# ZhongLingXiao/nano-kazen

Measured on AMD Instinct MI355X. Metric: Msamples/s (w*h*spp/s) at 1920x1080, 1 M-tri scene, higher is better.
Workload: dtype f32

## Files before the change

include/kazen_mi355x_dev.h:

```cpp
#ifndef KAZEN_MI355X_DEV_H
#define KAZEN_MI355X_DEV_H
#include "kazen_mi355x.h"
#ifdef __cplusplus
extern "C" {
#endif


typedef struct KzStats {
    uint64_t samples;
    uint64_t rays;
    uint64_t nodeVisits;
    uint64_t triTests;
    uint64_t shadedHits;
    uint64_t lightSamples;
    uint64_t droppedSamples;
    uint64_t beamPixels;
    uint64_t beamListEntries;
    uint64_t beamCompletePixels;
} KzStats;

typedef struct KzHit {
    float t;
    float u, v;
    int32_t mesh;
    int32_t prim;
    float p[3];
    float uv[2];
    float sh_s[3], sh_t[3], sh_n[3];
    float geo_n[3];
} KzHit;

typedef struct KzBvhInfo { uint32_t nNodes, nLeaves, nTris, maxDepth, maxLeafSize; float sahCost; double buildSeconds; } KzBvhInfo;
int kz_scene_bvh_info(const KzScene *scene, KzBvhInfo *out);
int kz_scene_sample_count(const KzScene *scene, uint32_t *out);

int kz_scene_devices(const KzScene *scene, int32_t *devices, uint32_t cap, uint32_t *count);

int kz_film_merge(float *dst, const float *src, size_t nFloats);

int kz_film_download_on(KzScene *scene, int device, float *film, size_t nFloats);
int kz_film_clear_on(KzScene *scene, int device, void *stream);
int kz_sync_on(KzScene *scene, int device);

int kz_trace_rays(KzScene *scene, uint32_t n, const float *o, const float *d,
                  const float *tmin, const float *tmax, KzHit *hits);

int kz_render_samples(KzScene *scene, uint32_t n, const int32_t *pxy, const uint32_t *idx, float *out);
int kz_bsdf_query(KzScene *scene, uint32_t n, const int32_t *bsdf, const float *wi, const float *wo, const float *accRough,
                  const float *s3, const float *uv, float *evalOut, float *pdfOut, float *sampleOut);
int kz_texture_query(KzScene *scene, uint32_t n, const int32_t *tex, const float *uv, float *out);

int kz_camera_rays(KzScene *scene, uint32_t n, const float *sxy, const float *axy, float *out);
int kz_light_query(KzScene *scene, uint32_t n, const int32_t *light, const float *ref, const float *u3, float *out);

int kz_set_stats(KzScene *scene, int enable);
int kz_get_stats(KzScene *scene, KzStats *out, int reset);

int kz_last_kernel_ms(KzScene *scene, float *ms);
int kz_last_stage_ms(KzScene *scene, float *out6);

typedef struct KzPassInfo { uint32_t passes; uint32_t passesInFlight; uint64_t itemsPerPass; uint32_t sppPerPass; uint32_t pixels; uint64_t stateBytes;
                            uint32_t pixelsPerPass; uint32_t shadowBeside ; uint64_t firstPassItems; uint64_t largestPassItems;
                            uint64_t contextItems;
                          } KzPassInfo;
int kz_last_pass_info(KzScene *scene, KzPassInfo *out);
typedef struct KzPassModeInfo { int32_t kept; uint32_t timedPasses; uint64_t items; float msOneStream[2]; float msShadowBeside; float msHalves; } KzPassModeInfo;
int kz_pass_mode_info(KzScene *scene, int device, KzPassModeInfo *out);
int kz_last_grow_note(KzScene *scene, char *buf, size_t cap);

void kz_debug_fail_alloc(int nth);
void kz_debug_fail_device(int device, int nth);
void kz_debug_grow_delay(int ms);
void kz_debug_trace(int on);
void kz_debug_alias_devices(int n);

typedef struct KzPlanQuery {
    int32_t pipeline;
    uint32_t nPix;
    uint32_t sampleBegin, sampleEnd;
    uint64_t passItems;
    int32_t passesInFlight;
    int32_t sppPerPass;
    uint64_t limitBytes;
    uint64_t bytesPerItem;
    int32_t dealer;
    uint32_t takers, batchTiles, nTiles;
    const uint32_t *tilePixOffset;
    uint64_t heldItems;
} KzPlanQuery;
typedef struct KzPlanAnswer {
    int32_t autoShape, nCtx, multi, grow;
    uint32_t S, pixPerPass, batchTiles, nPixSet, nPasses;
    uint64_t need, wantItems, minStart;
    double graceMs;
} KzPlanAnswer;
int kz_plan_passes(const KzPlanQuery *q, KzPlanAnswer *a);
int kz_plan_schedule(const KzPlanQuery *q, const uint64_t *avail, uint32_t nAvail, uint32_t pixBegin, uint32_t pixEnd, uint32_t *passes, uint32_t cap, uint32_t *nPasses);

int kz_kat_dpdf(uint32_t n, const float *values, float *cdf, float *sumAndNormalization);
int kz_kat_pow4(int32_t spp, int32_t *out4);

enum { KZ_TABLE_NODES = 0, KZ_TABLE_NODES4 = 1, KZ_TABLE_TRIS = 2, KZ_TABLE_SHADE = 3, KZ_TABLE_CDF = 4, KZ_TABLE_LIGHTS = 5, KZ_TABLE_IL_TRIS = 6, KZ_TABLE_PARAMS = 7,
       KZ_TABLE_BSDFS = 8  };
int kz_scene_table(KzScene *scene, int device, int table, void *out, size_t cap, size_t *bytes);

#define KZ_BUILD_EXPERIMENTS 1
int kz_build_flags(void);
int kz_device_mem_info(int device, uint64_t *freeBytes, uint64_t *totalBytes);
int kz_kat_exact_math(int device, uint64_t *rcpMismatches, uint64_t *sqrtMismatches, uint64_t *checked);
int kz_kat_permute(int device, uint32_t n, const uint32_t *i, const uint32_t *l, const uint32_t *p, uint32_t *out);
int kz_kat_fresnel(int device, uint32_t n, int form, const float *cosThetaI, const float *a, const float *b, float *out);
int kz_kat_math(int device, int fn, uint32_t n, const float *x, const float *y, float *out);


#ifdef __cplusplus
}
#endif
#endif
```

nano-kazen_amd/abi.py:

```python
import ctypes as C
import os

KZ_ABI_VERSION = 6

KZ_OK, KZ_ERR_INVALID_ARG, KZ_ERR_UNSUPPORTED, KZ_ERR_NO_DEVICE, KZ_ERR_HIP, KZ_ERR_STATE, KZ_ERR_OOM = range(7)
KZ_BSDF_DIFFUSE, KZ_BSDF_KAZENSTANDARD, KZ_BSDF_MIRROR, KZ_BSDF_DIELECTRIC = 0, 1, 2, 3
KZ_BSDF_GGX, KZ_BSDF_ROUGHCONDUCTOR, KZ_BSDF_ROUGHPLASTIC, KZ_BSDF_ROUGHDIELECTRIC, KZ_BSDF_NORMALMAP = 4, 5, 6, 7, 8
KZ_TEX_CONSTANT, KZ_TEX_IMAGE, KZ_TEX_COLORRAMP, KZ_TEX_BLEND = 0, 1, 2, 3
KZ_BLEND_MIX, KZ_BLEND_MULTIPLY, KZ_BLEND_NONE = 0, 1, 2
KZ_PIXEL_U8, KZ_PIXEL_F32 = 0, 1
KZ_TEX_MAX_DEPTH = 8
KZ_SAMPLER_INDEPENDENT, KZ_SAMPLER_PMJ02BN, KZ_SAMPLER_STRATIFIED, KZ_SAMPLER_CORRELATED = 0, 1, 2, 3
KZ_CAMERA_PERSPECTIVE, KZ_CAMERA_THINLENS = 0, 1
KZ_INTEGRATOR_PATH_MIS, KZ_INTEGRATOR_NORMALS, KZ_INTEGRATOR_AO, KZ_INTEGRATOR_PATH_MATS = 0, 1, 2, 3
KZ_FILTER_GAUSSIAN, KZ_FILTER_MITCHELL, KZ_FILTER_TENT, KZ_FILTER_BOX = 0, 1, 2, 3
KZ_FILTER_RESOLUTION = 32
KZ_PMJ02BN_SETS, KZ_PMJ02BN_SAMPLES = 5, 65536
KZ_BLUENOISE_TEXTURES, KZ_BLUENOISE_RES = 48, 128

f32p = C.POINTER(C.c_float)
u32p = C.POINTER(C.c_uint32)
u16p = C.POINTER(C.c_uint16)


# ... 10 lines not shown
class KzImage(C.Structure):
    _fields_ = [("pixels", C.c_void_p), ("width", C.c_int32), ("height", C.c_int32), ("channels", C.c_int32), ("format", C.c_int32)]


class KzTexture(C.Structure):
    _fields_ = [("type", C.c_int32), ("color", C.c_float * 3), ("image", C.c_int32), ("scale", C.c_float), ("srgb", C.c_int32),
                ("rampMin", C.c_float), ("rampMax", C.c_float), ("blendMode", C.c_int32), ("child", C.c_int32 * 3), ("filter", C.c_int32), ("pad_", C.c_int32 * 2)]


class KzLight(C.Structure):
    _fields_ = [("color", C.c_float * 3), ("intensity", C.c_float), ("primaryVisibility", C.c_int32)]


class KzMesh(C.Structure):
    _fields_ = [("V", f32p), ("N", f32p), ("UV", f32p), ("F", u32p), ("nV", C.c_uint32), ("nF", C.c_uint32),
                ("bsdf", C.c_int32), ("light", C.c_int32)]


class KzFilter(C.Structure):
    _fields_ = [("type", C.c_int32), ("radius", C.c_float), ("stddev", C.c_float), ("B", C.c_float), ("C", C.c_float)]


class KzCamera(C.Structure):
    _fields_ = [("type", C.c_int32), ("width", C.c_int32), ("height", C.c_int32), ("toWorld", C.c_float * 16),
                ("fov", C.c_float), ("nearClip", C.c_float), ("farClip", C.c_float),
                ("apertureRadius", C.c_float), ("focusDistance", C.c_float),
                ("sampleToCamera", f32p), ("rfilter", KzFilter)]


class KzSampler(C.Structure):
    _fields_ = [("type", C.c_int32), ("sampleCount", C.c_uint32), ("resolution", C.c_int32), ("pad_", C.c_int32), ("seed", C.c_uint64),
                ("pmj02bnSamples", u32p), ("blueNoise", u16p)]


class KzIntegrator(C.Structure):
    _fields_ = [("type", C.c_int32), ("maxDepth", C.c_int32), ("traceBias", C.c_float),
                ("regularization", C.c_int32), ("accumulatedRoughness", C.c_float)]


class KzBackground(C.Structure):
    _fields_ = [("present", C.c_int32), ("color", C.c_float * 3), ("intensity", C.c_float), ("texture", C.c_int32)]


class KzSceneDesc(C.Structure):
    _fields_ = [("abiVersion", C.c_uint32),
                ("meshes", C.POINTER(KzMesh)), ("nMeshes", C.c_uint32),
                ("bsdfs", C.POINTER(KzBSDF)), ("nBsdfs", C.c_uint32),
                ("lights", C.POINTER(KzLight)), ("nLights", C.c_uint32),
                ("camera", KzCamera), ("sampler", KzSampler), ("integrator", KzIntegrator),
                ("background", KzBackground),
                ("textures", C.POINTER(KzTexture)), ("nTextures", C.c_uint32),
                ("images", C.POINTER(KzImage)), ("nImages", C.c_uint32)]


class KzTile(C.Structure):
    _fields_ = [("x0", C.c_int32), ("y0", C.c_int32), ("w", C.c_int32), ("h", C.c_int32)]


class KzTuning(C.Structure):
    _fields_ = [("refill", C.c_int32), ("postpone", C.c_int32), ("batch", C.c_int32), ("traceBlocksPerCU", C.c_int32),
                ("shadeBlocksPerCU", C.c_int32), ("ldsStack", C.c_int32), ("dev0", C.c_int32), ("packetPrimary", C.c_int32),
                ("dev1", C.c_int32), ("dev2", C.c_int32), ("filmGather", C.c_int32), ("dev3", C.c_int32), ("sppPerPass", C.c_int32), ("dev4", C.c_int32),
                ("dev5", C.c_int32), ("streamPriority", C.c_int32)]


class KzTileDealer(C.Structure):
    _fields_ = [("counter", u32p), ("batchTiles", C.c_uint32), ("takers", C.c_uint32), ("taken", u32p), ("takenCap", C.c_uint32), ("nTaken", u32p), ("agreed", u32p)]


class KzRenderOpts(C.Structure):
    _fields_ = [("sampleBegin", C.c_uint32), ("sampleEnd", C.c_uint32), ("tiles", C.POINTER(KzTile)),
                ("nTiles", C.c_uint32), ("pipeline", C.c_int32), ("accumulate", C.c_int32), ("stream", C.c_void_p),
                ("device", C.c_int32), ("passesInFlight", C.c_int32), ("passItems", C.c_uint64), ("maxStateBytes", C.c_uint64),
                ("tune", KzTuning), ("tileDealing", C.c_int32), ("packedOutput", C.c_int32), ("dealer", C.POINTER(KzTileDealer)),
                ("shadowBeside", C.c_int32), ("passHalves", C.c_int32)]


class KzPassInfo(C.Structure):
    _fields_ = [("passes", C.c_uint32), ("passesInFlight", C.c_uint32), ("itemsPerPass", C.c_uint64), ("sppPerPass", C.c_uint32),
                ("pixels", C.c_uint32), ("stateBytes", C.c_uint64), ("pixelsPerPass", C.c_uint32), ("shadowBeside", C.c_uint32),
                ("firstPassItems", C.c_uint64), ("largestPassItems", C.c_uint64), ("contextItems", C.c_uint64)]

    def as_dict(self):
        return {k: int(getattr(self, k)) for k, _ in self._fields_}


class KzPassModeInfo(C.Structure):
    _fields_ = [("kept", C.c_int32), ("timedPasses", C.c_uint32), ("items", C.c_uint64), ("msOneStream", C.c_float * 2), ("msShadowBeside", C.c_float), ("msHalves", C.c_float)]


class KzPlanQuery(C.Structure):
    _fields_ = [("pipeline", C.c_int32), ("nPix", C.c_uint32), ("sampleBegin", C.c_uint32), ("sampleEnd", C.c_uint32), ("passItems", C.c_uint64),
                ("passesInFlight", C.c_int32), ("sppPerPass", C.c_int32), ("limitBytes", C.c_uint64), ("bytesPerItem", C.c_uint64), ("dealer", C.c_int32),
                ("takers", C.c_uint32), ("batchTiles", C.c_uint32), ("nTiles", C.c_uint32), ("tilePixOffset", u32p), ("heldItems", C.c_uint64)]


class KzPlanAnswer(C.Structure):
    _fields_ = [("autoShape", C.c_int32), ("nCtx", C.c_int32), ("multi", C.c_int32), ("grow", C.c_int32), ("S", C.c_uint32), ("pixPerPass", C.c_uint32),
                ("batchTiles", C.c_uint32), ("nPixSet", C.c_uint32), ("nPasses", C.c_uint32), ("need", C.c_uint64), ("wantItems", C.c_uint64),
                ("minStart", C.c_uint64), ("graceMs", C.c_double)]

    def as_dict(self):
        return {k: getattr(self, k) for k, _ in self._fields_}


class KzStats(C.Structure):
    _fields_ = [("samples", C.c_uint64), ("rays", C.c_uint64), ("nodeVisits", C.c_uint64), ("triTests", C.c_uint64),
                ("shadedHits", C.c_uint64), ("lightSamples", C.c_uint64), ("droppedSamples", C.c_uint64),
                ("beamPixels", C.c_uint64), ("beamListEntries", C.c_uint64), ("beamCompletePixels", C.c_uint64)]

    def as_dict(self):
        return {k: int(getattr(self, k)) for k, _ in self._fields_}


class KzHit(C.Structure):
    _fields_ = [("t", C.c_float), ("u", C.c_float), ("v", C.c_float), ("mesh", C.c_int32), ("prim", C.c_int32),
                ("p", C.c_float * 3), ("uv", C.c_float * 2), ("sh_s", C.c_float * 3), ("sh_t", C.c_float * 3),
                ("sh_n", C.c_float * 3), ("geo_n", C.c_float * 3)]


class KzVertexUpdate(C.Structure):
    _fields_ = [("mesh", C.c_uint32), ("nV", C.c_uint32), ("V", f32p), ("N", f32p)]


class KzBsdfUpdate(C.Structure):
    _fields_ = [("row", C.c_uint32), ("bsdf", KzBSDF)]


class KzLightUpdate(C.Structure):
    _fields_ = [("light", C.c_uint32), ("value", KzLight)]


class KzTransformUpdate(C.Structure):
    _fields_ = [("mesh", C.c_uint32), ("toWorld", C.c_float * 16)]


class KzBvhInfo(C.Structure):
    _fields_ = [("nNodes", C.c_uint32), ("nLeaves", C.c_uint32), ("nTris", C.c_uint32), ("maxDepth", C.c_uint32),
                ("maxLeafSize", C.c_uint32), ("sahCost", C.c_float), ("buildSeconds", C.c_double)]


PRODUCT_EXPORTS = ["kz_scene_create", "kz_scene_destroy", "kz_scene_upload", "kz_scene_evict", "kz_render", "kz_render_tiles", "kz_render_multi", "kz_deal_tiles",
                   "kz_tiles_packed_floats", "kz_film_download_tiles", "kz_film_merge_tiles", "kz_film_merge_rects", "kz_film_download", "kz_film_clear", "kz_film_dims", "kz_film_to_rgb",
                   "kz_film_to_srgb8", "kz_sync", "kz_last_error", "kz_abi_version", "kz_device_count", "kz_device_trim"]
EXPORTS = ["kz_scene_create", "kz_scene_destroy", "kz_scene_bvh_info", "kz_scene_upload", "kz_render",
           "kz_film_download", "kz_film_clear", "kz_film_dims", "kz_film_to_rgb", "kz_trace_rays",
           "kz_set_stats", "kz_get_stats", "kz_sync", "kz_last_kernel_ms", "kz_last_error", "kz_abi_version",
           "kz_device_count", "kz_render_samples", "kz_bsdf_query", "kz_scene_sample_count", "kz_last_stage_ms", "kz_texture_query", "kz_film_to_srgb8",
           "kz_scene_evict", "kz_scene_devices", "kz_render_tiles", "kz_render_multi", "kz_deal_tiles", "kz_film_merge", "kz_film_download_on",
           "kz_film_clear_on", "kz_sync_on", "kz_last_pass_info", "kz_device_mem_info", "kz_camera_rays", "kz_light_query", "kz_kat_exact_math", "kz_kat_permute", "kz_kat_fresnel", "kz_kat_math", "kz_build_flags",
           "kz_tiles_packed_floats", "kz_film_download_tiles", "kz_film_merge_tiles", "kz_film_merge_rects", "kz_device_trim", "kz_kat_dpdf", "kz_kat_pow4", "kz_last_grow_note",
           "kz_plan_passes", "kz_plan_schedule", "kz_pass_mode_info", "kz_scene_table"]
EDIT_EXPORTS = ["kz_scene_set_camera", "kz_scene_set_vertices", "kz_scene_set_bsdfs", "kz_scene_set_lights", "kz_scene_set_transforms"]
KZ_TABLE_NODES, KZ_TABLE_NODES4, KZ_TABLE_TRIS, KZ_TABLE_SHADE, KZ_TABLE_CDF, KZ_TABLE_LIGHTS, KZ_TABLE_IL_TRIS, KZ_TABLE_PARAMS, KZ_TABLE_BSDFS = range(9)
DEV_ONLY_EXPORTS = ["kz_debug_fail_alloc", "kz_debug_fail_device", "kz_debug_grow_delay", "kz_debug_trace", "kz_debug_alias_devices"]

_HERE = os.path.dirname(os.path.abspath(__file__))
LIB_PATH = os.environ.get("KZ_LIB_PATH") or os.path.join(_HERE, "csrc", "libkazen_mi355x.so")
DEV_LIB_PATH = os.path.join(_HERE, "csrc", "variants", "experiments", "libkazen_mi355x.so")
_libs = {}


class KzError(RuntimeError):
    def __init__(self, code, msg):
        super().__init__("kazen_mi355x error %d: %s" % (code, msg))
        self.code = code


def load_dev_library():
    return load_library(DEV_LIB_PATH)


def load_library(path=None):
    path = path or LIB_PATH
    if path in _libs:
        return _libs[path]
    if not os.path.exists(path):
        raise ImportError("HIP extension %s is missing: run `python -c 'import __graft_entry__ as g; g.build()'` "
                          "(the product path has no CPU fallback)" % path)
    lib = C.CDLL(path)
    lib.kz_last_error.restype = C.c_char_p
    lib.kz_scene_create.argtypes = [C.POINTER(KzSceneDesc), C.POINTER(C.c_void_p)]
    lib.kz_scene_destroy.argtypes = [C.c_void_p]
    lib.kz_scene_destroy.restype = None
    lib.kz_scene_bvh_info.argtypes = [C.c_void_p, C.POINTER(KzBvhInfo)]
    lib.kz_scene_sample_count.argtypes = [C.c_void_p, u32p]
    lib.kz_scene_upload.argtypes = [C.c_void_p, C.c_int]
    lib.kz_render.argtypes = [C.c_void_p, C.POINTER(KzRenderOpts)]
    lib.kz_film_download.argtypes = [C.c_void_p, f32p, C.c_size_t]
    lib.kz_film_clear.argtypes = [C.c_void_p, C.c_void_p]
    lib.kz_film_dims.argtypes = [C.c_void_p, C.POINTER(C.c_int32), C.POINTER(C.c_int32), C.POINTER(C.c_int32)]
    lib.kz_film_to_rgb.argtypes = [f32p, C.c_int32, C.c_int32, C.c_int32, f32p]
    lib.kz_trace_rays.argtypes = [C.c_void_p, C.c_uint32, f32p, f32p, f32p, f32p, C.POINTER(KzHit)]
    lib.kz_set_stats.argtypes = [C.c_void_p, C.c_int]
    lib.kz_get_stats.argtypes = [C.c_void_p, C.POINTER(KzStats), C.c_int]
    lib.kz_sync.argtypes = [C.c_void_p]
    lib.kz_last_kernel_ms.argtypes = [C.c_void_p, f32p]
    lib.kz_last_stage_ms.argtypes = [C.c_void_p, f32p]
    lib.kz_render_samples.argtypes = [C.c_void_p, C.c_uint32, C.POINTER(C.c_int32), u32p, f32p]
    lib.kz_bsdf_query.argtypes = [C.c_void_p, C.c_uint32, C.POINTER(C.c_int32), f32p, f32p, f32p, f32p, f32p, f32p, f32p, f32p]
    lib.kz_film_to_srgb8.argtypes = [C.c_void_p, C.POINTER(C.c_uint8), C.c_size_t]
    lib.kz_texture_query.argtypes = [C.c_void_p, C.c_uint32, C.POINTER(C.c_int32), f32p, f32p]
    if hasattr(lib, "kz_camera_rays"):
        lib.kz_camera_rays.argtypes = [C.c_void_p, C.c_uint32, f32p, f32p, f32p]
        lib.kz_light_query.argtypes = [C.c_void_p, C.c_uint32, C.POINTER(C.c_int32), f32p, f32p, f32p]
    lib.kz_scene_evict.argtypes = [C.c_void_p, C.c_int]
    lib.kz_scene_devices.argtypes = [C.c_void_p, C.POINTER(C.c_int32), C.c_uint32, u32p]
    lib.kz_render_tiles.argtypes = [C.c_void_p, C.POINTER(KzRenderOpts), C.POINTER(KzTile), C.c_uint32, C.c_int, f32p, C.c_size_t]
    lib.kz_render_multi.argtypes = [C.c_void_p, C.POINTER(KzRenderOpts), C.POINTER(C.c_int32), C.c_uint32, C.c_int32, f32p, C.c_size_t, f32p]
    lib.kz_deal_tiles.argtypes = [C.c_int32, C.c_int32, C.c_int32, C.c_uint32, C.c_uint32, C.POINTER(KzTile), C.c_uint32, u32p]
    lib.kz_film_merge.argtypes = [f32p, f32p, C.c_size_t]
    lib.kz_tiles_packed_floats.argtypes = [C.c_void_p, C.POINTER(KzTile), C.c_uint32, C.POINTER(C.c_size_t)]
    lib.kz_film_download_tiles.argtypes = [C.c_void_p, C.c_int, C.POINTER(KzTile), C.c_uint32, f32p, C.c_size_t]
    lib.kz_film_merge_tiles.argtypes = [f32p, C.c_int32, C.c_int32, C.c_int32, C.POINTER(KzTile), C.c_uint32, f32p, C.c_size_t, C.c_int32]
    lib.kz_film_merge_rects.argtypes = [f32p, C.c_int32, C.c_int32, C.c_int32, C.POINTER(KzTile), C.POINTER(f32p), C.c_uint32, C.c_int32]
    lib.kz_film_download_on.argtypes = [C.c_void_p, C.c_int, f32p, C.c_size_t]
    lib.kz_film_clear_on.argtypes = [C.c_void_p, C.c_int, C.c_void_p]
    lib.kz_sync_on.argtypes = [C.c_void_p, C.c_int]
    lib.kz_last_pass_info.argtypes = [C.c_void_p, C.POINTER(KzPassInfo)]
    lib.kz_pass_mode_info.argtypes = [C.c_void_p, C.c_int32, C.POINTER(KzPassModeInfo)]
    lib.kz_device_mem_info.argtypes = [C.c_int, C.POINTER(C.c_uint64), C.POINTER(C.c_uint64)]
    lib.kz_device_trim.argtypes = [C.c_int]
    lib.kz_last_grow_note.argtypes = [C.c_void_p, C.c_char_p, C.c_size_t]
    for hook in DEV_ONLY_EXPORTS:
        if hasattr(lib, hook):
            getattr(lib, hook).argtypes = [C.c_int, C.c_int] if hook == "kz_debug_fail_device" else [C.c_int]
            getattr(lib, hook).restype = None
    if hasattr(lib, "kz_plan_passes"):
        lib.kz_plan_passes.argtypes = [C.POINTER(KzPlanQuery), C.POINTER(KzPlanAnswer)]
        lib.kz_plan_schedule.argtypes = [C.POINTER(KzPlanQuery), C.POINTER(C.c_uint64), C.c_uint32, C.c_uint32, C.c_uint32, u32p, C.c_uint32, u32p]
    lib.kz_kat_dpdf.argtypes = [C.c_uint32, f32p, f32p, f32p]
    if hasattr(lib, "kz_scene_set_vertices"):
        lib.kz_scene_set_camera.argtypes = [C.c_void_p, C.POINTER(KzCamera)]
        lib.kz_scene_set_vertices.argtypes = [C.c_void_p, C.POINTER(KzVertexUpdate), C.c_uint32]
        lib.kz_scene_table.argtypes = [C.c_void_p, C.c_int, C.c_int, C.c_void_p, C.c_size_t, C.POINTER(C.c_size_t)]
    if hasattr(lib, "kz_scene_set_transforms"):
        lib.kz_scene_set_bsdfs.argtypes = [C.c_void_p, C.POINTER(KzBsdfUpdate), C.c_uint32]
        lib.kz_scene_set_lights.argtypes = [C.c_void_p, C.POINTER(KzLightUpdate), C.c_uint32]
        lib.kz_scene_set_transforms.argtypes = [C.c_void_p, C.POINTER(KzTransformUpdate), C.c_uint32]
    lib.kz_kat_pow4.argtypes = [C.c_int32, C.POINTER(C.c_int32)]
    if hasattr(lib, "kz_kat_math"):
        lib.kz_kat_math.argtypes = [C.c_int, C.c_int, C.c_uint32, f32p, f32p, f32p]
    if hasattr(lib, "kz_kat_fresnel"):
        lib.kz_kat_fresnel.argtypes = [C.c_int, C.c_uint32, C.c_int, f32p, f32p, f32p, f32p]
    if hasattr(lib, "kz_kat_permute"):
        lib.kz_kat_permute.argtypes = [C.c_int, C.c_uint32, u32p, u32p, u32p, u32p]
    if hasattr(lib, "kz_kat_exact_math"):
        lib.kz_kat_exact_math.argtypes = [C.c_int, C.POINTER(C.c_uint64), C.POINTER(C.c_uint64), C.POINTER(C.c_uint64)]
    _libs[path] = lib
    return lib


def check(lib, rc):
    if rc != KZ_OK:
        msg = lib.kz_last_error()
        raise KzError(rc, msg.decode() if msg else "")
```

nano-kazen_amd/csrc/kz_debug.hip:

```cpp
#include "kz_state.h"

#include <algorithm>
#include <atomic>
#include <chrono>
#include <cmath>
#include <cstdio>
#include <cstdlib>
#include <cstring>
#include <mutex>
#include <string>
#include <thread>
#include <vector>
#include "kz_devfn.h"


__global__ __launch_bounds__(KZ_BLOCK) void kz_trace_kernel(KzParams P, KzDevTables T, uint32_t n, const float *__restrict__ o,
                                                            const float *__restrict__ d, const float *__restrict__ tmin,
                                                            const float *__restrict__ tmax, KzHit *__restrict__ hits) {
    __shared__ uint32_t s_stack[KZ_STACK_DEPTH * KZ_BLOCK];
    const uint32_t i = blockIdx.x * KZ_BLOCK + threadIdx.x;
    if (i >= n) return;
    Counters cn = {0, 0, 0, 0, 0, 0};
    RawHit rh;
    KzHit h; memset(&h, 0, sizeof h);
// ... 131 lines not shown

int kz_kat_fresnel(int device, uint32_t n, int form, const float *cosThetaI, const float *a, const float *b, float *out) {
    int nd = kz_device_count();
    if (device < 0 || device >= nd) return kz_fail(nd ? KZ_ERR_INVALID_ARG : KZ_ERR_NO_DEVICE, "device %d out of range (%d visible)", device, nd);
    if (!n) return KZ_OK;
    if (!cosThetaI || !a || !out || (form == 0 && !b) || (form != 0 && form != 1)) return kz_fail(KZ_ERR_INVALID_ARG, "null argument or form %d (0 = fresnel(cos, extIOR, intIOR), 1 = fresnelDielectric(cos, eta))", form);
    HIP_TRY(hipSetDevice(kzPhysicalDevice(device)));
    DevMem dC, dA, dB, dO;
    const size_t bytes = (size_t)n * sizeof(float);
    KZ_ALLOC(&dC.p, bytes); KZ_ALLOC(&dA.p, bytes); KZ_ALLOC(&dB.p, bytes); KZ_ALLOC(&dO.p, 2 * bytes);
    HIP_TRY(hipMemcpy(dC.p, cosThetaI, bytes, hipMemcpyHostToDevice)); HIP_TRY(hipMemcpy(dA.p, a, bytes, hipMemcpyHostToDevice));
    HIP_TRY(hipMemcpy(dB.p, b ? b : a, bytes, hipMemcpyHostToDevice));
    hipLaunchKernelGGL(kz_fresnel_kernel, dim3((n + 255) / 256), dim3(256), 0, 0, n, form, dC.as<float>(), dA.as<float>(), dB.as<float>(), dO.as<float>());
    HIP_TRY(hipGetLastError());
    HIP_TRY(hipMemcpy(out, dO.p, 2 * bytes, hipMemcpyDeviceToHost));
    return KZ_OK;
}

int kz_kat_math(int device, int fn, uint32_t n, const float *x, const float *y, float *out) {
    int nd = kz_device_count();
    if (device < 0 || device >= nd) return kz_fail(nd ? KZ_ERR_INVALID_ARG : KZ_ERR_NO_DEVICE, "device %d out of range (%d visible)", device, nd);
    if (!n) return KZ_OK;
    if (!x || !out || fn < 0 || fn > 11) return kz_fail(KZ_ERR_INVALID_ARG, "null argument or function %d (0..11)", fn);
    HIP_TRY(hipSetDevice(kzPhysicalDevice(device)));
    DevMem dX, dY, dO;
    const size_t bytes = (size_t)n * sizeof(float);
    KZ_ALLOC(&dX.p, bytes); KZ_ALLOC(&dY.p, bytes); KZ_ALLOC(&dO.p, bytes);
    HIP_TRY(hipMemcpy(dX.p, x, bytes, hipMemcpyHostToDevice)); HIP_TRY(hipMemcpy(dY.p, y ? y : x, bytes, hipMemcpyHostToDevice));
    hipLaunchKernelGGL(kz_math_kernel, dim3((n + 255) / 256), dim3(256), 0, 0, n, fn, dX.as<float>(), dY.as<float>(), dO.as<float>());
    HIP_TRY(hipGetLastError());
    HIP_TRY(hipMemcpy(out, dO.p, bytes, hipMemcpyDeviceToHost));
    return KZ_OK;
}

int kz_kat_exact_math(int device, uint64_t *rcpMismatches, uint64_t *sqrtMismatches, uint64_t *checked) {
    int n = kz_device_count();
    if (device < 0 || device >= n) return kz_fail(n ? KZ_ERR_INVALID_ARG : KZ_ERR_NO_DEVICE, "device %d out of range (%d visible)", device, n);
    HIP_TRY(hipSetDevice(kzPhysicalDevice(device)));
    DevMem dC;
    KZ_ALLOC(&dC.p, 3 * sizeof(unsigned long long));
    HIP_TRY(hipMemset(dC.p, 0, 3 * sizeof(unsigned long long)));
    for (unsigned long long base = 0; base < (1ull << 32); base += (1ull << 28)) {
        hipLaunchKernelGGL(kz_exact_math_kernel, dim3(1u << 20), dim3(256), 0, 0, base, dC.as<unsigned long long>());
        HIP_TRY(hipGetLastError());
    }
    HIP_TRY(hipDeviceSynchronize());
    unsigned long long h[3];
    HIP_TRY(hipMemcpy(h, dC.p, sizeof h, hipMemcpyDeviceToHost));
    if (rcpMismatches) *rcpMismatches = h[0];
    if (sqrtMismatches) *sqrtMismatches = h[1];
    if (checked) *checked = h[2];
    return KZ_OK;
}

int kz_trace_rays(KzScene *scene, uint32_t n, const float *o, const float *d, const float *tmin, const float *tmax, KzHit *hits) {
    KzDeviceState *ds; int rc;
    if ((rc = requireDevice(scene, &ds))) return rc;
    if (n == 0) return KZ_OK;
    if (!o || !d || !tmin || !tmax || !hits) return kz_fail(KZ_ERR_INVALID_ARG, "null ray buffer");
    if ((rc = kzEnsureBvh2(scene, ds))) return rc;
    DevMem dO, dD, dA, dB, dH;
    KZ_ALLOC(&dO.p, (size_t)n * 12); KZ_ALLOC(&dD.p, (size_t)n * 12); KZ_ALLOC(&dA.p, (size_t)n * 4); KZ_ALLOC(&dB.p, (size_t)n * 4);
    KZ_ALLOC(&dH.p, (size_t)n * sizeof(KzHit));
    HIP_TRY(hipMemcpy(dO.p, o, (size_t)n * 12, hipMemcpyHostToDevice)); HIP_TRY(hipMemcpy(dD.p, d, (size_t)n * 12, hipMemcpyHostToDevice));
    HIP_TRY(hipMemcpy(dA.p, tmin, (size_t)n * 4, hipMemcpyHostToDevice)); HIP_TRY(hipMemcpy(dB.p, tmax, (size_t)n * 4, hipMemcpyHostToDevice));
    hipLaunchKernelGGL(kz_trace_kernel, dim3((n + KZ_BLOCK - 1) / KZ_BLOCK), dim3(KZ_BLOCK), 0, 0, scene->prm, ds->T, n, dO.as<float>(), dD.as<float>(), dA.as<float>(),
                       dB.as<float>(), dH.as<KzHit>());
    HIP_TRY(hipGetLastError());
    HIP_TRY(hipDeviceSynchronize());
    HIP_TRY(hipMemcpy(hits, dH.p, (size_t)n * sizeof(KzHit), hipMemcpyDeviceToHost));
    return KZ_OK;
}

int kz_bsdf_query(KzScene *scene, uint32_t n, const int32_t *bsdf, const float *wi, const float *wo, const float *accRough, const float *s3,
                  const float *uv, float *evalOut, float *pdfOut, float *sampleOut) {
    KzDeviceState *ds; int rc;
    if ((rc = requireDevice(scene, &ds))) return rc;
    if (n == 0) return KZ_OK;
    if (!bsdf || !wi || !wo || !accRough || !s3 || !evalOut || !pdfOut || !sampleOut) return kz_fail(KZ_ERR_INVALID_ARG, "null buffer");
    for (uint32_t i = 0; i < n; ++i) if (bsdf[i] < 0 || (size_t)bsdf[i] >= scene->bsdfs.size()) return kz_fail(KZ_ERR_INVALID_ARG, "bsdf index %d", bsdf[i]);
    DevMem dF, dBs;
    const size_t fl = (size_t)n * (3 + 3 + 1 + 3 + 3 + 1 + 8 + 2);
    KZ_ALLOC(&dF.p, fl * 4); KZ_ALLOC(&dBs.p, (size_t)n * 4);
    float *d = dF.as<float>(); int32_t *dB = dBs.as<int32_t>();
    float *dWi = d, *dWo = d + 3 * (size_t)n, *dAcc = d + 6 * (size_t)n, *dS = d + 7 * (size_t)n, *dE = d + 10 * (size_t)n, *dP = d + 13 * (size_t)n,
          *dSm = d + 14 * (size_t)n, *dUv = d + 22 * (size_t)n;
    HIP_TRY(hipMemcpy(dB, bsdf, (size_t)n * 4, hipMemcpyHostToDevice));
    HIP_TRY(hipMemcpy(dWi, wi, (size_t)n * 12, hipMemcpyHostToDevice)); HIP_TRY(hipMemcpy(dWo, wo, (size_t)n * 12, hipMemcpyHostToDevice));
    HIP_TRY(hipMemcpy(dAcc, accRough, (size_t)n * 4, hipMemcpyHostToDevice)); HIP_TRY(hipMemcpy(dS, s3, (size_t)n * 12, hipMemcpyHostToDevice));
    if (uv) HIP_TRY(hipMemcpy(dUv, uv, (size_t)n * 8, hipMemcpyHostToDevice));
    hipLaunchKernelGGL(kz_bsdf_kernel, dim3((n + 63) / 64), dim3(64), 0, 0, ds->T, n, dB, dWi, dWo, dAcc, dS, uv ? dUv : (const float *)nullptr, dE, dP, dSm);
    HIP_TRY(hipGetLastError());
    HIP_TRY(hipDeviceSynchronize());
    HIP_TRY(hipMemcpy(evalOut, dE, (size_t)n * 12, hipMemcpyDeviceToHost)); HIP_TRY(hipMemcpy(pdfOut, dP, (size_t)n * 4, hipMemcpyDeviceToHost));
    HIP_TRY(hipMemcpy(sampleOut, dSm, (size_t)n * 32, hipMemcpyDeviceToHost));
    return KZ_OK;
}

int kz_texture_query(KzScene *scene, uint32_t n, const int32_t *tex, const float *uv, float *out) {
    KzDeviceState *ds; int rc;
    if ((rc = requireDevice(scene, &ds))) return rc;
    if (n == 0) return KZ_OK;
    if (!tex || !uv || !out) return kz_fail(KZ_ERR_INVALID_ARG, "null buffer");
    for (uint32_t i = 0; i < n; ++i) if (tex[i] < 0 || (size_t)tex[i] >= scene->texProgs.size()) return kz_fail(KZ_ERR_INVALID_ARG, "texture index %d", tex[i]);
    DevMem dF, dTx;
    KZ_ALLOC(&dF.p, (size_t)n * 5 * 4); KZ_ALLOC(&dTx.p, (size_t)n * 4);
    float *d = dF.as<float>(); int32_t *dT = dTx.as<int32_t>();
    float *dUv = d, *dO = d + 2 * (size_t)n;
    HIP_TRY(hipMemcpy(dT, tex, (size_t)n * 4, hipMemcpyHostToDevice)); HIP_TRY(hipMemcpy(dUv, uv, (size_t)n * 8, hipMemcpyHostToDevice));
    hipLaunchKernelGGL(kz_texture_kernel, dim3((n + 63) / 64), dim3(64), 0, 0, ds->T, n, dT, dUv, dO);
    HIP_TRY(hipGetLastError());
    HIP_TRY(hipDeviceSynchronize());
    HIP_TRY(hipMemcpy(out, dO, (size_t)n * 12, hipMemcpyDeviceToHost));
    return KZ_OK;
}

int kz_camera_rays(KzScene *scene, uint32_t n, const float *sxy, const float *axy, float *out) {
    KzDeviceState *ds; int rc;
    if ((rc = requireDevice(scene, &ds))) return rc;
    if (n == 0) return KZ_OK;
    if (!sxy || !out) return kz_fail(KZ_ERR_INVALID_ARG, "null buffer");
    DevMem dF;
    KZ_ALLOC(&dF.p, (size_t)n * 12 * 4);
    float *d = dF.as<float>(), *dS = d, *dA = d + 2 * (size_t)n, *dO = d + 4 * (size_t)n;
    HIP_TRY(hipMemcpy(dS, sxy, (size_t)n * 8, hipMemcpyHostToDevice));
    if (axy) HIP_TRY(hipMemcpy(dA, axy, (size_t)n * 8, hipMemcpyHostToDevice));
    hipLaunchKernelGGL(kz_camera_kernel, dim3((n + 63) / 64), dim3(64), 0, 0, scene->prm, n, dS, axy ? dA : (const float *)nullptr, dO);
    HIP_TRY(hipGetLastError());
    HIP_TRY(hipDeviceSynchronize());
    HIP_TRY(hipMemcpy(out, dO, (size_t)n * 32, hipMemcpyDeviceToHost));
    return KZ_OK;
}

int kz_light_query(KzScene *scene, uint32_t n, const int32_t *light, const float *ref, const float *u3, float *out) {
    KzDeviceState *ds; int rc;
    if ((rc = requireDevice(scene, &ds))) return rc;
    if (n == 0) return KZ_OK;
    if (!light || !ref || !u3 || !out) return kz_fail(KZ_ERR_INVALID_ARG, "null buffer");
    for (uint32_t i = 0; i < n; ++i) if (light[i] < 0 || (uint32_t)light[i] >= scene->prm.nLights) return kz_fail(KZ_ERR_INVALID_ARG, "light index %d", light[i]);
    DevMem dF, dL;
    KZ_ALLOC(&dF.p, (size_t)n * 20 * 4); KZ_ALLOC(&dL.p, (size_t)n * 4);
    float *d = dF.as<float>(), *dR = d, *dU = d + 3 * (size_t)n, *dO = d + 6 * (size_t)n;
    HIP_TRY(hipMemcpy(dL.p, light, (size_t)n * 4, hipMemcpyHostToDevice));
    HIP_TRY(hipMemcpy(dR, ref, (size_t)n * 12, hipMemcpyHostToDevice)); HIP_TRY(hipMemcpy(dU, u3, (size_t)n * 12, hipMemcpyHostToDevice));
    hipLaunchKernelGGL(kz_light_kernel, dim3((n + 63) / 64), dim3(64), 0, 0, ds->T, n, dL.as<int32_t>(), dR, dU, dO);
    HIP_TRY(hipGetLastError());
    HIP_TRY(hipDeviceSynchronize());
    HIP_TRY(hipMemcpy(out, dO, (size_t)n * 56, hipMemcpyDeviceToHost));
    return KZ_OK;
}


}
```

nano-kazen_amd/csrc/kz_host.cpp:

```cpp
#include "kz_internal.h"

#include <algorithm>
#include <cmath>
#include <cstdarg>
#include <cstdio>
#include <cstring>

static thread_local char g_err[512] = "";

int kz_fail(int code, const char *fmt, ...) {
    va_list ap; va_start(ap, fmt);
    std::vsnprintf(g_err, sizeof g_err, fmt, ap);
    va_end(ap);
    return code;
}

namespace {

bool isPowerOf4(int n) {
    if (n <= 0) return false;
    int x = (int)std::sqrt((double)n);
    if (x * x != n) return false;
    return !(n & (n - 1));
}
// ... 19 lines not shown
}
bool mat4inv(const double *m, double *out) {
    double a[4][8];
    for (int i = 0; i < 4; ++i) for (int j = 0; j < 4; ++j) { a[i][j] = m[i * 4 + j]; a[i][j + 4] = (i == j); }
    for (int c = 0; c < 4; ++c) {
        int piv = c; for (int r = c + 1; r < 4; ++r) if (std::fabs(a[r][c]) > std::fabs(a[piv][c])) piv = r;
        if (a[piv][c] == 0) return false;
        if (piv != c) for (int j = 0; j < 8; ++j) std::swap(a[c][j], a[piv][j]);
        double inv = 1.0 / a[c][c];
        for (int j = 0; j < 8; ++j) a[c][j] *= inv;
        for (int r = 0; r < 4; ++r) if (r != c) { double f = a[r][c]; for (int j = 0; j < 8; ++j) a[r][j] -= f * a[c][j]; }
    }
    for (int i = 0; i < 4; ++i) for (int j = 0; j < 4; ++j) out[i * 4 + j] = a[i][j + 4];
    return true;
}

float filterEval(const KzFilter &f, float x) {
    switch (f.type) {
    case KZ_FILTER_GAUSSIAN: {
        float alpha = -1.0f / (2.0f * f.stddev * f.stddev);
        return std::max(0.0f, std::exp(alpha * x * x) - std::exp(alpha * f.radius * f.radius));
    }
    case KZ_FILTER_MITCHELL: {
        float B = f.B, C = f.C;
        x = std::fabs(2.0f * x / f.radius);
        float x2 = x * x, x3 = x2 * x;
        if (x < 1) return 1.0f / 6.0f * ((12 - 9 * B - 6 * C) * x3 + (-18 + 12 * B + 6 * C) * x2 + (6 - 2 * B));
        if (x < 2) return 1.0f / 6.0f * ((-B - 6 * C) * x3 + (6 * B + 30 * C) * x2 + (-12 * B - 48 * C) * x + (8 * B + 24 * C));
        return 0.0f;
    }
    case KZ_FILTER_TENT: return std::max(0.0f, 1.0f - std::fabs(x));
    default: return 1.0f;
    }
}

const uint64_t PCG32_MULT = 0x5851f42d4c957f2dULL;

static int emitTexture(const KzSceneDesc *d, KzScene *sc, int32_t t, int depthBudget, int &stackNow, int &stackMax) {
    if (depthBudget <= 0) return kz_fail(KZ_ERR_UNSUPPORTED, "texture graph is cyclic or deeper than 32 levels");
    if (sc->texOps.size() > (1u << 16)) return kz_fail(KZ_ERR_UNSUPPORTED, "texture graphs flatten to more than 65536 operations");
    const KzTexture &k = d->textures[t];
    KzTexOp op; std::memset(&op, 0, sizeof op);
    auto pushConst = [&](float v) { KzTexOp c; std::memset(&c, 0, sizeof c); c.op = KZ_TOP_CONST; c.f0 = c.f1 = c.f2 = v; sc->texOps.push_back(c); stackNow++; stackMax = std::max(stackMax, stackNow); };
    auto child = [&](int i, float dflt) -> int {
        const int32_t c = k.child[i];
        if (c < 0) { pushConst(dflt); return KZ_OK; }
        if (c >= (int32_t)d->nTextures) return kz_fail(KZ_ERR_INVALID_ARG, "texture %d: child %d out of range", t, c);
        return emitTexture(d, sc, c, depthBudget - 1, stackNow, stackMax);
    };
    switch (k.type) {
    case KZ_TEX_CONSTANT:
        op.op = KZ_TOP_CONST; op.f0 = k.color[0]; op.f1 = k.color[1]; op.f2 = k.color[2];
        sc->texOps.push_back(op); stackNow++; stackMax = std::max(stackMax, stackNow);
        return KZ_OK;
    case KZ_TEX_IMAGE:
        if (k.image < 0 || k.image >= (int32_t)d->nImages) return kz_fail(KZ_ERR_INVALID_ARG, "texture %d: image index %d out of range", t, k.image);
        if (k.filter != KZ_TEXFILTER_BILINEAR && k.filter != KZ_TEXFILTER_BICUBIC) return kz_fail(KZ_ERR_INVALID_ARG, "texture %d: filter %d (KZ_TEXFILTER_BILINEAR or KZ_TEXFILTER_BICUBIC)", t, k.filter);
        op.op = KZ_TOP_IMAGE; op.a = (uint32_t)k.image; op.f0 = k.scale; op.b = (k.srgb ? 1u : 0u) | ((uint32_t)k.filter << 1);
        {
            const KzImageRow &row = sc->images[(size_t)k.image];
            const uint32_t off16 = (uint32_t)(row.offset >> 4), wh = (uint32_t)(row.width - 1) | ((uint32_t)(row.height - 1) << 16);
            if ((row.offset >> 4) >> 32) return kz_fail(KZ_ERR_UNSUPPORTED, "more than 64 GB of texels");
            std::memcpy(&op.f1, &off16, 4); std::memcpy(&op.f2, &wh, 4);
            op.b |= ((uint32_t)row.channels << 8) | ((uint32_t)row.format << 16);
        }
        sc->texOps.push_back(op); stackNow++; stackMax = std::max(stackMax, stackNow);
        return KZ_OK;
    case KZ_TEX_COLORRAMP: {
        if (k.child[0] < 0) { pushConst(0.f); return KZ_OK; }
        int rc = child(0, 0.f); if (rc != KZ_OK) return rc;
        op.op = KZ_TOP_RAMP; op.f0 = k.rampMin; op.f1 = k.rampMax;
        sc->texOps.push_back(op);
        return KZ_OK; }
    case KZ_TEX_BLEND: {
        if (k.blendMode < KZ_BLEND_MIX || k.blendMode > KZ_BLEND_NONE) return kz_fail(KZ_ERR_INVALID_ARG, "texture %d: blend mode %d", t, k.blendMode);
        int rc = child(0, 0.5f); if (rc != KZ_OK) return rc;
        rc = child(1, 0.f); if (rc != KZ_OK) return rc;
        rc = child(2, 1.f); if (rc != KZ_OK) return rc;
        op.op = KZ_TOP_BLEND; op.a = (uint32_t)k.blendMode;
        sc->texOps.push_back(op); stackNow -= 2;
        return KZ_OK; }
    default:
        return kz_fail(KZ_ERR_UNSUPPORTED, "texture %d has type %d (supported: constanttexture, imagetexture, colorramp, blend)", t, k.type);
    }
}
static int flattenTextures(const KzSceneDesc *d, KzScene *sc) {
    for (uint32_t i = 0; i < d->nImages; ++i) {
        const KzImage &im = d->images[i];
        if (!im.pixels || im.width <= 0 || im.height <= 0 || im.channels <= 0 || im.channels > 16 || im.width > 65536 || im.height > 65536 ||
            (im.format != KZ_PIXEL_U8 && im.format != KZ_PIXEL_F32))
            return kz_fail(KZ_ERR_INVALID_ARG, "image %u: %dx%dx%d format %d", i, im.width, im.height, im.channels, im.format);
        const size_t bytes = (size_t)im.width * im.height * im.channels * (im.format == KZ_PIXEL_F32 ? 4 : 1);
        KzImageRow row; row.offset = (sc->texels.size() + 15) & ~(size_t)15; row.width = im.width; row.height = im.height; row.channels = im.channels; row.format = im.format;
        sc->texels.resize(row.offset + bytes);
        std::memcpy(sc->texels.data() + row.offset, im.pixels, bytes);
        sc->images.push_back(row);
        if ((im.width & (im.width - 1)) || (im.height & (im.height - 1))) sc->texPow2 = 0;
    }
    for (uint32_t t = 0; t < d->nTextures; ++t) {
        KzTexProg pr; pr.start = (uint32_t)sc->texOps.size();
        int now = 0, mx = 0;
        int rc = emitTexture(d, sc, (int32_t)t, 32, now, mx);
        if (rc != KZ_OK) return rc;
        if (mx > KZ_TEX_MAX_DEPTH) return kz_fail(KZ_ERR_UNSUPPORTED, "texture %u needs an operand stack of %d (limit %d)", t, mx, KZ_TEX_MAX_DEPTH);
        pr.count = ((uint32_t)sc->texOps.size() - pr.start) | ((uint32_t)mx << 16);
        sc->texProgs.push_back(pr);
    }
    return KZ_OK;
}

}

void kzLightCdf(const KzTriShade *shade, uint32_t nF, std::vector<float> &t, float &normalization) {
    t.assign(1, 0.0f);
    for (uint32_t f = 0; f < nF; ++f) {
        const KzTriShade &s = shade[f];
        float e1[3], e2[3];
        for (int a = 0; a < 3; ++a) { e1[a] = s.p[3 + a] - s.p[a]; e2[a] = s.p[6 + a] - s.p[a]; }
        float cx = e1[1] * e2[2] - e1[2] * e2[1], cy = e1[2] * e2[0] - e1[0] * e2[2], cz = e1[0] * e2[1] - e1[1] * e2[0];
        float area = 0.5f * std::sqrt(cx * cx + cy * cy + cz * cz);
        t.push_back(t.back() + area);
    }
    normalization = dpdfNormalize(t, 0, nullptr);
}

void kzInvisibleLights(KzScene *sc) {
    KzParams &p = sc->prm;
    sc->ilTris.clear();
    p.shadowFast = 1; p.nIlTris = 0; p.anyInvisibleLight = 0;
    uint32_t ilGidLo = 0xFFFFFFFFu, ilGidHi = 0;
    for (int a = 0; a < 3; ++a) { p.ilLo[a] = INFINITY; p.ilHi[a] = -INFINITY; }
    for (const KzLightRow &lr : sc->lightRows) {
        if (lr.primaryVisibility) continue;
        p.anyInvisibleLight = 1;
        if (lr.nF) { ilGidLo = std::min(ilGidLo, lr.triOffset); ilGidHi = std::max(ilGidHi, lr.triOffset + lr.nF - 1); }
        for (uint32_t f = 0; f < lr.nF; ++f) {
            const KzTriShade &s = sc->shade[lr.triOffset + f];
            KzTri t; std::memset(&t, 0, sizeof t);
            for (int a = 0; a < 3; ++a) {
                t.p0[a] = s.p[a]; t.e1[a] = s.p[3 + a] - s.p[a]; t.e2[a] = s.p[6 + a] - s.p[a];
                for (int v = 0; v < 3; ++v) { p.ilLo[a] = std::min(p.ilLo[a], s.p[3 * v + a]); p.ilHi[a] = std::max(p.ilHi[a], s.p[3 * v + a]); }
            }
            t.mesh = lr.mesh; t.prim = f; t.gid = lr.triOffset + f;
            sc->ilTris.push_back(t);
        }
    }
    if (sc->ilTris.size() > 64) { p.shadowFast = 0; sc->ilTris.clear(); }
    p.nIlTris = (uint32_t)sc->ilTris.size();
    p.ilGidLo = ilGidLo <= ilGidHi ? ilGidLo : 1u; p.ilGidSpan = ilGidLo <= ilGidHi ? ilGidHi - ilGidLo : 0u;
    for (int a = 0; a < 3; ++a) {
        float m = std::max(std::fabs(p.ilLo[a]), std::fabs(p.ilHi[a]));
        if (std::isfinite(m)) { float e = m * 4e-7f + 1e-30f; p.ilLo[a] -= e; p.ilHi[a] += e; }
    }
}

int kzCheckBsdfs(const char *who, const KzBSDF *rows, uint32_t n, uint32_t nTextures, int32_t integ) {
    for (uint32_t i = 0; i < n; ++i) {
        const KzBSDF &b = rows[i];
        if (b.type < KZ_BSDF_DIFFUSE || b.type > KZ_BSDF_NORMALMAP)
            return kz_fail(KZ_ERR_UNSUPPORTED, "%sbsdf %u has type %d (supported: diffuse, kazenstandard, mirror, dielectric, ggx, roughconductor, roughplastic, roughdielectric, normalmap)", who, i, b.type);
        const int32_t ids[4] = {b.albedoTex, b.roughnessTex, b.metallicTex, b.normalTex};
        for (int32_t id : ids) if (id < 0 || id > (int32_t)nTextures) return kz_fail(KZ_ERR_INVALID_ARG, "%sbsdf %u: texture id %d out of range (0 = constant, 1..%u)", who, i, id, nTextures);
        const bool takesAlbedo = b.type == KZ_BSDF_DIFFUSE || b.type == KZ_BSDF_GGX || b.type == KZ_BSDF_KAZENSTANDARD;
        if ((b.albedoTex && !takesAlbedo) || ((b.roughnessTex || b.metallicTex) && b.type != KZ_BSDF_KAZENSTANDARD) || (b.normalTex && b.type != KZ_BSDF_NORMALMAP))
            return kz_fail(KZ_ERR_INVALID_ARG, "%sbsdf %u (type %d): a texture id is set on a parameter this model does not read through a texture", who, i, b.type);
        const bool rough = b.type == KZ_BSDF_ROUGHCONDUCTOR || b.type == KZ_BSDF_ROUGHPLASTIC || b.type == KZ_BSDF_ROUGHDIELECTRIC;
        if ((b.alphaResolved != 0 && b.alphaResolved != 1) || (b.alphaResolved && !rough))
            return kz_fail(KZ_ERR_INVALID_ARG, "%sbsdf %u (type %d): alphaResolved = %d (0 or 1, and only roughconductor / roughplastic / roughdielectric rows have a resolved alpha)", who, i, b.type, b.alphaResolved);
        if (b.type == KZ_BSDF_NORMALMAP && integ == KZ_INTEGRATOR_PATH_MATS)
            return kz_fail(KZ_ERR_UNSUPPORTED, "%sbsdf %u is a normalmap: path_mats does not support normal maps (its BSDF record carries no intersection frame)", who, i);
        if (b.type == KZ_BSDF_NORMALMAP) {
            if (b.normalTex == 0) return kz_fail(KZ_ERR_INVALID_ARG, "%sbsdf %u: normalmap without a normal texture", who, i);
            if (b.nested < 0 || b.nested >= (int32_t)n || rows[b.nested].type == KZ_BSDF_NORMALMAP)
                return kz_fail(KZ_ERR_INVALID_ARG, "%sbsdf %u: normalmap needs a nested BSDF row that is not itself a normalmap (got %d)", who, i, b.nested);
        }
    }
    return KZ_OK;
}
void kzResolveBsdf(KzBSDF &b) {
    if ((b.type == KZ_BSDF_ROUGHCONDUCTOR || b.type == KZ_BSDF_ROUGHPLASTIC || b.type == KZ_BSDF_ROUGHDIELECTRIC) && !b.alphaResolved) {
        const float MIN_ALPHA = 0.001f, a2 = b.alpha * b.alpha;
        b.alpha = std::max(MIN_ALPHA, a2); b.alphaResolved = 1;
    }
}
int32_t kzBsdfExt(const std::vector<KzBSDF> &rows) {
    int32_t ext = 0;
    for (const KzBSDF &b : rows) {
        if (b.type == KZ_BSDF_NORMALMAP) ext |= 4 | 2;
        else if (b.type > KZ_BSDF_KAZENSTANDARD) ext |= 1;
        if (b.albedoTex || b.roughnessTex || b.metallicTex) ext |= 2;
    }
    return ext;
}

int kzCameraParams(const KzCamera &c, KzParams &p) {
    if (c.type != KZ_CAMERA_PERSPECTIVE && c.type != KZ_CAMERA_THINLENS) return kz_fail(KZ_ERR_UNSUPPORTED, "camera type %d is not supported (\"perspective\", \"thinlens\")", c.type);
    p.width = c.width; p.height = c.height;
    p.invW = 1.0f / (float)c.width; p.invH = 1.0f / (float)c.height;
    p.nearClip = c.nearClip; p.farClip = c.farClip;
    std::memcpy(p.c2w, c.toWorld, sizeof p.c2w);
    if (c.sampleToCamera) std::memcpy(p.s2c, c.sampleToCamera, sizeof p.s2c);
    else {
        float aspect = c.width / (float)c.height;
        float recip = 1.0f / (c.farClip - c.nearClip);
        float cot = 1.0f / std::tan((c.fov / 2.0f) * (3.14159265358979323846f / 180.0f));
        double P[16] = {cot, 0, 0, 0, 0, cot, 0, 0, 0, 0, (double)(c.farClip * recip), (double)(-c.nearClip * c.farClip * recip), 0, 0, 1, 0};
        double T[16] = {1, 0, 0, -1, 0, 1, 0, (double)(-1.0f / aspect), 0, 0, 1, 0, 0, 0, 0, 1};
        double D[16] = {-0.5, 0, 0, 0, 0, (double)(-0.5f * aspect), 0, 0, 0, 0, 1, 0, 0, 0, 0, 1};
        double TP[16], M[16], Mi[16];
        mat4mul(T, P, TP); mat4mul(D, TP, M);
        if (!mat4inv(M, Mi)) return kz_fail(KZ_ERR_INVALID_ARG, "singular projection (fov %g, clip %g..%g)", c.fov, c.nearClip, c.farClip);
        for (int i = 0; i < 16; ++i) p.s2c[i] = (float)Mi[i];
    }
    {
        const float *m = p.s2c, *w = p.c2w;
        p.beamOk = 0;
        for (int r = 0; r < 3; ++r) p.beamO[r] = p.beamA[r] = p.beamU[r] = p.beamV[r] = 0.f;
        const float tiny = 1e-9f * std::fabs(m[15]);
        if (c.type != KZ_CAMERA_THINLENS && std::fabs(m[12]) <= tiny && std::fabs(m[13]) <= tiny && m[15] != 0.f && w[12] == 0.f && w[13] == 0.f && w[14] == 0.f && w[15] != 0.f) {
            const double rw = m[15];
            const double A[3] = {m[3] / rw, m[7] / rw, m[11] / rw}, U[3] = {m[0] * (double)p.invW / rw, m[4] * (double)p.invW / rw, m[8] * (double)p.invW / rw},
                         V[3] = {m[1] * (double)p.invH / rw, m[5] * (double)p.invH / rw, m[9] * (double)p.invH / rw};
            bool fin = true;
            for (int r = 0; r < 3; ++r) {
                p.beamA[r] = (float)(w[4 * r] * A[0] + w[4 * r + 1] * A[1] + w[4 * r + 2] * A[2]);
                p.beamU[r] = (float)(w[4 * r] * U[0] + w[4 * r + 1] * U[1] + w[4 * r + 2] * U[2]);
                p.beamV[r] = (float)(w[4 * r] * V[0] + w[4 * r + 1] * V[1] + w[4 * r + 2] * V[2]);
                p.beamO[r] = w[4 * r + 3] / w[15];
                fin = fin && std::isfinite(p.beamA[r]) && std::isfinite(p.beamU[r]) && std::isfinite(p.beamV[r]) && std::isfinite(p.beamO[r]);
            }
            p.beamOk = fin ? 1 : 0;
        }
    }
    p.cameraType = c.type; p.apertureRadius = c.apertureRadius; p.focusDistance = c.focusDistance;
    return KZ_OK;
}

namespace {
}

extern "C" {

const char *kz_last_error(void) { return g_err; }
int kz_abi_version(void) { return KZ_ABI_VERSION; }

int kz_kat_dpdf(uint32_t n, const float *values, float *cdf, float *sumAndNormalization) {
    if ((n && !values) || !cdf || !sumAndNormalization) return kz_fail(KZ_ERR_INVALID_ARG, "null argument");
    std::vector<float> t(1, 0.0f);
    for (uint32_t i = 0; i < n; ++i) t.push_back(t.back() + values[i]);
    sumAndNormalization[1] = dpdfNormalize(t, 0, &sumAndNormalization[0]);
    std::memcpy(cdf, t.data(), t.size() * sizeof(float));
    return KZ_OK;
}
int kz_kat_pow4(int32_t spp, int32_t *out4) {
    if (spp < 1 || !out4) return kz_fail(KZ_ERR_INVALID_ARG, "kz_kat_pow4(%d)", spp);
    out4[0] = isPowerOf4(spp) ? 1 : 0; out4[1] = roundUpPow4(spp); out4[2] = log4i((uint32_t)out4[1]); out4[3] = pmjPixelTile((uint32_t)spp);
    return KZ_OK;
}
int kz_build_flags(void) {
#ifdef KZ_EXPERIMENTS
    return KZ_BUILD_EXPERIMENTS;
#else
    return 0;
#endif
}

int kz_scene_create(const KzSceneDesc *d, KzScene **out) {
    if (!d || !out) return kz_fail(KZ_ERR_INVALID_ARG, "kz_scene_create: null argument");
    *out = nullptr;
    if (d->abiVersion != KZ_ABI_VERSION) return kz_fail(KZ_ERR_INVALID_ARG, "ABI version %u, library is %u", d->abiVersion, KZ_ABI_VERSION);
    if (d->camera.type != KZ_CAMERA_PERSPECTIVE && d->camera.type != KZ_CAMERA_THINLENS) return kz_fail(KZ_ERR_UNSUPPORTED, "camera type %d is not supported (\"perspective\", \"thinlens\")", d->camera.type);
    const int32_t integ = d->integrator.type;
    if (integ != KZ_INTEGRATOR_PATH_MIS && integ != KZ_INTEGRATOR_NORMALS && integ != KZ_INTEGRATOR_AO && integ != KZ_INTEGRATOR_PATH_MATS)
        return kz_fail(KZ_ERR_UNSUPPORTED, "integrator type %d is not on the hot path (\"path_mis\", \"normals\", \"ao\", \"path_mats\")", integ);
    if (d->sampler.type < KZ_SAMPLER_INDEPENDENT || d->sampler.type > KZ_SAMPLER_CORRELATED)
        return kz_fail(KZ_ERR_UNSUPPORTED, "sampler type %d is not supported (\"independent\", \"pmj02bn\", \"stratified\", \"correlated\")", d->sampler.type);
    if (d->sampler.type == KZ_SAMPLER_STRATIFIED && (d->sampler.resolution < 1 || d->sampler.resolution > 256)) return kz_fail(KZ_ERR_INVALID_ARG, "stratified resolution %d", d->sampler.resolution);
    if (d->sampler.sampleCount > 65536) return kz_fail(KZ_ERR_UNSUPPORTED, "sampleCount %u (limit 65536)", d->sampler.sampleCount);
    if (d->camera.rfilter.type < KZ_FILTER_GAUSSIAN || d->camera.rfilter.type > KZ_FILTER_BOX) return kz_fail(KZ_ERR_UNSUPPORTED, "rfilter type %d", d->camera.rfilter.type);
    if (d->camera.width <= 0 || d->camera.height <= 0 || d->camera.width > 65535 || d->camera.height > 65535) return kz_fail(KZ_ERR_INVALID_ARG, "image size %dx%d", d->camera.width, d->camera.height);
    if (d->sampler.sampleCount == 0) return kz_fail(KZ_ERR_INVALID_ARG, "sampleCount is 0");
    if (!(d->camera.rfilter.radius > 0.f) || d->camera.rfilter.radius > 4.0f) return kz_fail(KZ_ERR_UNSUPPORTED, "filter radius %g (supported: (0, 4])", d->camera.rfilter.radius);
    if ((d->nMeshes && !d->meshes) || (d->nBsdfs && !d->bsdfs) || (d->nLights && !d->lights)) return kz_fail(KZ_ERR_INVALID_ARG, "null table with non-zero count");
    if ((d->nTextures && !d->textures) || (d->nImages && !d->images)) return kz_fail(KZ_ERR_INVALID_ARG, "null texture/image table with non-zero count");
    { const int brc = kzCheckBsdfs("", d->bsdfs, d->nBsdfs, d->nTextures, integ); if (brc != KZ_OK) return brc; }

    KzScene *sc = new KzScene();
    std::memset(&sc->prm, 0, sizeof sc->prm);
    sc->bsdfs.assign(d->bsdfs, d->bsdfs + d->nBsdfs);
    for (KzBSDF &b : sc->bsdfs) kzResolveBsdf(b);
    sc->nDescBsdfs = d->nBsdfs; sc->nDescLights = d->nLights;
    { int trc = flattenTextures(d, sc); if (trc != KZ_OK) { delete sc; return trc; } }
    int defaultBsdf = -1;

    std::vector<KzBuildTri> bt;
    size_t totalF = 0;
    for (uint32_t m = 0; m < d->nMeshes; ++m) totalF += d->meshes[m].nF;
    if (totalF >= (1ull << 28)) { delete sc; return kz_fail(KZ_ERR_UNSUPPORTED, "%zu triangles (limit 2^28)", totalF); }
    bt.reserve(totalF); sc->shade.reserve(totalF); sc->triVtx.reserve(3 * totalF);
    uint32_t gid = 0;
    for (uint32_t m = 0; m < d->nMeshes; ++m) {
        const KzMesh &km = d->meshes[m];
        if (!km.V || !km.F) { delete sc; return kz_fail(KZ_ERR_INVALID_ARG, "mesh %u has no V/F", m); }
        if (km.bsdf >= (int)d->nBsdfs || km.light >= (int)d->nLights || km.bsdf < -1 || km.light < -1) { delete sc; return kz_fail(KZ_ERR_INVALID_ARG, "mesh %u: bsdf/light index out of range", m); }
        KzMeshRow row; std::memset(&row, 0, sizeof row);
        row.bsdf = km.bsdf; row.light = -1;
        if (km.bsdf < 0) {
            if (defaultBsdf < 0) {
                KzBSDF b; std::memset(&b, 0, sizeof b);
                b.type = KZ_BSDF_DIFFUSE; b.albedo[0] = b.albedo[1] = b.albedo[2] = 0.5f;
                defaultBsdf = (int)sc->bsdfs.size(); sc->bsdfs.push_back(b);
            }
            row.bsdf = defaultBsdf;
        }
        row.flags = (km.N ? 1u : 0u) | (km.UV ? 2u : 0u);
        row.triOffset = gid; row.nF = km.nF;
        const int32_t lightRow = km.light >= 0 ? (int32_t)sc->lightRows.size() : -1;
        for (uint32_t f = 0; f < km.nF; ++f, ++gid) {
            uint32_t idx[3] = {km.F[3 * f], km.F[3 * f + 1], km.F[3 * f + 2]};
            KzBuildTri t; t.mesh = m; t.prim = f; t.gid = gid;
            KzTriShade s; std::memset(&s, 0, sizeof s);
            s.mesh = m; s.prim = f; s.bsdf = (uint32_t)row.bsdf; s.lightFlags = ((uint32_t)(lightRow + 1) << 2) | row.flags;
            for (int v = 0; v < 3; ++v) {
                if (idx[v] >= km.nV) { delete sc; return kz_fail(KZ_ERR_INVALID_ARG, "mesh %u face %u: vertex index %u >= %u", m, f, idx[v], km.nV); }
                for (int a = 0; a < 3; ++a) {
                    t.v[v][a] = km.V[3 * (size_t)idx[v] + a];
                    s.p[3 * v + a] = t.v[v][a];
                    if (km.N) s.n[3 * v + a] = km.N[3 * (size_t)idx[v] + a];
                }
                if (km.UV) { s.uv[2 * v] = km.UV[2 * (size_t)idx[v]]; s.uv[2 * v + 1] = km.UV[2 * (size_t)idx[v] + 1]; }
            }
            bt.push_back(t); sc->shade.push_back(s);
            sc->triVtx.insert(sc->triVtx.end(), idx, idx + 3);
        }
        if (km.light >= 0) {
            const KzLight &kl = d->lights[km.light];
            KzLightRow lr; std::memset(&lr, 0, sizeof lr);
            for (int a = 0; a < 3; ++a) lr.radiance[a] = kl.intensity * kl.color[a];
            lr.primaryVisibility = kl.primaryVisibility ? 1 : 0;
            while (sc->cdf.size() & 3u) sc->cdf.push_back(2.0f);
            lr.mesh = m; lr.triOffset = row.triOffset; lr.nF = km.nF; lr.cdfOffset = (uint32_t)sc->cdf.size(); lr.hasN = km.N ? 1u : 0u;
            std::vector<float> t;
            kzLightCdf(&sc->shade[row.triOffset], km.nF, t, lr.normalization);
            sc->cdf.insert(sc->cdf.end(), t.begin(), t.end());
            row.light = (int32_t)sc->lightRows.size();
            sc->lightRows.push_back(lr);
            sc->lightDesc.push_back((uint32_t)km.light);
        }
        sc->meshRows.push_back(row);
        sc->meshNV.push_back(km.nV);
    }
    sc->cdf.insert(sc->cdf.end(), 8, 2.0f);
    std::string berr;
    uint32_t rootRef = 0xFFFFFFFFu;
    int rc = kz_build_bvh(bt, sc->nodes, sc->tris, rootRef, sc->bvh, berr);
    if (rc != KZ_OK) { delete sc; return kz_fail(rc, "BVH build: %s", berr.c_str()); }

    KzParams &p = sc->prm;
    p.rootRef = rootRef;
    { int sb = 1; uint32_t r4 = rootRef;
      rc = kz_collapse_bvh4(sc->nodes, rootRef, sc->nodes4, r4, sb, &sc->slotSrc);
      if (rc != KZ_OK) { delete sc; return kz_fail(rc, "BVH4 collapse failed"); }
      if (sc->nodes4.size() > (size_t(1) << 26)) { delete sc; return kz_fail(KZ_ERR_UNSUPPORTED, "scene too large: %zu BVH4 packets (limit 2^26 = 4 GB of packets)", sc->nodes4.size()); }
      p.rootRef4 = r4; p.stackBound4 = sb; }
    p.stackDepth = (int32_t)std::max<uint32_t>(2u, sc->bvh.maxDepth + 1);
    p.bsdfExt = kzBsdfExt(sc->bsdfs);
    kzInvisibleLights(sc);
    const KzCamera &c = d->camera;
    if ((rc = kzCameraParams(c, p)) != KZ_OK) { delete sc; return rc; }
    sc->rfilter = c.rfilter;
    const KzFilter &rf = c.rfilter;
    p.filterRadius = rf.radius;
    p.border = (int)std::ceil(rf.radius - 0.5f);
    for (int i = 0; i < KZ_FILTER_RESOLUTION; ++i) sc->filter[i] = filterEval(rf, (rf.radius * i) / KZ_FILTER_RESOLUTION);
    sc->filter[KZ_FILTER_RESOLUTION] = 0.0f;
    p.lookupFactor = KZ_FILTER_RESOLUTION / rf.radius;
    p.tapLo = (int)std::floor(-rf.radius - 0.5f) + 1;
    p.tapHi = (int)std::floor(rf.radius + 0.5f);
    if (p.tapHi - p.tapLo + 1 > KZ_MAX_FILTER_TAPS) { delete sc; return kz_fail(KZ_ERR_UNSUPPORTED, "filter radius %g needs too many taps", rf.radius); }
    p.integrator = integ;
    if (integ == KZ_INTEGRATOR_PATH_MIS) {
        p.maxDepth = std::min(512, d->integrator.maxDepth);
        p.traceBias = d->integrator.traceBias;
        p.regularization = d->integrator.regularization ? 1 : 0;
        p.accumulatedRoughness = d->integrator.accumulatedRoughness;
    } else {
        p.maxDepth = integ == KZ_INTEGRATOR_PATH_MATS ? KZ_PATH_MATS_MAX_DEPTH : 1;
        p.traceBias = 1e-5f; p.regularization = 0; p.accumulatedRoughness = 0.f;
    }
    p.nLights = (uint32_t)sc->lightRows.size();
    p.lightPickPdf = p.nLights ? 1.f / (float)p.nLights : 0.f;
    p.lightPickScale = (p.nLights && (p.nLights & (p.nLights - 1)) == 0) ? (float)p.nLights : 0.f;
    p.bgPresent = d->background.present ? 1 : 0;
    p.bgImage = -1; p.bgIntensity = d->background.intensity;
    {
        float col[3] = {d->background.color[0], d->background.color[1], d->background.color[2]};
        if (d->background.present && d->background.texture != 0) {
            const int32_t t = d->background.texture - 1;
            if (t < 0 || (uint32_t)t >= d->nTextures) { delete sc; return kz_fail(KZ_ERR_INVALID_ARG, "background texture id %d out of range", d->background.texture); }
            const KzTexture &k = d->textures[t];
            if (k.type == KZ_TEX_CONSTANT) { col[0] = k.color[0]; col[1] = k.color[1]; col[2] = k.color[2]; }
            else if (k.type == KZ_TEX_IMAGE) {
                if (k.image < 0 || (uint32_t)k.image >= d->nImages) { delete sc; return kz_fail(KZ_ERR_INVALID_ARG, "background image index %d out of range", k.image); }
                if (k.filter != KZ_TEXFILTER_BILINEAR && k.filter != KZ_TEXFILTER_BICUBIC) { delete sc; return kz_fail(KZ_ERR_INVALID_ARG, "background texture: filter %d", k.filter); }
                p.bgImage = k.image; p.bgFilter = k.filter; col[0] = col[1] = col[2] = 0.f;
            } else col[0] = col[1] = col[2] = 0.f;
        }
        for (int a = 0; a < 3; ++a) p.bgRadiance[a] = d->background.present ? d->background.intensity * col[a] : 0.f;
    }
    p.samplerType = d->sampler.type;
    p.seed = d->sampler.seed;
    p.sampleCount = d->sampler.sampleCount;
    p.resX = p.resY = 1;
    if (d->sampler.type == KZ_SAMPLER_STRATIFIED) {
        int res = d->sampler.resolution;
        while ((uint32_t)(res * res) < p.sampleCount) res++;
        p.resX = p.resY = res; p.sampleCount = (uint32_t)(res * res);
    }
    if (d->sampler.type == KZ_SAMPLER_CORRELATED) {
        int r1 = (int)std::sqrt((double)p.sampleCount);
        int r0 = (int)((p.sampleCount + r1 - 1) / r1);
        p.resX = r0; p.resY = r1; p.sampleCount = (uint32_t)(r0 * r1);
    }
    if (d->sampler.type == KZ_SAMPLER_PMJ02BN) {
        if (!d->sampler.pmj02bnSamples || !d->sampler.blueNoise) { delete sc; return kz_fail(KZ_ERR_INVALID_ARG, "pmj02bn sampler without its tables"); }
        if (p.sampleCount > KZ_PMJ02BN_SAMPLES) p.sampleCount = KZ_PMJ02BN_SAMPLES;
        const size_t nPmj = (size_t)KZ_PMJ02BN_SETS * KZ_PMJ02BN_SAMPLES * 2, nBn = (size_t)KZ_BLUENOISE_TEXTURES * KZ_BLUENOISE_RES * KZ_BLUENOISE_RES;
        sc->pmj.resize(nPmj); sc->bn.resize(nBn);
        for (size_t i = 0; i < nPmj; ++i) sc->pmj[i] = (float)((double)d->sampler.pmj02bnSamples[i] * 0x1p-32);
        for (size_t i = 0; i < nBn; ++i) sc->bn[i] = (float)d->sampler.blueNoise[i] / 65535.f;
        uint32_t spp = p.sampleCount;
        int tile = pmjPixelTile(spp);
        p.pixelTileSize = tile;
        sc->pixelSamples.assign((size_t)tile * tile * spp * 2, 0.f);
        std::vector<uint32_t> nStored((size_t)tile * tile, 0);
        for (int i = 0; i < KZ_PMJ02BN_SAMPLES; ++i) {
            float x = sc->pmj[2 * (size_t)i], y = sc->pmj[2 * (size_t)i + 1];
            x *= tile; y *= tile;
            int ix = (int)x, iy = (int)y;
            if (ix >= tile || iy >= tile) { delete sc; return kz_fail(KZ_ERR_INVALID_ARG, "pmj02bn table entry %d rounds to 1.0f (the reference would index out of range)", i); }
            size_t po = (size_t)ix + (size_t)iy * tile;
            if (nStored[po] == spp) continue;
            size_t so = po * spp + nStored[po];
            sc->pixelSamples[2 * so] = x - std::floor(x);
            sc->pixelSamples[2 * so + 1] = y - std::floor(y);
            ++nStored[po];
        }
    } else {
        sc->jump.resize(p.sampleCount);
        for (uint32_t s = 0; s < p.sampleCount; ++s) {
            uint64_t cur_mult = PCG32_MULT, cur_plus = 1u, acc_mult = 1u, acc_plus = 0u;
            uint64_t delta = (uint64_t)s * 65536ull;
            while (delta > 0) {
                if (delta & 1) { acc_mult *= cur_mult; acc_plus = acc_plus * cur_mult + cur_plus; }
                cur_plus = (cur_mult + 1) * cur_plus;
                cur_mult *= cur_mult;
                delta /= 2;
            }
            sc->jump[s].mult = acc_mult; sc->jump[s].plus = acc_plus;
        }
    }
    p.sppPow2 = (p.sampleCount & (p.sampleCount - 1)) == 0 ? 1 : 0;
    p.invSpp = 1.0f / (float)p.sampleCount;
    kz_device_init(sc);
    *out = sc;
    return KZ_OK;
}

void kz_scene_destroy(KzScene *scene) {
    if (!scene) return;
    kz_device_release(scene);
    delete scene;
}

int kz_scene_bvh_info(const KzScene *scene, KzBvhInfo *out) {
    if (!scene || !out) return kz_fail(KZ_ERR_INVALID_ARG, "null argument");
    kzHostSync(const_cast<KzScene *>(scene));
    *out = scene->bvh;
    return KZ_OK;
}

int kz_scene_sample_count(const KzScene *scene, uint32_t *out) {
    if (!scene || !out) return kz_fail(KZ_ERR_INVALID_ARG, "null argument");
    *out = scene->prm.sampleCount;
    return KZ_OK;
}

int kz_film_dims(const KzScene *scene, int32_t *width, int32_t *height, int32_t *border) {
    if (!scene) return kz_fail(KZ_ERR_INVALID_ARG, "null scene");
    if (width) *width = scene->prm.width;
    if (height) *height = scene->prm.height;
    if (border) *border = scene->prm.border;
    return KZ_OK;
}

int kz_film_to_rgb(const float *film, int32_t width, int32_t height, int32_t border, float *rgb) {
    if (!film || !rgb || width <= 0 || height <= 0 || border < 0) return kz_fail(KZ_ERR_INVALID_ARG, "kz_film_to_rgb: bad argument");
    size_t cols = (size_t)width + 2 * (size_t)border;
    for (int y = 0; y < height; ++y)
        for (int x = 0; x < width; ++x) {
            const float *px = film + ((size_t)(y + border) * cols + (size_t)(x + border)) * 4;
            float *o = rgb + ((size_t)y * width + x) * 3;
            if (px[3] != 0) { o[0] = px[0] / px[3]; o[1] = px[1] / px[3]; o[2] = px[2] / px[3]; }
            else { o[0] = o[1] = o[2] = 0.f; }
        }
    return KZ_OK;
}

}
```

nano-kazen_amd/csrc/kz_internal.h:

```cpp
#pragma once
#include "../../include/kazen_mi355x_dev.h"
#include "../../include/kazen_mi355x_edit.h"

#include <cstdint>
#include <mutex>
#include <string>
#include <vector>

#define KZ_STACK_DEPTH 32
#define KZ_MAX_LEAF 4
#define KZ_MAX_FILTER_TAPS 9
#define KZ_PATH_MATS_MAX_DEPTH 512

struct KzNode { float q[12]; uint32_t child[2]; uint32_t pad[2]; };
static_assert(sizeof(KzNode) == 64, "node packet must be 64 B");

struct KzNode4 { float p[3]; float scaleX; uint32_t qlo[3]; uint32_t qhi[3]; float scaleY, scaleZ; uint32_t child[4]; };
static_assert(sizeof(KzNode4) == 64, "BVH4 packet must be 64 B");

struct KzTri { float p0[3]; float e1[3]; float e2[3]; uint32_t mesh, prim, gid; };
static_assert(sizeof(KzTri) == 48, "leaf triangle must be 48 B");

struct KzTriShade { float p[9]; float n[9]; float uv[6]; uint32_t mesh, prim, bsdf, lightFlags; };
static_assert(sizeof(KzTriShade) == 112, "shading record must be 112 B");

struct KzMeshRow {
    int32_t bsdf;
    int32_t light;
    uint32_t flags;
    uint32_t triOffset;
    uint32_t nF;
    uint32_t pad[3];
};
struct KzLightRow {
    float radiance[3];
    int32_t primaryVisibility;
    uint32_t mesh;
    uint32_t triOffset;
    uint32_t nF;
    uint32_t cdfOffset;
    float normalization;
    uint32_t hasN;
    uint32_t pad[2];
};
enum { KZ_TOP_CONST = 0, KZ_TOP_IMAGE = 1, KZ_TOP_RAMP = 2, KZ_TOP_BLEND = 3 };
struct KzTexOp {
    uint32_t op;
    uint32_t a;
    float f0, f1, f2;
    uint32_t b;
    uint32_t pad[2];
};
static_assert(sizeof(KzTexOp) == 32, "texture op must be 32 B");
struct KzTexProg { uint32_t start, count; };
struct KzImageRow { uint64_t offset; int32_t width, height, channels, format; };
static_assert(sizeof(KzBSDF) == 128, "BSDF row must be 128 B");

struct KzPcgJump { uint64_t mult, plus; };

struct KzParams {
    float s2c[16];
    float c2w[16];
    float invW, invH, nearClip, farClip;
    int32_t width, height, border;
    int32_t maxDepth; float traceBias; int32_t regularization; float accumulatedRoughness;
    int32_t samplerType; uint32_t sampleCount; uint64_t seed; int32_t pixelTileSize;
    int32_t resX, resY;
    int32_t sppPow2; float invSpp;
    int32_t cameraType; float apertureRadius, focusDistance;
    uint32_t nLights; float lightPickPdf;
    float lightPickScale;
    int32_t bgPresent; float bgRadiance[3];
    int32_t bgImage; float bgIntensity;
    int32_t bgFilter;
    int32_t integrator;
    float filterRadius, lookupFactor; int32_t tapLo, tapHi;
    uint32_t rootRef;
    uint32_t rootRef4; int32_t stackBound4;
    int32_t shadowFast; uint32_t nIlTris; float ilLo[3], ilHi[3];
    int32_t anyInvisibleLight; int32_t stackDepth;
    uint32_t ilGidLo, ilGidSpan;
    int32_t beamOk; float beamO[3], beamA[3], beamU[3], beamV[3];
    int32_t bsdfExt;
};

struct KzDevTables {
    const KzNode *nodes;
    const KzNode4 *nodes4;
    const KzTri *tris;
    const KzTriShade *shade;
    const KzMeshRow *meshes;
    const KzBSDF *bsdfs;
    const KzLightRow *lights;
    const float *cdf;
    const float *pmj;
    const float *bn;
    const float *pixelSamples;
    const KzPcgJump *jump;
    const float *filter;
    const KzTri *ilTris;
    const KzTexProg *texProgs;
    const KzTexOp *texOps;
    const KzImageRow *images;
    const uint8_t *texels;
    uint32_t texPow2;
};

struct KzXform {
    float m[16];
    double c[9];
    double det;
};

struct KzScene {
    std::vector<KzNode> nodes;
    std::vector<KzNode4> nodes4;
    std::vector<KzTri> tris;
    std::vector<KzTriShade> shade;
    std::vector<KzMeshRow> meshRows;
    std::vector<KzBSDF> bsdfs;
    std::vector<KzLightRow> lightRows;
    std::vector<float> cdf;
    std::vector<float> pmj;
    std::vector<float> bn;
    std::vector<float> pixelSamples;
    std::vector<KzPcgJump> jump;
    std::vector<KzTri> ilTris;
    std::vector<KzTexProg> texProgs;
    std::vector<KzTexOp> texOps;
    std::vector<KzImageRow> images;
    std::vector<uint8_t> texels;
    float filter[KZ_FILTER_RESOLUTION + 1];
    KzParams prm;
    uint32_t texPow2 = 1;
    KzBvhInfo bvh;
    KzFilter rfilter;
    std::vector<uint32_t> triVtx;
    std::vector<uint32_t> meshNV;
    std::vector<uint32_t> slotSrc;
    std::vector<uint32_t> levelStart;
    std::vector<std::vector<float>> pendV, pendN;
    uint32_t nDescBsdfs = 0, nDescLights = 0;
    std::vector<uint32_t> lightDesc;
    std::vector<std::vector<float>> baseV, baseN;
    std::vector<KzXform> pendX;
    std::vector<uint8_t> pendXOn;
    bool hostStale = false;
    std::mutex editMutex;
    void *dev = nullptr;
};

struct KzBuildTri { float v[3][3]; uint32_t mesh, prim, gid; };
int kz_build_bvh(const std::vector<KzBuildTri> &in, std::vector<KzNode> &nodes, std::vector<KzTri> &tris,
                 uint32_t &rootRef, KzBvhInfo &info, std::string &err);
int kz_collapse_bvh4(const std::vector<KzNode> &nodes, uint32_t rootRef, std::vector<KzNode4> &out, uint32_t &rootRef4, int &stackBound,
                     std::vector<uint32_t> *slotSrc = nullptr);

int kz_fail(int code, const char *fmt, ...);
int kzCameraParams(const KzCamera &c, KzParams &p);
void kzLightCdf(const KzTriShade *shade, uint32_t nF, std::vector<float> &t, float &normalization);
void kzInvisibleLights(KzScene *sc);
int kzCheckBsdfs(const char *who, const KzBSDF *rows, uint32_t n, uint32_t nTextures, int32_t integrator);
void kzResolveBsdf(KzBSDF &b);
int32_t kzBsdfExt(const std::vector<KzBSDF> &rows);

void kzHostSync(KzScene *scene);
int kzEditWait(KzScene *scene);
int kzEditPrepare(KzScene *scene);
int kzEditBeamsUnbuilt(KzScene *scene);
int kzEditVertices(KzScene *scene, const KzVertexUpdate *u, uint32_t n, const std::vector<uint32_t> &lightRows);
int kzEditBsdfRows(KzScene *scene, const uint32_t *rows, uint32_t n, bool extChanged);
int kzEditLightRows(KzScene *scene);
struct KzXformJob { uint32_t mesh; const KzXform *x; };
int kzEditReplicaCount(KzScene *scene);
int kzEditXformStage(KzScene *scene, const KzXformJob *jobs, uint32_t n, int32_t *bad);
int kzEditXformCommit(KzScene *scene, const KzXformJob *jobs, uint32_t n, const std::vector<uint32_t> &lightRows);

void kz_device_init(KzScene *scene);
void kz_device_release(KzScene *scene);
```

nano-kazen_amd/csrc/kz_refit.hip:

```cpp
#include <hip/hip_runtime.h>

#include "kz_state.h"
#include "kz_refit.h"
#include "kz_xform.h"

#include <algorithm>
#include <cstring>
#include <vector>

#define KZ_EDIT_BLOCK 256

__global__ __launch_bounds__(KZ_EDIT_BLOCK) void kz_edit_shade(KzTriShade *__restrict__ shade, const uint32_t *__restrict__ triVtx, uint32_t gid0, uint32_t nF,
                                                               const float *__restrict__ V, const float *__restrict__ N) {
    const uint32_t f = blockIdx.x * KZ_EDIT_BLOCK + threadIdx.x;
    if (f >= nF) return;
    const size_t g = (size_t)gid0 + f;
    KzTriShade &s = shade[g];
    for (int v = 0; v < 3; ++v) {
        const size_t i = triVtx[3 * g + v];
        for (int a = 0; a < 3; ++a) {
            s.p[3 * v + a] = V[3 * i + a];
            if (N) s.n[3 * v + a] = N[3 * i + a];
        }
    }
}

__global__ __launch_bounds__(KZ_EDIT_BLOCK) void kz_edit_xform(const float *__restrict__ baseV, const float *__restrict__ baseN, float *__restrict__ outV, float *__restrict__ outN,
                                                               uint32_t nV, KzXform x, uint32_t *__restrict__ flag) {
    const uint32_t i = blockIdx.x * KZ_EDIT_BLOCK + threadIdx.x;
    if (i >= nV) return;
    const size_t o = 3 * (size_t)i;
    const float p[3] = {baseV[o], baseV[o + 1], baseV[o + 2]};
    float q[3];
    kzXfPoint(x, p, q);
    outV[o] = q[0]; outV[o + 1] = q[1]; outV[o + 2] = q[2];
    if (!kzFinite(q[0]) || !kzFinite(q[1]) || !kzFinite(q[2])) flag[0] = 1u;
    if (baseN) {
        const float n[3] = {baseN[o], baseN[o + 1], baseN[o + 2]};
        float r[3];
        kzXfNormal(x, n, r);
        outN[o] = r[0]; outN[o + 1] = r[1]; outN[o + 2] = r[2];
    }
}

__global__ __launch_bounds__(KZ_EDIT_BLOCK) void kz_edit_tris(KzTri *__restrict__ tris, const KzTriShade *__restrict__ shade, uint32_t n) {
    const uint32_t i = blockIdx.x * KZ_EDIT_BLOCK + threadIdx.x;
    if (i >= n) return;
    KzTri &t = tris[i];
    const float *p = shade[t.gid].p;
    for (int a = 0; a < 3; ++a) { t.p0[a] = p[a]; t.e1[a] = __fsub_rn(p[3 + a], p[a]); t.e2[a] = __fsub_rn(p[6 + a], p[a]); }
}

__global__ __launch_bounds__(KZ_EDIT_BLOCK) void kz_edit_level(KzNode *__restrict__ nodes, const KzTri *__restrict__ tris, const KzTriShade *__restrict__ shade,
                                                               uint32_t first, uint32_t count, float *__restrict__ absPad) {
    const uint32_t i = blockIdx.x * KZ_EDIT_BLOCK + threadIdx.x;
    if (i >= count) return;
    const uint32_t h = first + i;
    KzNode &nd = nodes[h];
    KzBox b[2];
    for (int k = 0; k < 2; ++k) {
        const uint32_t c = nd.child[k];
        if (c & 0x80000000u) kzLeafBox(b[k], tris, shade, c);
        else { KzBox r; kzNodeBox(nodes[c].q, 0, b[k]); kzNodeBox(nodes[c].q, 1, r); kzBoxGrow(b[k], r); }
    }
    kzSetNodeBox(nd.q, 0, b[0]); kzSetNodeBox(nd.q, 1, b[1]);
    if (h == 0) { KzBox root = b[0]; kzBoxGrow(root, b[1]); absPad[0] = kzAbsPad(root); }
}

__global__ __launch_bounds__(KZ_EDIT_BLOCK) void kz_edit_pad(KzNode *__restrict__ nodes, uint32_t n, const float *__restrict__ absPad) {
    const uint32_t h = blockIdx.x * KZ_EDIT_BLOCK + threadIdx.x;
    if (h >= n) return;
    const float pad = absPad[0];
    for (int k = 0; k < 2; ++k) { KzBox b; kzNodeBox(nodes[h].q, k, b); kzPadBox(b, pad); kzSetNodeBox(nodes[h].q, k, b); }
}

__global__ __launch_bounds__(KZ_EDIT_BLOCK) void kz_edit_quant(KzNode4 *__restrict__ nodes4, uint32_t n, const KzNode *__restrict__ nodes, const uint32_t *__restrict__ slotSrc) {
    const uint32_t h = blockIdx.x * KZ_EDIT_BLOCK + threadIdx.x;
    if (h >= n) return;
    KzBox cb[4]; int cnt = 0;
    for (int i = 0; i < 4; ++i) { const uint32_t s = slotSrc[4 * (size_t)h + i]; if (s == 0xFFFFFFFFu) break; kzNodeBox(nodes[s >> 1].q, (int)(s & 1u), cb[cnt++]); }
    KzNode4 nd = nodes4[h];
    kzQuantiseNode4(nd, cb, cnt);
    nodes4[h] = nd;
}

static inline dim3 editGrid(size_t n) { return dim3((unsigned)((n + KZ_EDIT_BLOCK - 1) / KZ_EDIT_BLOCK)); }

template <class Fn> static int forEachReplica(KzScene *scene, Fn fn) {
    KzReplicaSet *rs = replicaSet(scene);
    std::vector<KzDeviceState *> v;
    { std::lock_guard<std::mutex> g(rs->m); v = rs->v; }
    for (KzDeviceState *ds : v) {
        HIP_TRY(hipSetDevice(ds->hipDevice));
        const int rc = fn(ds);
        if (rc != KZ_OK) return rc;
    }
    return KZ_OK;
}

int kzEditWait(KzScene *scene) {
    return forEachReplica(scene, [](KzDeviceState *) -> int { HIP_TRY(hipDeviceSynchronize()); return KZ_OK; });
}

static int beamsUnbuilt(KzDeviceState *ds) {
    if (ds->beamCount) HIP_TRY(hipMemset(ds->beamCount, 0xFF, ds->beamCap * sizeof(uint2)));
    ds->beamDone.clear();
    return KZ_OK;
}

int kzEditBeamsUnbuilt(KzScene *scene) {
    return forEachReplica(scene, [](KzDeviceState *ds) -> int {
        const int rc = beamsUnbuilt(ds); if (rc) return rc;
        HIP_TRY(hipDeviceSynchronize());
        return KZ_OK;
    });
}

int kzEditPrepare(KzScene *scene) {
    return forEachReplica(scene, [scene](KzDeviceState *ds) -> int {
        int rc;
        if ((rc = kzEnsureBvh2(scene, ds))) return rc;
        auto up = [&](const std::vector<uint32_t> &v, uint32_t **out) -> int {
            if (*out) return KZ_OK;
            void *p = nullptr;
            const size_t bytes = std::max<size_t>(256, v.size() * sizeof(uint32_t));
            KZ_ALLOC(&p, bytes);
            ds->allocs.push_back(p);
            if (!v.empty()) HIP_TRY(hipMemcpy(p, v.data(), v.size() * sizeof(uint32_t), hipMemcpyHostToDevice));
            *out = (uint32_t *)p; ds->editBytes += bytes;
            return KZ_OK;
        };
        if ((rc = up(scene->triVtx, &ds->editTriVtx))) return rc;
        if ((rc = up(scene->slotSrc, &ds->editSlotSrc))) return rc;
        if (!ds->editPad) {
            void *p = nullptr;
            KZ_ALLOC(&p, 256);
            ds->allocs.push_back(p); ds->editPad = (float *)p; ds->editBytes += 256;
        }
        return KZ_OK;
    });
}

static int stageRoom(KzDeviceState *ds, size_t floats) {
    if (ds->editStageCap >= floats) return KZ_OK;
    if (ds->editStage) { (void)hipFree(ds->editStage); ds->editBytes -= ds->editStageCap * sizeof(float); ds->editStage = nullptr; ds->editStageCap = 0; }
    KZ_ALLOC(&ds->editStage, floats * sizeof(float));
    ds->editStageCap = floats; ds->editBytes += floats * sizeof(float);
    return KZ_OK;
}

static int refitChain(KzScene *scene, KzDeviceState *ds, const std::vector<uint32_t> &lightRows) {
    KzTri *tris = const_cast<KzTri *>(ds->T.tris);
    KzNode *nodes = const_cast<KzNode *>(ds->T.nodes);
    if (!scene->tris.empty()) hipLaunchKernelGGL(kz_edit_tris, editGrid(scene->tris.size()), dim3(KZ_EDIT_BLOCK), 0, 0, tris, ds->T.shade, (uint32_t)scene->tris.size());
    if (!scene->nodes.empty()) {
        const std::vector<uint32_t> &L = scene->levelStart;
        for (size_t d = L.size() - 1; d-- > 0;)
            hipLaunchKernelGGL(kz_edit_level, editGrid(L[d + 1] - L[d]), dim3(KZ_EDIT_BLOCK), 0, 0, nodes, (const KzTri *)tris, ds->T.shade, L[d], L[d + 1] - L[d], ds->editPad);
        hipLaunchKernelGGL(kz_edit_pad, editGrid(scene->nodes.size()), dim3(KZ_EDIT_BLOCK), 0, 0, nodes, (uint32_t)scene->nodes.size(), (const float *)ds->editPad);
        if (!scene->nodes4.empty())
            hipLaunchKernelGGL(kz_edit_quant, editGrid(scene->nodes4.size()), dim3(KZ_EDIT_BLOCK), 0, 0, const_cast<KzNode4 *>(ds->T.nodes4), (uint32_t)scene->nodes4.size(),
                               (const KzNode *)nodes, (const uint32_t *)ds->editSlotSrc);
    }
    HIP_TRY(hipGetLastError());
    for (uint32_t l : lightRows) {
        const KzLightRow &lr = scene->lightRows[l];
        HIP_TRY(hipMemcpy(const_cast<float *>(ds->T.cdf) + lr.cdfOffset, scene->cdf.data() + lr.cdfOffset, (lr.nF + 1) * sizeof(float), hipMemcpyHostToDevice));
    }
    if (!lightRows.empty()) {
        HIP_TRY(hipMemcpy(const_cast<KzLightRow *>(ds->T.lights), scene->lightRows.data(), scene->lightRows.size() * sizeof(KzLightRow), hipMemcpyHostToDevice));
        if (!scene->ilTris.empty()) HIP_TRY(hipMemcpy(const_cast<KzTri *>(ds->T.ilTris), scene->ilTris.data(), scene->ilTris.size() * sizeof(KzTri), hipMemcpyHostToDevice));
    }
    const int rc = beamsUnbuilt(ds); if (rc) return rc;
    HIP_TRY(hipDeviceSynchronize());
    return KZ_OK;
}

int kzEditVertices(KzScene *scene, const KzVertexUpdate *u, uint32_t n, const std::vector<uint32_t> &lightRows) {
    size_t floats = 0;
    for (uint32_t i = 0; i < n; ++i) floats += 3 * (size_t)u[i].nV * (u[i].N ? 2 : 1);
    return forEachReplica(scene, [&](KzDeviceState *ds) -> int {
        int rc;
        if ((rc = stageRoom(ds, floats))) return rc;
        KzTriShade *shade = const_cast<KzTriShade *>(ds->T.shade);
        size_t off = 0;
        for (uint32_t i = 0; i < n; ++i) {
            const KzVertexUpdate &x = u[i];
            const size_t k = 3 * (size_t)x.nV;
            if (!k) continue;
            float *V = ds->editStage + off, *N = x.N ? V + k : nullptr;
            HIP_TRY(hipMemcpy(V, x.V, k * sizeof(float), hipMemcpyHostToDevice));
            if (N) HIP_TRY(hipMemcpy(N, x.N, k * sizeof(float), hipMemcpyHostToDevice));
            off += N ? 2 * k : k;
            if (x.mesh < ds->editBase.size() && ds->editBase[x.mesh]) HIP_TRY(hipMemcpy(ds->editBase[x.mesh], V, (N ? 2 * k : k) * sizeof(float), hipMemcpyDeviceToDevice));
            const KzMeshRow &row = scene->meshRows[x.mesh];
            if (row.nF) hipLaunchKernelGGL(kz_edit_shade, editGrid(row.nF), dim3(KZ_EDIT_BLOCK), 0, 0, shade, (const uint32_t *)ds->editTriVtx, row.triOffset, row.nF, (const float *)V, (const float *)N);
        }
        return refitChain(scene, ds, lightRows);
    });
}

int kzEditReplicaCount(KzScene *scene) {
    KzReplicaSet *rs = replicaSet(scene);
    std::lock_guard<std::mutex> g(rs->m);
    return (int)rs->v.size();
}

int kzEditBsdfRows(KzScene *scene, const uint32_t *rows, uint32_t n, bool extChanged) {
    return forEachReplica(scene, [&](KzDeviceState *ds) -> int {
        for (uint32_t i = 0; i < n; ++i)
            HIP_TRY(hipMemcpy(const_cast<KzBSDF *>(ds->T.bsdfs) + rows[i], &scene->bsdfs[rows[i]], sizeof(KzBSDF), hipMemcpyHostToDevice));
        if (extChanged) { ds->largeMode = -1; ds->probeLaunched = 0; }
        HIP_TRY(hipDeviceSynchronize());
        return KZ_OK;
    });
}

int kzEditLightRows(KzScene *scene) {
    return forEachReplica(scene, [&](KzDeviceState *ds) -> int {
        if (!ds->ilTrisRoomy) {
            void *p = nullptr;
            KZ_ALLOC(&p, 64 * sizeof(KzTri));
            ds->allocs.push_back(p);
            HIP_TRY(hipMemset(p, 0, 64 * sizeof(KzTri)));
            ds->T.ilTris = (const KzTri *)p; ds->ilTrisRoomy = true; ds->editBytes += 64 * sizeof(KzTri);
        }
        if (!scene->lightRows.empty()) HIP_TRY(hipMemcpy(const_cast<KzLightRow *>(ds->T.lights), scene->lightRows.data(), scene->lightRows.size() * sizeof(KzLightRow), hipMemcpyHostToDevice));
        if (!scene->ilTris.empty()) HIP_TRY(hipMemcpy(const_cast<KzTri *>(ds->T.ilTris), scene->ilTris.data(), scene->ilTris.size() * sizeof(KzTri), hipMemcpyHostToDevice));
        HIP_TRY(hipDeviceSynchronize());
        return KZ_OK;
    });
}

static size_t xformFloats(const KzScene *scene, uint32_t mesh) { return 3 * (size_t)scene->meshNV[mesh] * ((scene->meshRows[mesh].flags & 1u) ? 2 : 1); }

int kzEditXformStage(KzScene *scene, const KzXformJob *jobs, uint32_t n, int32_t *bad) {
    *bad = -1;
    size_t floats = 0;
    for (uint32_t i = 0; i < n; ++i) floats += xformFloats(scene, jobs[i].mesh);
    std::vector<uint32_t> flags(n);
    return forEachReplica(scene, [&](KzDeviceState *ds) -> int {
        int rc;
        if ((rc = stageRoom(ds, floats))) return rc;
        if (ds->editBase.size() != scene->meshRows.size()) ds->editBase.assign(scene->meshRows.size(), nullptr);
        if (!ds->editFlag) {
            void *p = nullptr;
            KZ_ALLOC(&p, 4096 * sizeof(uint32_t));
            ds->allocs.push_back(p); ds->editFlag = (uint32_t *)p; ds->editBytes += 4096 * sizeof(uint32_t);
        }
        size_t off = 0;
        for (uint32_t first = 0; first < n; first += 4096) {
            const uint32_t cnt = std::min<uint32_t>(4096, n - first);
            HIP_TRY(hipMemset(ds->editFlag, 0, cnt * sizeof(uint32_t)));
            for (uint32_t j = 0; j < cnt; ++j) {
                const uint32_t m = jobs[first + j].mesh, nV = scene->meshNV[m];
                const size_t k = 3 * (size_t)nV, all = xformFloats(scene, m);
                if (!k) continue;
                if (!ds->editBase[m]) {
                    void *p = nullptr;
                    KZ_ALLOC(&p, all * sizeof(float));
                    ds->allocs.push_back(p); ds->editBytes += all * sizeof(float);
                    HIP_TRY(hipMemcpy(p, scene->baseV[m].data(), k * sizeof(float), hipMemcpyHostToDevice));
                    if (all > k) HIP_TRY(hipMemcpy((float *)p + k, scene->baseN[m].data(), k * sizeof(float), hipMemcpyHostToDevice));
                    ds->editBase[m] = (float *)p;
                }
                const float *bV = ds->editBase[m], *bN = all > k ? bV + k : nullptr;
                float *V = ds->editStage + off, *N = bN ? V + k : nullptr;
                off += all;
                hipLaunchKernelGGL(kz_edit_xform, editGrid(nV), dim3(KZ_EDIT_BLOCK), 0, 0, bV, bN, V, N, nV, *jobs[first + j].x, ds->editFlag + j);
            }
            HIP_TRY(hipGetLastError());
            HIP_TRY(hipMemcpy(flags.data() + first, ds->editFlag, cnt * sizeof(uint32_t), hipMemcpyDeviceToHost));
        }
        for (uint32_t i = 0; i < n; ++i) if (flags[i] && *bad < 0) *bad = (int32_t)i;
        return KZ_OK;
    });
}

int kzEditXformCommit(KzScene *scene, const KzXformJob *jobs, uint32_t n, const std::vector<uint32_t> &lightRows) {
    return forEachReplica(scene, [&](KzDeviceState *ds) -> int {
        KzTriShade *shade = const_cast<KzTriShade *>(ds->T.shade);
        size_t off = 0;
        for (uint32_t i = 0; i < n; ++i) {
            const uint32_t m = jobs[i].mesh;
            const size_t k = 3 * (size_t)scene->meshNV[m], all = xformFloats(scene, m);
            if (!k) continue;
            const float *V = ds->editStage + off, *N = all > k ? V + k : nullptr;
            off += all;
            const KzMeshRow &row = scene->meshRows[m];
            if (row.nF) hipLaunchKernelGGL(kz_edit_shade, editGrid(row.nF), dim3(KZ_EDIT_BLOCK), 0, 0, shade, (const uint32_t *)ds->editTriVtx, row.triOffset, row.nF, V, N);
        }
        return refitChain(scene, ds, lightRows);
    });
}

extern "C" int kz_scene_table(KzScene *scene, int device, int table, void *out, size_t cap, size_t *bytes) {
    if (!scene || !bytes) return kz_fail(KZ_ERR_INVALID_ARG, "kz_scene_table: null argument");
    if (table < KZ_TABLE_NODES || table > KZ_TABLE_BSDFS) return kz_fail(KZ_ERR_INVALID_ARG, "kz_scene_table: table %d (KZ_TABLE_NODES .. KZ_TABLE_BSDFS)", table);
    if (device >= 0 && table == KZ_TABLE_PARAMS) return kz_fail(KZ_ERR_INVALID_ARG, "kz_scene_table: the render constants (KZ_TABLE_PARAMS) are a host table: device must be -1");
    kzHostSync(scene);
    const void *host = nullptr; size_t n = 0;
    switch (table) {
    case KZ_TABLE_NODES: host = scene->nodes.data(); n = scene->nodes.size() * sizeof(KzNode); break;
    case KZ_TABLE_NODES4: host = scene->nodes4.data(); n = scene->nodes4.size() * sizeof(KzNode4); break;
    case KZ_TABLE_TRIS: host = scene->tris.data(); n = scene->tris.size() * sizeof(KzTri); break;
    case KZ_TABLE_SHADE: host = scene->shade.data(); n = scene->shade.size() * sizeof(KzTriShade); break;
    case KZ_TABLE_CDF: host = scene->cdf.data(); n = scene->cdf.size() * sizeof(float); break;
    case KZ_TABLE_LIGHTS: host = scene->lightRows.data(); n = scene->lightRows.size() * sizeof(KzLightRow); break;
    case KZ_TABLE_IL_TRIS: host = scene->ilTris.data(); n = scene->ilTris.size() * sizeof(KzTri); break;
    case KZ_TABLE_BSDFS: host = scene->bsdfs.data(); n = scene->bsdfs.size() * sizeof(KzBSDF); break;
    default: host = &scene->prm; n = sizeof(KzParams); break;
    }
    *bytes = n;
    if (!out || !n) return KZ_OK;
    const size_t copy = std::min(cap, n);
    if (device < 0) { std::memcpy(out, host, copy); return KZ_OK; }
    KzDeviceState *ds; int rc;
    if ((rc = findReplica(scene, device, &ds))) return rc;
    const void *src = nullptr;
    switch (table) {
    case KZ_TABLE_NODES:
        if (!ds->bvh2Resident) return kz_fail(KZ_ERR_STATE, "kz_scene_table: the BVH2 of the replica on device %d is not resident (no BVH2 path or edit has used it)", device);
        src = ds->T.nodes; break;
    case KZ_TABLE_NODES4: src = ds->T.nodes4; break;
    case KZ_TABLE_TRIS: src = ds->T.tris; break;
    case KZ_TABLE_SHADE: src = ds->T.shade; break;
    case KZ_TABLE_CDF: src = ds->T.cdf; break;
    case KZ_TABLE_LIGHTS: src = ds->T.lights; break;
    case KZ_TABLE_BSDFS: src = ds->T.bsdfs; break;
    default: src = ds->T.ilTris; break;
    }
    HIP_TRY(hipDeviceSynchronize());
    HIP_TRY(hipMemcpy(out, src, copy, hipMemcpyDeviceToHost));
    return KZ_OK;
}
```

nano-kazen_amd/csrc/kz_render.hip:

```cpp
#include <hip/hip_runtime.h>

#include "kz_internal.h"
#include "kz_devfn.h"
#include "kz_wavefront.h"
#include "kz_integrators.h"
#include "kz_plan.h"
#include <algorithm>
#include <atomic>
#include <chrono>
#include <cmath>
#include <cstdio>
#include <cstdlib>
#include <cstring>
#include <mutex>
#include <string>
#include <thread>
#include <vector>

template <bool STATS, int EXT>
__global__ __launch_bounds__(KZ_BLOCK) void kz_path_megakernel(KzParams P, KzDevTables T, const uint32_t *__restrict__ pixList,
                                                               uint32_t nItems, uint32_t S, uint32_t sampleBegin, const uint32_t *__restrict__ itemSample,
                                                               float *__restrict__ outJx, float *__restrict__ outJy, float *__restrict__ outR,
                                                               float *__restrict__ outG, float *__restrict__ outB,
                                                               unsigned long long *__restrict__ stats) {
    __shared__ uint32_t s_stack[KZ_STACK_DEPTH * KZ_BLOCK];
    const uint32_t item = blockIdx.x * KZ_BLOCK + threadIdx.x;
    Counters cn = {0, 0, 0, 0, 0, 0};
    if (item < nItems) {
        const uint32_t pl = item / S, so = item - pl * S;
        const uint32_t pxy = pixList[pl];
        const int px = (int)(pxy & 0xffffu), py = (int)(pxy >> 16);
        Sampler smp; smp.type = P.samplerType;
        smp.generateSample(P, T, px, py, itemSample ? itemSample[item] : sampleBegin + so);
        float jx, jy; smp.nextPixel2D(P, T, jx, jy);
        const float sx = (float)px + jx, sy = (float)py + jy;
        float ax, ay; smp.next2D(P, T, ax, ay);
        V3 ro, rd; float mint, maxt;
        cameraRay(P, sx, sy, ax, ay, ro, rd, mint, maxt);
        V3 L = pathLi<STATS, EXT>(P, T, smp, ro, rd, mint, maxt, s_stack + threadIdx.x, cn);
        outJx[item] = jx; outJy[item] = jy; outR[item] = L.x; outG[item] = L.y; outB[item] = L.z;
        if (STATS) {
            bool valid = L.x >= 0 && L.y >= 0 && L.z >= 0 && isfinite(L.x) && isfinite(L.y) && isfinite(L.z);
            if (!valid) cn.dropped++;
        }
    }
    if (STATS) {
        unsigned long long v[7] = {item < nItems ? 1ull : 0ull, cn.rays, cn.nodes, cn.tris, cn.hits, cn.lsamples, cn.dropped};
        for (int k = 0; k < 7; ++k) {
            unsigned long long x = v[k];
            for (int off = 32; off > 0; off >>= 1) x += __shfl_down(x, off, 64);
            if ((threadIdx.x & 63) == 0 && x) atomicAdd(&stats[k], x);
        }
    }
}

#ifdef KZ_EXPERIMENTS
static thread_local int g_failAlloc = 0;
static std::atomic<int> g_failDevice[64];
#endif
hipError_t kzMalloc(void **p, size_t bytes) {
    *p = nullptr;
#ifdef KZ_EXPERIMENTS
    if (g_failAlloc > 0 && --g_failAlloc == 0) return hipErrorOutOfMemory;
#endif
    hipError_t e = hipMalloc(p, bytes);
    if (e == hipErrorOutOfMemory) {
        (void)hipGetLastError();
        int dev = 0;
        if (hipGetDevice(&dev) == hipSuccess && kzCtxPoolTrimPhysical(dev) > 0) e = hipMalloc(p, bytes);
    }
    return e;
}

template <class Tp> static int uploadVec(KzDeviceState *ds, const std::vector<Tp> &v, const Tp **out) {
    *out = nullptr;
    void *p = nullptr;
    const size_t bytes = v.empty() ? 256 : v.size() * sizeof(Tp);
    KZ_ALLOC(&p, bytes);
    ds->allocs.push_back(p);
    if (v.empty()) HIP_TRY(hipMemset(p, 0, bytes));
    else HIP_TRY(hipMemcpy(p, v.data(), bytes, hipMemcpyHostToDevice));
    *out = (const Tp *)p;
    return KZ_OK;
}

static void releaseReplica(KzDeviceState *ds) {
    (void)hipSetDevice(ds->hipDevice);
    (void)hipDeviceSynchronize();
    for (void *p : ds->allocs) (void)hipFree(p);
    for (void *p : {(void *)ds->film, (void *)ds->tapSums, (void *)ds->srgb, (void *)ds->pixList, (void *)ds->stats, (void *)ds->packDev, (void *)ds->rectsDev, (void *)ds->beamEntries, (void *)ds->beamCount, (void *)ds->tileDev, (void *)ds->editStage}) if (p) (void)hipFree(p);
    if (ds->tileHost) (void)hipHostFree(ds->tileHost);
    if (ds->evTiles) (void)hipEventDestroy(ds->evTiles);
    if (ds->evBeam) (void)hipEventDestroy(ds->evBeam);
    if (ds->packHost) (void)hipHostFree(ds->packHost);
    for (PassCtx *&c : ds->ctx) if (c) { kzCtxRelease(ds->device, c); c = nullptr; }
    for (auto &e : ds->events) { (void)hipEventDestroy(e.a); (void)hipEventDestroy(e.b); }
    for (hipStream_t st : ds->passStream) if (st) (void)hipStreamDestroy(st);
    for (hipEvent_t e : ds->evFilm) if (e) (void)hipEventDestroy(e);
    for (hipEvent_t e : {ds->evFork, ds->evCallA, ds->evCallB, ds->evProbe[0][0], ds->evProbe[0][1], ds->evProbe[1][0], ds->evProbe[1][1], ds->evProbe[2][0], ds->evProbe[2][1], ds->evProbe[3][0], ds->evProbe[3][1]}) if (e) (void)hipEventDestroy(e);
    delete ds;
}

void kz_device_init(KzScene *scene) { scene->dev = new KzReplicaSet(); }

void kz_device_release(KzScene *scene) {
    KzReplicaSet *rs = replicaSet(scene);
    if (!rs) return;
    for (KzDeviceState *ds : rs->v) releaseReplica(ds);
    delete rs;
    scene->dev = nullptr;
}

static int resolveTune(const KzTuning &t, KzTune &r) {
    auto pick = [](int a, int d) { return a > 0 ? a : d; };
    r = KzTune{};
    r.refill = pick(t.refill, 0); r.postpone = pick(t.postpone, 24); r.batch = pick(t.batch, 0);
    r.travBlocksPerCU = std::min(8, pick(t.traceBlocksPerCU, KZ_TRACE_WAVES)); r.shadeBlocksPerCU = std::min(16, pick(t.shadeBlocksPerCU, 0));
    r.ldsStack = pick(t.ldsStack, 16);
    r.packet = pick(t.packetPrimary, 0); r.filmGather = pick(t.filmGather, 0);
    if (t.dev0 || t.dev1 > 0 || t.dev2 > 0 || t.dev3 > 1 || t.dev4 > 0 || t.dev5 > 0)
        return kz_fail(KZ_ERR_UNSUPPORTED, "KzTuning.dev0 .. dev5 are reserved: the kernels of rejected experiments they selected (LAB_NOTES 4) have been removed");
    r.ovf = nullptr; r.ovfStride = 0;
    return KZ_OK;
}

int findReplica(const KzScene *scene, int device, KzDeviceState **out) {
    if (!scene) return kz_fail(KZ_ERR_INVALID_ARG, "null scene");
    KzReplicaSet *rs = replicaSet(scene);
    KzDeviceState *ds = nullptr;
    if (rs) {
        std::lock_guard<std::mutex> g(rs->m);
        if (device < 0) ds = rs->v.empty() ? nullptr : rs->v.front();
        else for (KzDeviceState *d : rs->v) if (d->device == device) { ds = d; break; }
    }
    if (!ds) {
        if (device < 0 || !rs || rs->v.empty()) return kz_fail(KZ_ERR_STATE, "scene is not on a device: call kz_scene_upload first");
        return kz_fail(KZ_ERR_STATE, "scene is not resident on device %d: call kz_scene_upload(scene, %d) first", device, device);
    }
    hipError_t e = hipSetDevice(ds->hipDevice);
    if (e != hipSuccess) return kz_fail(KZ_ERR_HIP, "hipSetDevice(%d): %s", ds->hipDevice, hipGetErrorString(e));
#ifdef KZ_EXPERIMENTS
    { const int n = g_failDevice[ds->device & 63].exchange(0); if (n > 0) g_failAlloc = n; }
#endif
    *out = ds;
    return KZ_OK;
}

static int uploadReplica(KzScene *scene, KzDeviceState *ds) {
    int rc;
    KZ_TRACE("upload: start (%.1f MB of tables)", (scene->nodes.size() * sizeof(scene->nodes[0]) + scene->nodes4.size() * sizeof(scene->nodes4[0]) + scene->tris.size() * sizeof(scene->tris[0]) + scene->shade.size() * sizeof(scene->shade[0])) / 1e6);
    {
        struct Job { const void *src; void *dst; size_t bytes; hipError_t err; };
        Job jobs[4] = {};
        auto prep = [&](auto &vec, auto **out, Job &j) -> int {
            using Tp = typename std::remove_reference<decltype(vec)>::type::value_type;
            *out = nullptr;
            void *p = nullptr;
            const size_t bytes = vec.empty() ? 256 : vec.size() * sizeof(Tp);
            KZ_ALLOC(&p, bytes);
            ds->allocs.push_back(p);
            if (vec.empty()) HIP_TRY(hipMemset(p, 0, bytes));
            *out = (const Tp *)p;
            j = Job{vec.empty() ? nullptr : (const void *)vec.data(), p, bytes, hipSuccess};
            return KZ_OK;
        };
        static const std::vector<KzNode> noNodes;
        if ((rc = prep(noNodes, &ds->T.nodes, jobs[0]))) return rc;
        if ((rc = prep(scene->nodes4, &ds->T.nodes4, jobs[1]))) return rc;
        if ((rc = prep(scene->tris, &ds->T.tris, jobs[2]))) return rc;
        if ((rc = prep(scene->shade, &ds->T.shade, jobs[3]))) return rc;
        std::vector<std::thread> th;
        const int dev = ds->hipDevice;
        for (Job &j : jobs) if (j.src && j.bytes >= ((size_t)4 << 20)) th.emplace_back([&j, dev] { j.err = hipSetDevice(dev); if (j.err == hipSuccess) j.err = hipMemcpy(j.dst, j.src, j.bytes, hipMemcpyHostToDevice); });
        for (Job &j : jobs) if (j.src && j.bytes < ((size_t)4 << 20)) j.err = hipMemcpy(j.dst, j.src, j.bytes, hipMemcpyHostToDevice);
        for (std::thread &t : th) t.join();
        for (Job &j : jobs) if (j.err != hipSuccess) return kz_fail(KZ_ERR_HIP, "upload of a scene table (%zu bytes) failed: %s", j.bytes, hipGetErrorString(j.err));
    }
    KZ_TRACE("upload: nodes, nodes4, tris, shade there");
    if ((rc = uploadVec(ds, scene->meshRows, &ds->T.meshes))) return rc;
    if ((rc = uploadVec(ds, scene->bsdfs, &ds->T.bsdfs))) return rc;
    if ((rc = uploadVec(ds, scene->lightRows, &ds->T.lights))) return rc;
    if ((rc = uploadVec(ds, scene->cdf, &ds->T.cdf))) return rc;
    if ((rc = uploadVec(ds, scene->pmj, &ds->T.pmj))) return rc;
    if ((rc = uploadVec(ds, scene->bn, &ds->T.bn))) return rc;
    if ((rc = uploadVec(ds, scene->pixelSamples, &ds->T.pixelSamples))) return rc;
    if ((rc = uploadVec(ds, scene->jump, &ds->T.jump))) return rc;
    std::vector<float> ft(scene->filter, scene->filter + KZ_FILTER_RESOLUTION + 1);
    if ((rc = uploadVec(ds, ft, &ds->T.filter))) return rc;
    if ((rc = uploadVec(ds, scene->ilTris, &ds->T.ilTris))) return rc;
    if ((rc = uploadVec(ds, scene->texProgs, &ds->T.texProgs))) return rc;
    if ((rc = uploadVec(ds, scene->texOps, &ds->T.texOps))) return rc;
    if ((rc = uploadVec(ds, scene->images, &ds->T.images))) return rc;
    if ((rc = uploadVec(ds, scene->texels, &ds->T.texels))) return rc;
    ds->T.texPow2 = scene->texPow2;
    const KzParams &P = scene->prm;
    ds->filmPixels = (size_t)(P.width + 2 * P.border) * (size_t)(P.height + 2 * P.border);
    KZ_TRACE("upload: small tables there");
    KZ_ALLOC(&ds->film, ds->filmPixels * sizeof(float4));
    HIP_TRY(hipMemset(ds->film, 0, ds->filmPixels * sizeof(float4)));
    KZ_ALLOC(&ds->stats, 32 * sizeof(unsigned long long));
    HIP_TRY(hipMemset(ds->stats, 0, 32 * sizeof(unsigned long long)));
    { hipDeviceProp_t prop; HIP_TRY(hipGetDeviceProperties(&prop, ds->hipDevice)); ds->numCU = prop.multiProcessorCount > 0 ? prop.multiProcessorCount : 256; ds->totalMem = prop.totalGlobalMem; }
    KZ_TRACE("upload: film + counters there");
    HIP_TRY(hipDeviceSynchronize());
    KZ_TRACE("upload: done");
    return KZ_OK;
}

int kzEnsureBvh2(KzScene *scene, KzDeviceState *ds) {
    if (ds->bvh2Resident || scene->nodes.empty()) return KZ_OK;
    kzHostSync(scene);
    void *p = nullptr;
    const size_t bytes = scene->nodes.size() * sizeof(KzNode);
    KZ_ALLOC(&p, bytes);
    ds->allocs.push_back(p);
    HIP_TRY(hipMemcpy(p, scene->nodes.data(), bytes, hipMemcpyHostToDevice));
    ds->T.nodes = (const KzNode *)p;
    ds->bvh2Resident = true;
    return KZ_OK;
}

extern "C" {

#ifdef KZ_EXPERIMENTS
void kz_debug_fail_alloc(int nth) { g_failAlloc = nth > 0 ? nth : 0; }
void kz_debug_fail_device(int device, int nth) { g_failDevice[device & 63].store(nth > 0 ? nth : 0); }
#endif

int kz_device_count(void) { return kzLogicalDeviceCount(); }

int kz_device_mem_info(int device, uint64_t *freeBytes, uint64_t *totalBytes) {
    int n = kz_device_count();
    if (device < 0 || device >= n) return kz_fail(n ? KZ_ERR_INVALID_ARG : KZ_ERR_NO_DEVICE, "device %d out of range (%d visible)", device, n);
    HIP_TRY(hipSetDevice(kzPhysicalDevice(device)));
    size_t f = 0, t = 0;
    HIP_TRY(hipMemGetInfo(&f, &t));
    if (freeBytes) *freeBytes = f;
    if (totalBytes) *totalBytes = t;
    return KZ_OK;
}

int kz_scene_upload(KzScene *scene, int device) {
    if (!scene) return kz_fail(KZ_ERR_INVALID_ARG, "null scene");
    const int n = kzLogicalDeviceCount();
    if (n <= 0) return kz_fail(KZ_ERR_NO_DEVICE, "no HIP device visible (the product path has no CPU fallback)");
    if (device < 0 || device >= n) return kz_fail(KZ_ERR_INVALID_ARG, "device %d out of range (%d visible)", device, n);
    KzReplicaSet *rs = replicaSet(scene);
    {
        std::lock_guard<std::mutex> g(rs->m);
        for (KzDeviceState *d : rs->v) if (d->device == device) return KZ_OK;
    }
    KZ_TRACE("kz_scene_upload(%d)", device);
    HIP_TRY(hipSetDevice(kzPhysicalDevice(device)));
    KZ_TRACE("upload: hipSetDevice done");
    kzHostSync(scene);
    KzDeviceState *ds = new KzDeviceState();
    ds->device = device; ds->hipDevice = kzPhysicalDevice(device);
    const int rc = uploadReplica(scene, ds);
    if (rc) { releaseReplica(ds); return rc; }
    std::lock_guard<std::mutex> g(rs->m);
    for (KzDeviceState *d : rs->v) if (d->device == device) { releaseReplica(ds); return KZ_OK; }
    rs->v.push_back(ds);
    return KZ_OK;
}

int kz_scene_evict(KzScene *scene, int device) {
    if (!scene) return kz_fail(KZ_ERR_INVALID_ARG, "null scene");
    KzReplicaSet *rs = replicaSet(scene);
    std::vector<KzDeviceState *> gone;
    {
        std::lock_guard<std::mutex> g(rs->m);
        for (size_t i = 0; i < rs->v.size();) {
            if (device < 0 || rs->v[i]->device == device) { gone.push_back(rs->v[i]); rs->v.erase(rs->v.begin() + i); } else ++i;
        }
    }
    if (gone.empty() && device >= 0) return kz_fail(KZ_ERR_STATE, "scene is not resident on device %d", device);
    for (KzDeviceState *d : gone) releaseReplica(d);
    return KZ_OK;
}

int kz_scene_devices(const KzScene *scene, int32_t *devices, uint32_t cap, uint32_t *count) {
    if (!scene || !count) return kz_fail(KZ_ERR_INVALID_ARG, "null argument");
    KzReplicaSet *rs = replicaSet(scene);
    std::lock_guard<std::mutex> g(rs->m);
    *count = (uint32_t)rs->v.size();
    for (uint32_t i = 0; i < *count && i < cap && devices; ++i) devices[i] = rs->v[i]->device;
    return KZ_OK;
}

}

__global__ __launch_bounds__(256) void kz_tiles_expand(const KzTileDesc *__restrict__ tiles, uint32_t nTiles, uint32_t nPix, int width,
                                                       uint32_t *__restrict__ pixList) {
    const uint32_t i = blockIdx.x * 256u + threadIdx.x;
    if (i >= nPix) return;
    uint32_t lo = 0, hi = nTiles;
    while (hi - lo > 1) { const uint32_t mid = (lo + hi) >> 1; if (tiles[mid].pixOffset <= i) lo = mid; else hi = mid; }
    const KzTileDesc t = tiles[lo];
    const uint32_t local = i - t.pixOffset, w = (uint32_t)t.w, h = (uint32_t)t.h;
    const uint32_t r = local / (8u * w), rem = local - r * 8u * w, hb = min(8u, h - 8u * r);
    const uint32_t c = rem / (8u * hb), rem2 = rem - c * 8u * hb, wb = min(8u, w - 8u * c);
    const uint32_t yl = rem2 / wb, xl = rem2 - yl * wb;
    const uint32_t x = (uint32_t)t.x0 + 8u * c + xl, y = (uint32_t)t.y0 + 8u * r + yl;
    pixList[i] = x | (y << 16);
}

static int prepareTiles(KzScene *scene, KzDeviceState *ds, const KzTile *tiles, uint32_t nTiles, hipStream_t stream) {
    const KzParams &P = scene->prm;
    KzTile whole = {0, 0, P.width, P.height};
    if (!tiles || nTiles == 0) { tiles = &whole; nTiles = 1; }
    bool same = ds->tilesValid && ds->curTiles.size() == nTiles && std::memcmp(ds->curTiles.data(), tiles, nTiles * sizeof(KzTile)) == 0;
    if (same) return KZ_OK;
    std::vector<KzTileDesc> desc(nTiles);
    std::vector<uint32_t> offs(nTiles + 1);
    bool grid = true;
    uint64_t total = 0;
    for (uint32_t t = 0; t < nTiles; ++t) {
        const KzTile &tl = tiles[t];
        if (tl.x0 < 0 || tl.y0 < 0 || tl.w <= 0 || tl.h <= 0 || tl.x0 + tl.w > P.width || tl.y0 + tl.h > P.height)
            return kz_fail(KZ_ERR_INVALID_ARG, "tile %u (%d,%d %dx%d) outside the %dx%d image", t, tl.x0, tl.y0, tl.w, tl.h, P.width, P.height);
        if ((tl.x0 & 7) || (tl.y0 & 7) || ((tl.w & 7) && tl.x0 + tl.w != P.width) || ((tl.h & 7) && tl.y0 + tl.h != P.height)) grid = false;
        desc[t] = KzTileDesc{tl.x0, tl.y0, tl.w, tl.h, (uint32_t)total};
        offs[t] = (uint32_t)total;
        total += (uint64_t)tl.w * (uint64_t)tl.h;
    }
    offs[nTiles] = (uint32_t)total;
    if (total > (uint64_t)P.width * (uint64_t)P.height) return kz_fail(KZ_ERR_INVALID_ARG, "tiles overlap (%llu pixels in a %dx%d image)", (unsigned long long)total, P.width, P.height);
    if (grid) {
        const int gw = (P.width + 7) / 8, gh = (P.height + 7) / 8;
        std::vector<uint8_t> occ((size_t)gw * gh, 0);
        for (uint32_t t = 0; t < nTiles; ++t) {
            const KzTile &tl = tiles[t];
            for (int gy = tl.y0 / 8; gy < (tl.y0 + tl.h + 7) / 8; ++gy)
                for (int gx = tl.x0 / 8; gx < (tl.x0 + tl.w + 7) / 8; ++gx) {
                    uint8_t &o = occ[(size_t)gy * gw + gx];
                    if (o) return kz_fail(KZ_ERR_INVALID_ARG, "tiles overlap at pixel (%d,%d)", gx * 8, gy * 8);
                    o = 1;
                }
        }
    } else {
        for (uint32_t a = 0; a < nTiles; ++a) for (uint32_t b2 = a + 1; b2 < nTiles; ++b2) {
            const KzTile &A = tiles[a], &B = tiles[b2];
            if (A.x0 < B.x0 + B.w && B.x0 < A.x0 + A.w && A.y0 < B.y0 + B.h && B.y0 < A.y0 + A.h)
                return kz_fail(KZ_ERR_INVALID_ARG, "tiles overlap at pixel (%d,%d)", std::max(A.x0, B.x0), std::max(A.y0, B.y0));
        }
    }
    const size_t framePix = (size_t)P.width * P.height;
    if (ds->pixCap < framePix || ds->tileDevCap < nTiles) {
        HIP_TRY(hipDeviceSynchronize());
        if (ds->pixCap < framePix) {
            if (ds->pixList) (void)hipFree(ds->pixList);
            ds->pixList = nullptr; ds->pixCap = 0;
            KZ_ALLOC(&ds->pixList, framePix * sizeof(uint32_t));
            ds->pixCap = framePix;
        }
        if (ds->tileDevCap < nTiles) {
            if (ds->tileDev) (void)hipFree(ds->tileDev);
            ds->tileDev = nullptr; ds->tileDevCap = 0;
            const size_t cap = std::max<size_t>(nTiles, 4096);
            KZ_ALLOC(&ds->tileDev, cap * sizeof(KzTileDesc));
            ds->tileDevCap = cap;
        }
    }
    ds->tilesValid = false;
    if (ds->evCallB) HIP_TRY(hipStreamWaitEvent(stream, ds->evCallB, 0));
    if (ds->tileHostCap < nTiles) {
        if (ds->evTiles) HIP_TRY(hipEventSynchronize(ds->evTiles));
        if (ds->tileHost) (void)hipHostFree(ds->tileHost);
        ds->tileHost = nullptr; ds->tileHostCap = 0;
        const size_t cap = std::max<size_t>(nTiles, 4096);
        HIP_TRY(hipHostMalloc((void **)&ds->tileHost, cap * sizeof(KzTileDesc), hipHostMallocDefault));
        ds->tileHostCap = cap;
    }
    if (!ds->evTiles) HIP_TRY(hipEventCreateWithFlags(&ds->evTiles, hipEventDisableTiming));
    else HIP_TRY(hipEventSynchronize(ds->evTiles));
    std::memcpy(ds->tileHost, desc.data(), nTiles * sizeof(KzTileDesc));
    HIP_TRY(hipMemcpyAsync(ds->tileDev, ds->tileHost, nTiles * sizeof(KzTileDesc), hipMemcpyHostToDevice, stream));
    HIP_TRY(hipEventRecord(ds->evTiles, stream));
    hipLaunchKernelGGL(kz_tiles_expand, dim3((unsigned)((total + 255) / 256)), dim3(256), 0, stream, (const KzTileDesc *)ds->tileDev, nTiles, (uint32_t)total, P.width, ds->pixList);
    HIP_TRY(hipGetLastError());
    ds->nPix = (uint32_t)total;
    ds->curTiles.assign(tiles, tiles + nTiles);
    ds->tilePixOffset = std::move(offs);
    ds->tilesValid = true; ++ds->tileGen;
    return KZ_OK;
}

static int stageMark(PassCtx &c, hipStream_t stream, int kind) {
    if (c.stageUsed == c.stageEv.size()) { hipEvent_t e; HIP_TRY(hipEventCreate(&e)); c.stageEv.push_back(e); c.stageKind.push_back(0); }
    c.stageKind[c.stageUsed] = kind;
    HIP_TRY(hipEventRecord(c.stageEv[c.stageUsed++], stream));
    return KZ_OK;
}

static constexpr size_t KZ_STATE_BYTES_PER_ITEM = 8 * sizeof(float4) + sizeof(uint4) + 3 * sizeof(uint32_t);
static constexpr size_t KZ_SAMPLE_BYTES_PER_ITEM = 5 * sizeof(float);

static int ctxEnsure(PassCtx &c, size_t want, size_t minItems, double graceMs, hipStream_t stream, size_t *usable) {
    if (!c.counts) { KZ_ALLOC(&c.counts, 8 * 520 * sizeof(uint32_t)); }
    KzArena &A = *c.arena;
    if (A.wouldReallocate(want)) HIP_TRY(hipDeviceSynchronize());
#ifdef KZ_EXPERIMENTS
    if (g_failAlloc > 0) { A.failCountdown.store(g_failAlloc); g_failAlloc = 0; }
#endif
    size_t got = 0;
    const int rc = A.request(want, minItems, graceMs, &got);
#ifdef KZ_EXPERIMENTS
    { std::lock_guard<std::mutex> g(A.m); if (!A.busy) g_failAlloc = A.failCountdown.exchange(0); }
#endif
    if (rc) return rc;
    KzWf W{};
    W.rayA.p = A.array<float4>(0); W.rayB.p = A.array<float4>(1); W.hit.p = A.array<float4>(2); W.thr.p = A.array<float4>(3);
    W.misc.p = A.array<float4>(4); W.shA.p = A.array<float4>(5); W.shB.p = A.array<float4>(6); W.shL.p = A.array<float4>(7);
    W.smp = A.array<uint4>(8);
    for (int q = 0; q < 3; ++q) W.queue[q] = A.array<uint32_t>(9 + q);
    W.counts = c.counts;
    c.wf = W;
    for (int k = 0; k < 5; ++k) c.plane[k] = A.array<float>(12 + k);
    *usable = std::min(got, want);
    return KZ_OK;
}

typedef void (*KzTraceFn)(KzParams, KzDevTables, KzWf, const uint32_t *, const uint32_t *, uint32_t, uint32_t *, KzTune, uint32_t *, uint32_t *);
static KzTraceFn traceFn(int mode, bool stats) {
    static const KzTraceFn tab[5][2] = {{kz_wf_trace<0, false>, kz_wf_trace<0, true>}, {kz_wf_trace<1, false>, kz_wf_trace<1, true>},
                                        {kz_wf_trace<2, false>, kz_wf_trace<2, true>}, {nullptr, nullptr}, {kz_wf_trace<4, false>, kz_wf_trace<4, true>}};
    return tab[mode][stats ? 1 : 0];
}
typedef void (*KzListFn)(KzParams, KzDevTables, KzWf, const uint32_t *, uint32_t, uint32_t, const uint2 *, const uint2 *, uint32_t *, uint32_t *, uint32_t *, uint32_t *);
static KzListFn listFn(bool stats, bool fix) {
    static const KzListFn tab[2][2] = {{kz_wf_trace_list<false, false>, kz_wf_trace_list<false, true>}, {kz_wf_trace_list<true, false>, kz_wf_trace_list<true, true>}};
    return tab[stats ? 1 : 0][fix ? 1 : 0];
}
typedef void (*KzPacketFn)(KzParams, KzDevTables, KzWf, const uint32_t *, const uint32_t *, uint32_t, uint32_t *, int, uint32_t *, uint32_t *);
static KzPacketFn packetFn(bool stats, bool fix) {
    static const KzPacketFn tab[2][2] = {{kz_wf_trace_packet<false, false>, kz_wf_trace_packet<false, true>}, {kz_wf_trace_packet<true, false>, kz_wf_trace_packet<true, true>}};
    return tab[stats ? 1 : 0][fix ? 1 : 0];
}

static int ensureBeamBuffers(KzScene *scene, KzDeviceState *ds, hipStream_t stream) {
    const KzParams &P = scene->prm;
    const size_t framePix = (size_t)P.width * P.height;
    if (!ds->evBeam) HIP_TRY(hipEventCreateWithFlags(&ds->evBeam, hipEventDisableTiming));
    if (!ds->beamEntries || !ds->beamCount) {
        if (!ds->beamEntries) KZ_ALLOC(&ds->beamEntries, framePix * KZ_BEAM_CAP * sizeof(uint2));
        if (!ds->beamCount) KZ_ALLOC(&ds->beamCount, framePix * sizeof(uint2));
        ds->beamCap = framePix;
        HIP_TRY(hipMemsetAsync(ds->beamCount, 0xFF, framePix * sizeof(uint2), stream));
        ds->beamDone.clear(); ds->beamDoneGen = ds->tileGen;
    }
    return KZ_OK;
}
static int ensureBeams(KzScene *scene, KzDeviceState *ds, hipStream_t stream, uint32_t p0, uint32_t n) {
    const KzParams &P = scene->prm;
    { const int rc_ = ensureBeamBuffers(scene, ds, stream); if (rc_) return rc_; }
    if (ds->beamDoneGen != ds->tileGen) { ds->beamDone.clear(); ds->beamDoneGen = ds->tileGen; }
    for (const auto &r : ds->beamDone) if (r.first <= p0 && p0 + n <= r.first + r.second) return KZ_OK;
    const int LS = std::max(1, std::min(P.stackBound4, KZ_BEAM_STACK));
    const dim3 gBeam((n + KZ_BLOCK - 1) / KZ_BLOCK);
    const size_t beamLds = (size_t)2 * LS * KZ_BLOCK * sizeof(uint32_t);
    hipLaunchKernelGGL(kz_wf_beam, gBeam, dim3(KZ_BLOCK), beamLds, stream, P, ds->T, (const uint32_t *)(ds->pixList + p0), n, LS, ds->beamEntries, ds->beamCount);
    if (ds->statsOn) hipLaunchKernelGGL(kz_wf_beam_count, gBeam, dim3(KZ_BLOCK), 0, stream, (const uint2 *)ds->beamCount, (const uint32_t *)(ds->pixList + p0), P.width, n, ds->stats + 24);
    HIP_TRY(hipGetLastError());
    HIP_TRY(hipEventRecord(ds->evBeam, stream));
    ++ds->beamSeq;
    ds->beamDone.emplace_back(p0, n);
    return KZ_OK;
}

static int ensureOverflow(KzScene *scene, KzDeviceState *ds, PassCtx &c, const KzTune &tune, hipStream_t stream) {
    const KzParams &P = scene->prm;
    const int stackBound = std::max(P.stackBound4, 2);
    const int ldsStack = std::max(2, std::min(tune.ldsStack, stackBound));
    const size_t stride = (size_t)(ds->numCU * tune.travBlocksPerCU) * KZ_BLOCK, needOvf = stride * (size_t)std::max(1, stackBound - ldsStack) * 3;
    if (needOvf > c.ovfCap) {
        HIP_TRY(hipStreamSynchronize(stream));
        if (c.ovf) (void)hipFree(c.ovf);
        c.ovf = nullptr; c.ovfCap = 0;
        KZ_ALLOC(&c.ovf, needOvf * sizeof(uint32_t));
        c.ovfCap = needOvf;
    }
    return KZ_OK;
}

#ifndef KZ_BESIDE_ITEMS
#define KZ_BESIDE_ITEMS (1u << 27)
#endif
#ifndef KZ_BESIDE_ITEMS_IN_FLIGHT
#define KZ_BESIDE_ITEMS_IN_FLIGHT (1u << 24)
#endif

static int wfPass(KzScene *scene, KzDeviceState *ds, PassCtx &c, hipStream_t stream, const uint32_t *pixList, uint32_t p0, uint32_t nPixPass, uint32_t sBegin, uint32_t Sp, uint32_t items, KzTune tune, bool beams, int shadowBeside) {
    const bool mis = scene->prm.integrator == KZ_INTEGRATOR_PATH_MIS;
    KzParams P = scene->prm;
    if (!mis) { P.anyInvisibleLight = 0; P.nIlTris = 0; P.shadowFast = 1; }
    KzWf W = c.wf;
    W.outJx = c.plane[0]; W.outJy = c.plane[1]; W.outR = c.plane[2]; W.outG = c.plane[3]; W.outB = c.plane[4]; W.stats = ds->stats;
    const bool st = ds->statsOn;
    const dim3 blk(KZ_BLOCK);
    const int shadeBlocks = tune.shadeBlocksPerCU > 0 ? tune.shadeBlocksPerCU : !mis ? 8 : (P.bsdfExt ? 6 : KZ_SHADE_WAVES);
    const dim3 gTrav((unsigned)(ds->numCU * tune.travBlocksPerCU)), gShade((unsigned)(ds->numCU * shadeBlocks));
    const dim3 gPacket((unsigned)(ds->numCU * 8));
    const int stackBound = std::max(P.stackBound4, 2);
    tune.ldsStack = std::max(2, std::min(tune.ldsStack, stackBound));
    const size_t traceLds = (size_t)(tune.ldsStack + 1) * KZ_BLOCK * sizeof(uint32_t);
    {
        const int rc_ = ensureOverflow(scene, ds, c, tune, stream);
        if (rc_) return rc_;
        tune.ovf = c.ovf; tune.ovfStride = (uint32_t)((size_t)gTrav.x * KZ_BLOCK);
    }
    const int maxDepth = P.maxDepth;
    c.stageUsed = 0;
    HIP_TRY(hipMemsetAsync(W.counts, 0, 8 * 520 * sizeof(uint32_t), stream));
    { int rc_ = stageMark(c, stream, -1); if (rc_) return rc_; }
    hipLaunchKernelGGL(kz_wf_generate, dim3((items + KZ_BLOCK - 1) / KZ_BLOCK), blk, 0, stream, P, ds->T, W, pixList, items, Sp, sBegin);
    { int rc_ = stageMark(c, stream, 0); if (rc_) return rc_; }
    if (mis && maxDepth <= 0) return KZ_OK;
    const size_t ovfPart = (size_t)tune.ovfStride * (size_t)std::max(1, stackBound - tune.ldsStack);
    auto trace = [&](int mode, const uint32_t *q, const uint32_t *cptr, uint32_t cimm, uint32_t *head, uint32_t *qb, uint32_t *cb, hipStream_t on = nullptr) {
        KzTune t = tune;
        const bool side = on != nullptr;
        if (side) t.ovf = tune.ovf + 2 * ovfPart; else on = stream;
        if (t.batch <= 0) t.batch = 128;
        if (t.refill <= 0) t.refill = (mode == 2 || mode == 4) ? 32 : 40;
        hipLaunchKernelGGL(traceFn(mode, st), gTrav, blk, traceLds, on, P, ds->T, W, q, cptr, cimm, head, t, qb, cb);
    };
    const bool packet = tune.packet != 1 && P.stackBound4 <= 128, fix = P.anyInvisibleLight != 0;
    if (packet && beams) {
        uint32_t *fbQ = W.queue[0], *fbCount = W.counts + 8 * 520 - 8, *fbHead = fbCount + 1;
        hipLaunchKernelGGL(listFn(st, fix), dim3((items + KZ_BLOCK - 1) / KZ_BLOCK), blk, 0, stream, P, ds->T, W, pixList, items, Sp, (const uint2 *)ds->beamEntries, (const uint2 *)ds->beamCount,
                           fbQ, fbCount, W.queue[2], W.counts + 0);
        hipLaunchKernelGGL(packetFn(st, fix), gPacket, blk, 0, stream, P, ds->T, W, (const uint32_t *)fbQ, (const uint32_t *)fbCount, 0u, fbHead, 8, W.queue[2], W.counts + 0);
    } else if (packet) {
        hipLaunchKernelGGL(packetFn(st, fix), gPacket, blk, 0, stream, P, ds->T, W, (const uint32_t *)nullptr, (const uint32_t *)nullptr, items, W.counts + 2, 8, W.queue[2], W.counts + 0);
    } else {
        trace(0, nullptr, nullptr, items, W.counts + 2, nullptr, nullptr);
        if (fix) hipLaunchKernelGGL(kz_wf_primary_fix, gShade, blk, 0, stream, P, ds->T, W, items, W.queue[2], W.counts + 0);
    }
    if (fix) trace(1, W.queue[2], W.counts + 0, 0u, W.counts + 3, nullptr, nullptr);
    { int rc_ = stageMark(c, stream, 5); if (rc_) return rc_; }
    const uint32_t *cur = nullptr, *curCount = nullptr;
    if (P.integrator == KZ_INTEGRATOR_NORMALS) {
        hipLaunchKernelGGL(kz_wf_normals, gShade, blk, 0, stream, P, ds->T, W, items);
        { int rc_ = stageMark(c, stream, 2); if (rc_) return rc_; }
    } else if (P.integrator == KZ_INTEGRATOR_AO) {
        uint32_t *shQ = W.queue[2], *shCount = W.counts + 5;
        hipLaunchKernelGGL(kz_wf_ao, gShade, blk, 0, stream, P, ds->T, W, pixList, Sp, sBegin, items, shQ, shCount);
        { int rc_ = stageMark(c, stream, 2); if (rc_) return rc_; }
        trace(4, shQ, shCount, 0u, W.counts + 7, nullptr, nullptr);
        { int rc_ = stageMark(c, stream, 3); if (rc_) return rc_; }
    } else if (!mis) {
        const int xsel = P.bsdfExt == 0 ? 0 : (P.bsdfExt == KZ_X_MODELS ? KZ_X_MODELS : KZ_X_MATS);
        for (int iter = 0; iter < maxDepth; ++iter) {
            uint32_t *nextQ = W.queue[iter & 1], *nextCount = W.counts + 4 * (iter + 1);
#define KZ_MATS(EX) hipLaunchKernelGGL((kz_wf_mats<EX>), gShade, blk, 0, stream, P, ds->T, W, pixList, Sp, sBegin, iter, cur, curCount, cur ? 0u : items, nextQ, nextCount)
            if (xsel == KZ_X_MATS) KZ_MATS(KZ_X_MATS); else if (xsel) KZ_MATS(KZ_X_MODELS); else KZ_MATS(0);
#undef KZ_MATS
            { int rc_ = stageMark(c, stream, 2); if (rc_) return rc_; }
            if (iter == maxDepth - 1) break;
            if ((iter & 3) == 3) {
                uint32_t left = 0;
                HIP_TRY(hipMemcpyAsync(&left, nextCount, sizeof left, hipMemcpyDeviceToHost, stream));
                HIP_TRY(hipStreamSynchronize(stream));
                if (left == 0) break;
            }
            trace(0, nextQ, nextCount, 0u, nextCount + 2, nullptr, nullptr);
            { int rc_ = stageMark(c, stream, 1); if (rc_) return rc_; }
            cur = nextQ; curCount = nextCount;
        }
    } else {
        const bool beside = P.nLights > 0 && maxDepth > 1 && (shadowBeside == 2 || (shadowBeside == 0 && items <= KZ_BESIDE_ITEMS));
        ds->lastInfo.shadowBeside = beside ? 1u : 0u;
        if (beside && !c.side) {
            HIP_TRY(hipStreamCreateWithFlags(&c.side, hipStreamNonBlocking));
            HIP_TRY(hipEventCreateWithFlags(&c.evFork, hipEventDisableTiming));
            HIP_TRY(hipEventCreateWithFlags(&c.evJoin, hipEventDisableTiming));
        }
        for (int iter = 0; iter < maxDepth; ++iter) {
            uint32_t *nextQ = W.queue[iter & 1], *nextCount = W.counts + 4 * (iter + 1), *shQ = W.queue[2], *shCount = W.counts + 4 * (iter + 1) + 1;
#define KZ_SHADE(ST, EX) hipLaunchKernelGGL((kz_wf_shade<ST, EX>), gShade, blk, 0, stream, P, ds->T, W, pixList, Sp, sBegin, iter, cur, curCount, items, nextQ, nextCount, shQ, shCount)
            const int xsel = P.bsdfExt == 0 ? 0 : (P.bsdfExt == KZ_X_MODELS ? KZ_X_MODELS : KZ_X_ALL);
            if (st) { if (xsel == KZ_X_ALL) KZ_SHADE(true, KZ_X_ALL); else if (xsel) KZ_SHADE(true, KZ_X_MODELS); else KZ_SHADE(true, 0); }
            else { if (xsel == KZ_X_ALL) KZ_SHADE(false, KZ_X_ALL); else if (xsel) KZ_SHADE(false, KZ_X_MODELS); else KZ_SHADE(false, 0); }
#undef KZ_SHADE
            const bool needExtend = iter < maxDepth - 1 || P.bgPresent;
            { int rc_ = stageMark(c, stream, 2); if (rc_) return rc_; }
            hipStream_t shOn = nullptr;
            if (beside && needExtend) {
                HIP_TRY(hipEventRecord(c.evFork, stream));
                HIP_TRY(hipStreamWaitEvent(c.side, c.evFork, 0));
                shOn = c.side;
            }
            if (P.nLights > 0) {
                if (P.shadowFast) {
                    uint32_t *litQ = W.queue[(iter & 1) ^ 1], *litCount = W.counts + 4 * 520 + 2 * (iter + 1), *litHead = litCount + 1;
                    trace(4, shQ, shCount, 0u, nextCount + 3, litQ, litCount, shOn);
                    if (P.anyInvisibleLight) trace(2, litQ, litCount, 0u, litHead, nullptr, nullptr, shOn);
                } else trace(2, shQ, shCount, 0u, nextCount + 3, nullptr, nullptr, shOn);
            }
            if (shOn) HIP_TRY(hipEventRecord(c.evJoin, c.side));
            { int rc_ = stageMark(c, stream, 3); if (rc_) return rc_; }
            if (needExtend) {
                trace(0, nextQ, nextCount, 0u, nextCount + 2, nullptr, nullptr);
                if (shOn) HIP_TRY(hipStreamWaitEvent(stream, c.evJoin, 0));
                int rc_ = stageMark(c, stream, 1); if (rc_) return rc_;
            }
            cur = nextQ; curCount = nextCount;
        }
        if (P.bgPresent) hipLaunchKernelGGL(kz_wf_final, gShade, blk, 0, stream, P, ds->T, W, cur, curCount);
    }
    if (st) hipLaunchKernelGGL(kz_wf_count, dim3((items + KZ_BLOCK - 1) / KZ_BLOCK), blk, 0, stream, W, items);
    HIP_TRY(hipGetLastError());
    return KZ_OK;
}

static int renderOn(KzScene *scene, KzDeviceState *ds, const KzRenderOpts *opts) {
    int rc;
    const KzParams &P = scene->prm;
    if (opts->pipeline < 0 || opts->pipeline > 2) return kz_fail(KZ_ERR_INVALID_ARG, "pipeline %d (0 = default, 1 = megakernel, 2 = wavefront)", opts->pipeline);
    if (opts->passesInFlight < 0 || opts->passesInFlight > KZ_MAX_PASSES_IN_FLIGHT)
        return kz_fail(KZ_ERR_INVALID_ARG, "passesInFlight %d (0 = default, 1 .. %d)", opts->passesInFlight, KZ_MAX_PASSES_IN_FLIGHT);
    if (opts->shadowBeside < 0 || opts->shadowBeside > 2) return kz_fail(KZ_ERR_INVALID_ARG, "shadowBeside %d (0 = default, 1 = never, 2 = always)", opts->shadowBeside);
    if (opts->passHalves < 0 || opts->passHalves > 2) return kz_fail(KZ_ERR_INVALID_ARG, "passHalves %d (0 = default, 1 = never, 2 = always)", opts->passHalves);
    const int pipeline = opts->pipeline ? opts->pipeline : 2;
    if (pipeline == 1 && (rc = kzEnsureBvh2(scene, ds))) return rc;
    uint32_t s0 = opts->sampleBegin, s1 = opts->sampleEnd;
    if (s0 == 0 && s1 == 0) s1 = P.sampleCount;
    if (s0 >= s1 || s1 > P.sampleCount) return kz_fail(KZ_ERR_INVALID_ARG, "sample range [%u,%u) outside [0,%u)", s0, s1, P.sampleCount);
    hipStream_t stream = (hipStream_t)opts->stream;
    if (ds->evCallB && stream != ds->lastStream) HIP_TRY(hipStreamWaitEvent(stream, ds->evCallB, 0));
    ds->lastStream = stream;
    KzTune tune;
    if ((rc = resolveTune(opts->tune, tune))) return rc;
    if (tune.filmGather != 0 && tune.filmGather != 3) return kz_fail(KZ_ERR_UNSUPPORTED, "KzTuning.filmGather %d: the staged gather kernel of round 1 is gone (round 6: the film is resolved from running tap sums for every filter); 0 = default, 3 = one lane per pixel", tune.filmGather);
    if ((rc = prepareTiles(scene, ds, opts->tiles, opts->nTiles, stream))) return rc;
    { const bool fresh = !ds->tapSums; if ((rc = kzFilmEnsureTapSums(scene, ds, stream))) return rc; if (!opts->accumulate && !fresh) HIP_TRY(hipMemsetAsync(ds->tapSums, 0, ds->tapSumsBytes, stream)); }
    const KzTileDealer *dealer = opts->dealer;
    if (dealer) {
        if (!dealer->counter || (dealer->takenCap && (!dealer->taken || !dealer->nTaken))) return kz_fail(KZ_ERR_INVALID_ARG, "KzTileDealer: null counter / taken buffer");
        if (pipeline != 2) return kz_fail(KZ_ERR_UNSUPPORTED, "dynamic tile dealing needs the wavefront pipeline");
        if (dealer->nTaken) *dealer->nTaken = 0;
    }
    KzPlanIn in;
    in.pipeline = pipeline; in.nPix = ds->nPix; in.s0 = s0; in.s1 = s1;
    in.passItems = opts->passItems; in.passesInFlight = opts->passesInFlight; in.sppPerPass = opts->tune.sppPerPass;
    in.perItem = (pipeline == 2 ? KZ_STATE_BYTES_PER_ITEM : 0) + KZ_SAMPLE_BYTES_PER_ITEM;
    in.limit = opts->maxStateBytes;
    if (!in.limit) {
        size_t freeB = 0, totalB = 0;
        const size_t held = ds->ctxBytes() + kzCtxPoolBytes(ds->device);
        if (hipMemGetInfo(&freeB, &totalB) == hipSuccess && totalB > 0) in.limit = std::min(totalB / 4 * 3, freeB + held - std::min(freeB + held, KzArena::kRuntimeReserve + ((size_t)256 << 20)));
        else in.limit = (size_t)32 << 30;
        if (in.limit == 0) return kz_fail(KZ_ERR_OOM, "the device has %.2f GB free and this replica holds no pass context: nothing is left for path state beyond the %.2f GB a context leaves to the HIP runtime's own allocations",
                                          freeB / 1e9, (KzArena::kRuntimeReserve + ((size_t)256 << 20)) / 1e9);
    }
    const uint32_t nTilesSet = (uint32_t)ds->curTiles.size();
    in.dealer = dealer != nullptr;
    if (dealer) { in.takers = dealer->takers; in.dealerBatchTiles = dealer->batchTiles; in.nTiles = nTilesSet; in.tilePixOffset = ds->tilePixOffset.data(); }
    in.heldBefore = ds->ctx[0] ? std::max(ds->ctx[0]->wanted, ds->ctx[0]->items()) : kzCtxPoolMaxItems(ds->device);
    KzPlan pl;
    { std::string why; if ((rc = kzPlanCall(in, pl, why))) return kz_fail(rc, "%s", why.c_str()); }
    const int nCtx = pl.nCtx;
    const bool multi = pl.multi;
    const size_t need = pl.need, limit = in.limit, perItem = in.perItem;
    const uint32_t batchTiles = pl.batchTiles;
    if (dealer && !kzDealerAgree(dealer, batchTiles, nTilesSet))
        return kz_fail(KZ_ERR_INVALID_ARG, "KzTileDealer: this taker resolved batches of %u tiles of a list of %u, another taker of the same counter resolved something else "
                                           "(all takers must pass the same tile list, sample range, pass options and `takers`)", batchTiles, nTilesSet);
    const bool beams = pipeline == 2 && P.beamOk && tune.packet != 1 && tune.packet != 2 && P.maxDepth > 0;
    {
        const size_t perCtx = need * perItem;
        size_t keep = 0;
        for (int i = 0; i < nCtx; ++i) { PassCtx &c = ds->ctxAt(i); if (c.arena) c.arena->lowerTarget(need); keep += std::max(c.bytes(), perCtx); }
        for (int i = KZ_MAX_PASSES_IN_FLIGHT - 1; i >= nCtx; --i) {
            if (!ds->ctx[i] || !ds->ctx[i]->bytes()) continue;
            if (keep + ds->ctx[i]->bytes() > limit) { HIP_TRY(hipDeviceSynchronize()); ds->ctx[i]->release(); } else keep += ds->ctx[i]->bytes();
        }
        if (keep + kzCtxPoolBytes(ds->device) > limit) (void)kzCtxPoolTrim(ds->device, limit > keep ? limit - keep : 0);
        if (keep > limit)
            for (int i = 0; i < nCtx; ++i) if (ds->ctx[i] && ds->ctx[i]->bytes() > perCtx) {
                HIP_TRY(hipDeviceSynchronize());
                if (need <= KzArena::kSmallMax) ds->ctx[i]->arena->releaseAll(); else ds->ctx[i]->arena->shrinkTo(need);
                ds->ctx[i]->trimAux();
            }
    }
    if (!ds->evCallA) { HIP_TRY(hipEventCreate(&ds->evCallA)); HIP_TRY(hipEventCreate(&ds->evCallB)); }
    if (multi) {
        int prLeast = 0, prGreatest = 0;
        HIP_TRY(hipDeviceGetStreamPriorityRange(&prLeast, &prGreatest));
        const int mode = opts->tune.streamPriority > 0 ? opts->tune.streamPriority : 3;
        if (mode != ds->streamMode) {
            HIP_TRY(hipDeviceSynchronize());
            for (hipStream_t &st : ds->passStream) if (st) { (void)hipStreamDestroy(st); st = nullptr; }
            ds->streamMode = mode;
        }
        const int nPr = std::max(1, prLeast - prGreatest + 1);
        for (int i = 0; i < nCtx; ++i) {
            if (!ds->evFilm[i]) HIP_TRY(hipEventCreateWithFlags(&ds->evFilm[i], hipEventDisableTiming));
            if (ds->passStream[i]) continue;
            const int pr = mode == 1 ? (prLeast + prGreatest) / 2 : mode == 2 ? ((i & 1) ? prGreatest : prLeast) : prLeast - (i % nPr);
            HIP_TRY(hipStreamCreateWithPriority(&ds->passStream[i], hipStreamNonBlocking, pr));
        }
        if (!ds->evFork) HIP_TRY(hipEventCreateWithFlags(&ds->evFork, hipEventDisableTiming));
    }
    if (dealer && !ds->evFilm[0]) HIP_TRY(hipEventCreateWithFlags(&ds->evFilm[0], hipEventDisableTiming));
    ds->eventsUsed = 0;
    HIP_TRY(hipEventRecord(ds->evCallA, stream));
    if (multi) {
        HIP_TRY(hipEventRecord(ds->evFork, stream));
        for (int i = 0; i < nCtx; ++i) HIP_TRY(hipStreamWaitEvent(ds->passStream[i], ds->evFork, 0));
    }
    if (pl.autoShape) for (int i = 0; i < nCtx; ++i) ds->ctxAt(i).wanted = need;
    KZ_TRACE("renderOn: %u pixels x samples [%u, %u), target pass %zu items (%u px x %u spp), limit %.1f GB, %d context(s)", ds->nPix, s0, s1, need, pl.pixPerPass, pl.S, limit / 1e9, nCtx);
    if (beams && (rc = ensureBeamBuffers(scene, ds, stream))) return rc;
    if (pipeline == 2) for (int i = 0; i < nCtx; ++i) if ((rc = ensureOverflow(scene, ds, ds->ctxAt(i), tune, multi ? ds->passStream[i] : stream))) return rc;
    KZ_TRACE("renderOn: beam / overflow buffers there");
    bool inFlight[KZ_MAX_PASSES_IN_FLIGHT] = {};
    uint32_t pass = 0;
    size_t firstPassItems = 0, largestPassItems = 0;
    size_t lastAvail = need;
    auto nextCtx = [&](size_t *usable) -> int {
        const int ci = multi ? (int)(pass % (uint32_t)nCtx) : 0;
        PassCtx &c = ds->ctxAt(ci);
        hipStream_t pst = multi ? ds->passStream[ci] : stream;
        if (pl.grow && !dealer && lastAvail < need && pass >= 2) HIP_TRY(hipEventSynchronize(ds->events[pass - 2].b));
        if (dealer && inFlight[ci]) HIP_TRY(hipEventSynchronize(ds->evFilm[ci]));
        const int rc_ = ctxEnsure(c, need, pl.minStart, pl.graceMs, pst, usable);
        lastAvail = *usable;
        KZ_TRACE("pass %u: context %d holds %zu M items", pass, ci, *usable >> 20);
        return rc_;
    };
    auto onePass = [&](uint32_t p0, uint32_t nPixPass, uint32_t s, uint32_t Sp) -> int {
        const uint32_t *pixList = ds->pixList + p0;
// ... 332 lines not shown
```

nano-kazen_amd/csrc/kz_state.h:

```cpp
#pragma once
#include <hip/hip_runtime.h>
#include "kz_internal.h"

#include <atomic>
#include <chrono>
#include <condition_variable>
#include <mutex>
#include <string>
#include <thread>
#include <vector>

template <class Tp> struct KzField {
    Tp *p;
    __device__ __forceinline__ Tp &operator[](uint32_t i) const { return p[(size_t)i]; }
};
struct KzWf {
    KzField<float4> rayA, rayB;
    KzField<float4> hit;
    KzField<float4> thr;
    KzField<float4> misc;
    uint4 *smp;
    KzField<float4> shA, shB, shL;
    uint32_t *queue[3];
    uint32_t *counts;
    float *outJx, *outJy, *outR, *outG, *outB;
    unsigned long long *stats;
};

struct KzTune { int refill, postpone, batch, travBlocksPerCU, shadeBlocksPerCU, ldsStack, packet, filmGather;
                uint32_t *ovf; uint32_t ovfStride; };


#ifndef KZ_BEAM_CAP
#define KZ_BEAM_CAP 32
#endif

struct KzTileRect { int32_t x0, y0, w, h; uint32_t offset; };
struct KzTileDesc { int32_t x0, y0, w, h; uint32_t pixOffset; };

#define HIP_TRY(expr) do { hipError_t e_ = (expr); if (e_ != hipSuccess) return kz_fail(KZ_ERR_HIP, "%s failed: %s", #expr, hipGetErrorString(e_)); } while (0)

hipError_t kzMalloc(void **p, size_t bytes);
#define KZ_ALLOC(pp, bytes) do { hipError_t e_ = kzMalloc((void **)(pp), (bytes)); if (e_ != hipSuccess) \
    return kz_fail(e_ == hipErrorOutOfMemory ? KZ_ERR_OOM : KZ_ERR_HIP, "device allocation of %zu bytes failed: %s", (size_t)(bytes), hipGetErrorString(e_)); } while (0)
struct DevMem {
    void *p = nullptr;
    DevMem() = default;
    DevMem(const DevMem &) = delete; DevMem &operator=(const DevMem &) = delete;
    ~DevMem() { if (p) (void)hipFree(p); }
    template <class Tp> Tp *as() const { return (Tp *)p; }
};

#ifdef KZ_EXPERIMENTS
extern std::atomic<int> g_kzTrace;
void kzTraceLine(const char *fmt, ...);
#define KZ_TRACE(...) do { if (g_kzTrace.load(std::memory_order_relaxed)) kzTraceLine(__VA_ARGS__); } while (0)
int kzPhysicalDevice(int logical);
#else
#define KZ_TRACE(...) do { } while (0)
static inline int kzPhysicalDevice(int logical) { return logical; }
#endif
int kzLogicalDeviceCount();

struct EventPair { hipEvent_t a, b; };
struct KzArena {
    static constexpr int kArrays = 17;
    size_t levelItems = (size_t)1 << 23;
    static constexpr size_t kSmallMax = (size_t)1 << 23;
    static constexpr size_t kRuntimeReserve = (size_t)2 << 30;
    int device;
    size_t capItems = 0;
    size_t smallItems = 0;
    char *base[kArrays]; size_t elem[kArrays];
    struct Level { size_t firstItem, items; hipMemGenericAllocationHandle_t h[kArrays]; int mappedArrays; };
    std::vector<Level> levels;
    std::atomic<size_t> mapped{0};
    std::mutex m; std::condition_variable cvProgress; std::thread th;
    bool stop = false, busy = false, growthFailed = false; size_t target = 0;
    std::atomic<int> failCountdown{0};
    bool injectedFailure() {
#ifdef KZ_EXPERIMENTS
        int fc = failCountdown.load();
        return fc > 0 && failCountdown.compare_exchange_strong(fc, fc - 1) && fc == 1;
#else
        return false;
#endif
    }
    int err = 0; std::string errMsg;
    std::chrono::steady_clock::time_point lastProgress;
    explicit KzArena(int dev);
    ~KzArena();
    KzArena(const KzArena &) = delete; KzArena &operator=(const KzArena &) = delete;
    static size_t bytesPerItem();
    size_t bytes() const { return mapped.load() * bytesPerItem(); }
    bool wouldReallocate(size_t items) const;
    int request(size_t items, size_t minItems, double graceMs, size_t *got);
    void shrinkTo(size_t items);
    void lowerTarget(size_t items);
    void releaseAll();
    template <class Tp> Tp *array(int a) const { return (Tp *)base[a]; }
private:
    int reserve(size_t cap, size_t firstTarget); int requestSmall(size_t items, size_t *got); void freeSmall();
    void growLoop(); bool growOneLevel(size_t first); void dropLevels(size_t keepLevels); void stopThread();
};
struct PassCtx {
    KzArena *arena = nullptr;
    KzWf wf{};
    float *plane[5] = {};
    uint32_t *counts = nullptr;
    uint32_t *ovf = nullptr; size_t ovfCap = 0;
    hipStream_t side = nullptr; hipEvent_t evFork = nullptr, evJoin = nullptr;
    PassCtx *view[2] = {nullptr, nullptr}; hipStream_t halfStream = nullptr; hipEvent_t evHalfFork = nullptr, evHalfJoin = nullptr;
    size_t wanted = 0;
    uint64_t beamSeen = 0;
    std::vector<hipEvent_t> stageEv; std::vector<int> stageKind; size_t stageUsed = 0;
    size_t items() const { return arena ? arena->mapped.load() : 0; }
    size_t bytes() const { return (arena ? arena->bytes() : 0) + ovfCap * sizeof(uint32_t) + (view[0] ? view[0]->bytes() : 0) + (view[1] ? view[1]->bytes() : 0); }
    void release() {
        if (arena) arena->shrinkTo(0);
        wf = KzWf{}; for (float *&q : plane) q = nullptr; wanted = 0;
        if (ovf) (void)hipFree(ovf); ovf = nullptr; ovfCap = 0;
        for (PassCtx *v : view) if (v) v->release();
    }
    void trimAux() {
        if (ovf) { (void)hipFree(ovf); ovf = nullptr; ovfCap = 0; }
        for (PassCtx *v : view) if (v) v->trimAux();
    }
    void destroy() {
        release();
        for (PassCtx *&v : view) if (v) { v->destroy(); delete v; v = nullptr; }
        if (halfStream) { (void)hipStreamDestroy(halfStream); halfStream = nullptr; }
        if (evHalfFork) { (void)hipEventDestroy(evHalfFork); evHalfFork = nullptr; }
        if (evHalfJoin) { (void)hipEventDestroy(evHalfJoin); evHalfJoin = nullptr; }
        if (counts) (void)hipFree(counts); counts = nullptr;
        delete arena; arena = nullptr;
        for (auto &e : stageEv) (void)hipEventDestroy(e);
        stageEv.clear(); stageKind.clear();
        if (side) { (void)hipStreamDestroy(side); side = nullptr; }
        if (evFork) { (void)hipEventDestroy(evFork); evFork = nullptr; }
        if (evJoin) { (void)hipEventDestroy(evJoin); evJoin = nullptr; }
    }
};
PassCtx *kzCtxAcquire(int device);
void kzCtxRelease(int device, PassCtx *c);
size_t kzCtxPoolBytes(int device);
size_t kzCtxPoolMaxItems(int device);
size_t kzCtxPoolTrim(int device, size_t keepBytes);
size_t kzCtxPoolTrimPhysical(int hipDevice);
struct KzDeviceState {
    int device = -1;
    int hipDevice = -1;
    KzDevTables T{};
    std::vector<void *> allocs;
    bool bvh2Resident = false;
    float4 *film = nullptr; size_t filmPixels = 0;
    float4 *tapSums = nullptr; size_t tapSumsBytes = 0;
    uint8_t *srgb = nullptr;
    float4 *packDev = nullptr; size_t packCap = 0; KzTileRect *rectsDev = nullptr; size_t rectsCap = 0;
    float4 *packHost = nullptr; size_t packHostCap = 0;
    uint32_t *pixList = nullptr; size_t pixCap = 0; uint32_t nPix = 0;
    KzTileDesc *tileDev = nullptr; size_t tileDevCap = 0; KzTileDesc *tileHost = nullptr; size_t tileHostCap = 0; hipEvent_t evTiles = nullptr;
    std::vector<KzTile> curTiles; std::vector<uint32_t> tilePixOffset;
    bool tilesValid = false; uint64_t tileGen = 0;
    unsigned long long *stats = nullptr; bool statsOn = false;
    hipStream_t lastStream = nullptr;
    int numCU = 256; size_t totalMem = 0;
    PassCtx *ctx[KZ_MAX_PASSES_IN_FLIGHT] = {};
    PassCtx &ctxAt(int i) { if (!ctx[i]) ctx[i] = kzCtxAcquire(device); return *ctx[i]; }
    std::vector<EventPair> events; size_t eventsUsed = 0;
    hipStream_t passStream[KZ_MAX_PASSES_IN_FLIGHT] = {}; hipEvent_t evFork = nullptr, evFilm[KZ_MAX_PASSES_IN_FLIGHT] = {}, evCallA = nullptr, evCallB = nullptr;
    hipEvent_t evProbe[4][2] = {}; size_t probeItems[4] = {}; int probeLaunched = 0; int largeMode = -1; float probeMs[4] = {};
    int lastCtx = 0; bool lastDual = false; int streamMode = 0;
    PassCtx *lastStageCtx = nullptr;
    uint2 *beamEntries = nullptr, *beamCount = nullptr; size_t beamCap = 0; hipEvent_t evBeam = nullptr; uint64_t beamSeq = 0;
    std::vector<std::pair<uint32_t, uint32_t>> beamDone; uint64_t beamDoneGen = 0;
    size_t beamBytes() const { return beamCap * (KZ_BEAM_CAP + 1) * sizeof(uint2); }
    size_t ctxBytes() const { size_t b = 0; for (const PassCtx *c : ctx) if (c) b += c->bytes(); return b; }
    KzPassInfo lastInfo{}; std::string growNote;
    uint32_t *editTriVtx = nullptr, *editSlotSrc = nullptr; float *editPad = nullptr; float *editStage = nullptr; size_t editStageCap = 0; size_t editBytes = 0;
    std::vector<float *> editBase; uint32_t *editFlag = nullptr; bool ilTrisRoomy = false;
};
struct KzReplicaSet { std::mutex m; std::vector<KzDeviceState *> v; };

static inline KzReplicaSet *replicaSet(const KzScene *scene) { return (KzReplicaSet *)scene->dev; }
int findReplica(const KzScene *scene, int device, KzDeviceState **out);
int kzEnsureBvh2(KzScene *scene, KzDeviceState *ds);
static inline int requireDevice(KzScene *scene, KzDeviceState **out) { return findReplica(scene, -1, out); }
size_t packedFloats(const KzParams &P, const KzTile *tiles, uint32_t nTiles);
int checkTiles(const KzParams &P, const KzTile *tiles, uint32_t nTiles);
int downloadTiles(KzScene *scene, KzDeviceState *ds, const KzTile *tiles, uint32_t nTiles, float *packed, size_t nFloats, hipStream_t stream);
#define KZ_FILM_GRID 64
int kzFilmEnsureTapSums(KzScene *scene, KzDeviceState *ds, hipStream_t stream);
int kzFilmClear(KzDeviceState *ds, hipStream_t stream);
int kzFilmStage(KzScene *scene, KzDeviceState *ds, PassCtx &c, hipStream_t pst, const uint32_t *pixList, uint32_t nPixPass, uint32_t Sp, hipEvent_t waitFilm, int lanesPerPixel);
int kzFilmResolve(KzScene *scene, KzDeviceState *ds, hipStream_t stream);
```

nano-kazen_amd/csrc/kz_wavefront.h:

```cpp
#pragma once
#include "kz_state.h"
#include "kz_devfn.h"

#ifndef KZ_WF_QCAP
#define KZ_WF_QCAP 960
#endif
#define KZ_WF_ROUNDS (KZ_WF_QCAP / KZ_BLOCK)

struct WfAppender {
    uint32_t *s_buf; uint32_t *s_n; uint32_t *s_gb; uint32_t *gQueue; uint32_t *gCount;
    __device__ __forceinline__ void push(bool pred, uint32_t val) {
        const unsigned long long m = __ballot(pred);
        const int lane = threadIdx.x & 63;
        uint32_t base = 0;
        if (lane == 0 && m) base = atomicAdd(s_n, (uint32_t)__popcll(m));
        base = __shfl(base, 0, 64);
        if (pred) s_buf[base + __popcll(m & ((1ull << lane) - 1ull))] = val;
    }
    __device__ __forceinline__ void maybeFlush(bool force) {
        __syncthreads();
        const uint32_t n = *s_n;
        if (force ? (n > 0) : (n > KZ_WF_QCAP - KZ_BLOCK)) {
            if (threadIdx.x == 0) *s_gb = atomicAdd(gCount, n);
            __syncthreads();
            const uint32_t gb = *s_gb;
            for (uint32_t i = threadIdx.x; i < n; i += KZ_BLOCK) gQueue[gb + i] = s_buf[i];
            __syncthreads();
            if (threadIdx.x == 0) *s_n = 0;
        }
        __syncthreads();
    }
};

__device__ __forceinline__ void wfStatsFlush(unsigned long long *stats, const Counters &cn, uint32_t samples) {
    unsigned long long v[7] = {samples, cn.rays, cn.nodes, cn.tris, cn.hits, cn.lsamples, cn.dropped};
    for (int k = 0; k < 7; ++k) {
        unsigned long long x = v[k];
        for (int off = 32; off > 0; off >>= 1) x += __shfl_down(x, off, 64);
        if ((threadIdx.x & 63) == 0 && x) atomicAdd(&stats[k], x);
    }
}

__device__ __forceinline__ uint32_t wfPmjDim(const KzParams &P, int iter) {
    return 4u + (uint32_t)iter * (4u + (P.nLights > 0 ? 3u : 0u)) + (iter > 3 ? (uint32_t)(iter - 3) : 0u);
}
__device__ __forceinline__ void wfLoadSampler(const KzParams &P, const KzWf &W, uint32_t slot, int px, int py, uint32_t sampleIndex, Sampler &s, uint32_t dimPmj) {
    s.type = P.samplerType; s.px = px; s.py = py; s.idx = sampleIndex;
    if (P.samplerType == KZ_SAMPLER_PMJ02BN) {
        s.state = 0ull; s.inc = 0ull; s.dim = dimPmj; s.hp = hashPixelBlock(px, py);
        return;
    }
    const uint4 v = W.smp[slot];
    s.state = (uint64_t)v.x | ((uint64_t)v.y << 32);
    s.dim = (uint32_t)__builtin_amdgcn_readfirstlane((int)v.z);
    s.inc = (P.samplerType == KZ_SAMPLER_PMJ02BN) ? 0ull : ((hashPixelSeed(px, py, P.seed) << 1u) | 1u);
    s.hp = (P.samplerType != KZ_SAMPLER_INDEPENDENT) ? hashPixelBlock(px, py) : 0ull;
}
__device__ __forceinline__ void wfStoreSampler(const KzParams &P, const KzWf &W, uint32_t slot, const Sampler &s) {
    uint4 v;
    if (P.samplerType == KZ_SAMPLER_PMJ02BN) return;
    v.x = (uint32_t)s.state; v.y = (uint32_t)(s.state >> 32); v.z = s.dim; v.w = 0;
    W.smp[slot] = v;
}

__global__ __launch_bounds__(KZ_BLOCK) void kz_wf_generate(KzParams P, KzDevTables T, KzWf W, const uint32_t *__restrict__ pixList,
                                                           uint32_t nItems, uint32_t S, uint32_t sampleBegin) {
    const uint32_t item = blockIdx.x * KZ_BLOCK + threadIdx.x;
    if (item >= nItems) return;
    uint32_t pl, pxy;
    if ((S & 63u) == 0) { pl = (uint32_t)__builtin_amdgcn_readfirstlane((int)item) / S; pxy = (uint32_t)__builtin_amdgcn_readfirstlane((int)pixList[pl]); }
    else { pl = item / S; pxy = pixList[pl]; }
    const uint32_t so = item - pl * S;
    const int px = (int)(pxy & 0xffffu), py = (int)(pxy >> 16);
    Sampler smp; smp.type = P.samplerType;
    smp.generateSample(P, T, px, py, sampleBegin + so);
    float jx, jy; smp.nextPixel2D(P, T, jx, jy);
    const float sx = (float)px + jx, sy = (float)py + jy;
    float ax, ay; smp.next2D(P, T, ax, ay);
    V3 ro, rd; float mint, maxt;
    cameraRay(P, sx, sy, ax, ay, ro, rd, mint, maxt);
    kzStoreStream(&W.rayA[item], make_float4(ro.x, ro.y, ro.z, mint));
    kzStoreStream(&W.rayB[item], make_float4(rd.x, rd.y, rd.z, maxt));
    wfStoreSampler(P, W, item, smp);
    W.outJx[item] = jx; W.outJy[item] = jy; W.outR[item] = 0.f; W.outG[item] = 0.f; W.outB[item] = 0.f;
}


__global__ __launch_bounds__(KZ_BLOCK) void kz_wf_primary_fix(KzParams P, KzDevTables T, KzWf W, uint32_t nItems, uint32_t *__restrict__ outQueue,
                                                              uint32_t *__restrict__ outCount) {
    __shared__ uint32_t s_buf[KZ_WF_QCAP]; __shared__ uint32_t s_n, s_gb;
    if (threadIdx.x == 0) s_n = 0;
    __syncthreads();
    WfAppender ap = {s_buf, &s_n, &s_gb, outQueue, outCount};
    for (uint32_t base = blockIdx.x * KZ_BLOCK; base < nItems; base += gridDim.x * KZ_BLOCK) {
        const uint32_t slot = base + threadIdx.x;
        bool need = false;
        if (slot < nItems) {
            const float4 h = kzLoadStream(&W.hit[slot]);
            if (h.x < KZ_INF) {
                RawHit rh; rh.t = h.x; rh.u = h.y; rh.v = h.z; rh.tri = 0; rh.gid = __float_as_uint(h.w);
                const int li = lightOfGid(T, rh.gid);
                if (li >= 0 && !T.lights[li].primaryVisibility) {
                    Its its; postIntersect<false>(T, rh, its);
                    const float4 b = kzLoadStream(&W.rayB[slot]);
                    const V3 rd = mk(b.x, b.y, b.z);
                    const V3 no = its.p + P.traceBias * rd;
                    kzStoreStream(&W.shA[slot], make_float4(no.x, no.y, no.z, KZ_INF));
                    kzStoreStream(&W.shB[slot], make_float4(rd.x, rd.y, rd.z, KZ_EPSILON));
                    need = true;
                }
            }
        }
        ap.push(need, slot);
        ap.maybeFlush(false);
    }
    ap.maybeFlush(true);
}

#ifndef KZ_SHADE_WAVES
#define KZ_SHADE_WAVES 4
#endif
struct KzSst {
#ifdef KZ_SHADESTAT
    unsigned long long t = __builtin_amdgcn_s_memtime(), acc[14] = {0, 0, 0, 0, 0, 0, 0, 0, 0, 0, 0, 0, 0, 0};
    __device__ __forceinline__ void mark(int k) { const unsigned long long t_ = __builtin_amdgcn_s_memtime(); acc[k] += t_ - t; t = t_; }
    __device__ __forceinline__ void markw(int k) { __builtin_amdgcn_s_waitcnt(0); mark(k); }
    __device__ __forceinline__ void flush(unsigned long long *stats) { if ((threadIdx.x & 63) == 0) for (int k = 0; k < 14; ++k) atomicAdd(stats + 8 + k, acc[k]); }
#else
    __device__ __forceinline__ void mark(int) {}
    __device__ __forceinline__ void markw(int) {}
    __device__ __forceinline__ void flush(unsigned long long *) {}
#endif
};

template <bool STATS, int EXT>
__device__ __forceinline__ bool wfClassify(const KzParams &P, const KzDevTables &T, const KzWf &W, const uint32_t *__restrict__ pixList, uint32_t S, uint32_t sampleBegin,
                                           int iter, bool compact, uint32_t slot, Its &its, uint32_t &modelKey, Counters &cn, KzSst &sst) {
    bool survivor = false;
    const float4 h = kzLoadStream(&W.hit[slot]);
    const float4 rb = kzLoadStream(&W.rayB[slot]);
    const V3 rd = mk(rb.x, rb.y, rb.z);
#ifdef KZ_SHADESTAT
    sst.markw(10);
    if (h.x < KZ_INF) { const float4 *sp_ = reinterpret_cast<const float4 *>(T.shade + __float_as_uint(h.w)); const float4 a_ = sp_[0], b_ = sp_[6]; asm volatile("" :: "v"(a_.x), "v"(b_.x)); }
    sst.markw(11);
#endif
    if (!(h.x < KZ_INF)) {
        if (iter > 0 && P.bgPresent) {
            const float4 th = kzLoadStream(&W.thr[slot]);
            const V3 c = mk(th.x, th.y, th.z) * backgroundRadiance(P, T, rd);
            unsafeAtomicAdd(W.outR + slot, c.x); unsafeAtomicAdd(W.outG + slot, c.y); unsafeAtomicAdd(W.outB + slot, c.z);
        }
        return false;
    }
    RawHit rh; rh.t = h.x; rh.u = h.y; rh.v = h.z; rh.tri = 0; rh.gid = __float_as_uint(h.w);
    postIntersect<false>(T, rh, its); if (STATS) cn.hits++;
    sst.markw(12);
    if (its.light >= 0) {
        const KzLightRow &lr = T.lights[its.light];
        const float4 ra = kzLoadStream(&W.rayA[slot]);
        const float4 th = iter == 0 ? make_float4(1.f, 1.f, 1.f, 1.f) : kzLoadStream(&W.thr[slot]);
        const float4 mi = iter == 0 ? make_float4(0.f, 0.f, 0.f, 0.f) : (compact ? make_float4(th.w, 0.f, 0.f, 0.f) : kzLoadStream(&W.misc[slot]));
        const V3 ro = mk(ra.x, ra.y, ra.z);
        const V3 wi = normalized(its.p - ro);
        float bsdfWeight = 1.f;
        if (iter > 0 && mi.z == 0.f) bsdfWeight = powerHeuristic(mi.x, lightPdfSolidAngle(lr.normalization, its.sh.n, wi, its.p, ro));
        if (dot(its.sh.n, -wi) > 0.f) {
            const V3 c = (bsdfWeight * mk(th.x, th.y, th.z)) * mk(lr.radiance[0], lr.radiance[1], lr.radiance[2]);
            unsafeAtomicAdd(W.outR + slot, c.x); unsafeAtomicAdd(W.outG + slot, c.y); unsafeAtomicAdd(W.outB + slot, c.z);
        }
        return false;
    }
    const float wz = dot(-rd, its.sh.n);
    bool twoSided = false;
    if (EXT) {
        const int bt = T.bsdfs[its.bsdf].type;
        twoSided = bt == KZ_BSDF_DIELECTRIC || bt == KZ_BSDF_ROUGHDIELECTRIC || bt == KZ_BSDF_NORMALMAP;
        modelKey = (uint32_t)bt;
        if ((EXT & KZ_X_NMAP) && bt == KZ_BSDF_NORMALMAP) modelKey = 8u + ((uint32_t)T.bsdfs[T.bsdfs[its.bsdf].nested].type & 7u);
    }
    survivor = (wz > 0.f) || twoSided || isnan(wz);
    if (survivor && iter >= 3) {
        const uint32_t pl = slot / S; const uint32_t pxy = pixList[pl];
        Sampler smp; wfLoadSampler(P, W, slot, (int)(pxy & 0xffffu), (int)(pxy >> 16), sampleBegin + (slot - pl * S), smp, wfPmjDim(P, iter));
        const float4 th = kzLoadStream(&W.thr[slot]);
        V3 throughput = mk(th.x, th.y, th.z);
        const float etaA = compact ? 1.f : th.w;
        const float probability = fminf(maxCoeff(throughput) * etaA * etaA, 0.95f);
        if (probability <= smp.next1D(P, T)) survivor = false;
        else {
            throughput = throughput / probability;
            kzStoreStream(&W.thr[slot], make_float4(throughput.x, throughput.y, throughput.z, th.w));
            wfStoreSampler(P, W, slot, smp);
        }
    } else if (STATS && !survivor && P.nLights > 0) {
        bool alive = true;
        if (iter >= 3) {
            const uint32_t pl = slot / S; const uint32_t pxy = pixList[pl];
            Sampler smp; wfLoadSampler(P, W, slot, (int)(pxy & 0xffffu), (int)(pxy >> 16), sampleBegin + (slot - pl * S), smp, wfPmjDim(P, iter));
            const float4 th = kzLoadStream(&W.thr[slot]);
            const float etaA = compact ? 1.f : th.w;
            if (fminf(maxCoeff(mk(th.x, th.y, th.z)) * etaA * etaA, 0.95f) <= smp.next1D(P, T)) alive = false;
        }
        if (alive) cn.lsamples++;
    }
    return survivor;
}

template <bool STATS, int EXT>
__device__ __forceinline__ void wfShadeSurvivor(const KzParams &P, const KzDevTables &T, const KzWf &W, const uint32_t *__restrict__ pixList, uint32_t S, uint32_t sampleBegin,
                                                int iter, bool compact, uint32_t slot, const Its &its, bool &pushNext, bool &pushShadow, Counters &cn, KzSst &sst) {
    const float eps = P.traceBias;
    const float4 rb = kzLoadStream(&W.rayB[slot]);
    const V3 rd = mk(rb.x, rb.y, rb.z);
    float4 th = iter == 0 ? make_float4(1.f, 1.f, 1.f, 1.f) : kzLoadStream(&W.thr[slot]);
    V3 throughput = mk(th.x, th.y, th.z);
    const float eta = compact ? 1.f : th.w;
    float accRough = (iter == 0 || compact) ? 0.f : W.misc[slot].y;
    const uint32_t pl = slot / S;
    const uint32_t pxy = pixList[pl];
    Sampler smp; wfLoadSampler(P, W, slot, (int)(pxy & 0xffffu), (int)(pxy >> 16), sampleBegin + (slot - pl * S), smp, wfPmjDim(P, iter) + (iter >= 3 ? 1u : 0u));
    KzBSDF bsdf = T.bsdfs[its.bsdf];
    NMap nm; surfaceSetup<EXT>(T, its, bsdf, nm);
    const V3 wiLocal = toLocal(its.sh, -rd);
    sst.mark(2);
    const float pick = smp.next1D(P, T);
    if (P.nLights > 0) {
        const uint32_t li = min((uint32_t)floorf((float)P.nLights * pick), P.nLights - 1);
        const KzLightRow lrow = T.lights[li];
        if (STATS) cn.lsamples++;
        const LightSample ls = lightSample(T, lrow, its.p, [&]() { return smp.next1D(P, T); });
        const V3 lwi = ls.wi; const float dist = ls.dist, lpdf = ls.pdf;
        V3 Ls = ls.Ls;
        Ls = lightPickDivide(P, Ls);
        sst.mark(3);
        const V3 woL = toLocal(its.sh, lwi);
        V3 f; float bpdfL;
        surfEvalPdf<EXT>(bsdf, nm, its, wiLocal, woL, accRough, f, bpdfL);
        const V3 pend = throughput * Ls * f * powerHeuristic(lpdf, bpdfL);
        if (!(pend.x == 0.f && pend.y == 0.f && pend.z == 0.f)) {
            kzStoreStream(&W.shA[slot], make_float4(its.p.x, its.p.y, its.p.z, dist - eps));
            kzStoreStream(&W.shB[slot], make_float4(lwi.x, lwi.y, lwi.z, eps));
            kzStoreStream(&W.shL[slot], make_float4(pend.x, pend.y, pend.z, 0.f));
            pushShadow = true;
        }
    }
    sst.mark(4);
    if (P.regularization && bsdf.type == KZ_BSDF_KAZENSTANDARD) accRough += bsdf.roughness * P.accumulatedRoughness;
    float s2x, s2y; smp.next2D(P, T, s2x, s2y);
    const float s1 = smp.next1D(P, T);
    sst.mark(5);
    V3 woLocal; bool ok, discrete, solid; float etaScale, pdfS;
    const V3 weight = surfSample<EXT>(bsdf, nm, its, wiLocal, accRough, s1, s2x, s2y, woLocal, ok, discrete, etaScale, pdfS, solid);
    sst.mark(6);
    throughput = throughput * weight;
    const float etaNext = eta * etaScale;
    if (ok && !(weight.x == 0.f && weight.y == 0.f && weight.z == 0.f)) {
        const float bpdf = pdfS >= 0.f ? pdfS : surfPdf<EXT>(bsdf, nm, its, wiLocal, woLocal, accRough, solid);
        const V3 nd = toWorld(its.sh, woLocal);
        if (iter + 1 < P.maxDepth || P.bgPresent) {
            kzStoreStream(&W.rayA[slot], make_float4(its.p.x, its.p.y, its.p.z, eps));
            kzStoreStream(&W.rayB[slot], make_float4(nd.x, nd.y, nd.z, KZ_INF));
            kzStoreStream(&W.thr[slot], make_float4(throughput.x, throughput.y, throughput.z, compact ? bpdf : etaNext));
            if (!compact) kzStoreStream(&W.misc[slot], make_float4(bpdf, accRough, discrete ? 1.f : 0.f, 0.f));
            wfStoreSampler(P, W, slot, smp);
            pushNext = true;
        }
    }
}

struct WfQueuePair {
    uint32_t *s_bufN, *s_bufS, *s_nN, *s_nS, *s_gbN, *s_gbS;
    uint32_t *nextQueue, *nextCount, *shadowQueue, *shadowCount;
    uint32_t cap = KZ_WF_QCAP;
    __device__ __forceinline__ void flush(bool force) {
        const uint32_t nN = *s_nN, nS = *s_nS;
        const bool fN = force ? (nN > 0) : (nN > cap - KZ_BLOCK), fS = force ? (nS > 0) : (nS > cap - KZ_BLOCK);
        if (fN || fS) {
            if (threadIdx.x == 0) { if (fN) *s_gbN = atomicAdd(nextCount, nN); if (fS) *s_gbS = atomicAdd(shadowCount, nS); }
            __syncthreads();
            if (fN) { const uint32_t gb = *s_gbN; for (uint32_t i = threadIdx.x; i < nN; i += KZ_BLOCK) nextQueue[gb + i] = s_bufN[i]; }
            if (fS) { const uint32_t gb = *s_gbS; for (uint32_t i = threadIdx.x; i < nS; i += KZ_BLOCK) shadowQueue[gb + i] = s_bufS[i]; }
            __syncthreads();
            if (threadIdx.x == 0) { if (fN) *s_nN = 0; if (fS) *s_nS = 0; }
        }
    }
    __device__ __forceinline__ void flushAll() {
        const uint32_t nN = *s_nN, nS = *s_nS;
        if (threadIdx.x == 0) { if (nN) *s_gbN = atomicAdd(nextCount, nN); if (nS) *s_gbS = atomicAdd(shadowCount, nS); }
        __syncthreads();
        { const uint32_t gb = *s_gbN; for (uint32_t i = threadIdx.x; i < nN; i += KZ_BLOCK) nextQueue[gb + i] = s_bufN[i]; }
        { const uint32_t gb = *s_gbS; for (uint32_t i = threadIdx.x; i < nS; i += KZ_BLOCK) shadowQueue[gb + i] = s_bufS[i]; }
        __syncthreads();
        if (threadIdx.x == 0) { *s_nN = 0; *s_nS = 0; }
        __syncthreads();
    }
};

#define KZ_SV_CAP (2 * KZ_BLOCK)
template <bool STATS, int EXT>
__global__ __launch_bounds__(KZ_BLOCK, ((EXT & (KZ_X_TEX | KZ_X_NMAP)) ? 3 : KZ_SHADE_WAVES)) void kz_wf_shade(KzParams P, KzDevTables T, KzWf W, const uint32_t *__restrict__ pixList, uint32_t S,
                                                        uint32_t sampleBegin, int iter, const uint32_t *__restrict__ queue,
                                                        const uint32_t *__restrict__ countPtr, uint32_t countImm,
                                                        uint32_t *__restrict__ nextQueue, uint32_t *__restrict__ nextCount,
                                                        uint32_t *__restrict__ shadowQueue, uint32_t *__restrict__ shadowCount) {
    constexpr bool NMAPX = (EXT & KZ_X_NMAP) != 0;
    constexpr int SVW = NMAPX ? 19 : 16;
    constexpr uint32_t QCAP = (uint32_t)KZ_WF_QCAP;
    __shared__ uint32_t s_bufN[QCAP], s_bufS[QCAP]; __shared__ uint32_t s_nN, s_nS, s_gbN, s_gbS;
    constexpr bool SORT = NMAPX;
    __shared__ uint32_t s_hist[SORT ? 16 : 1]; __shared__ uint16_t s_perm[SORT ? KZ_BLOCK : 1];
    __shared__ uint32_t s_sv[SVW * KZ_SV_CAP]; __shared__ uint32_t s_svCnt[2];
    if (threadIdx.x == 0) { s_nN = 0; s_nS = 0; s_svCnt[0] = 0; s_svCnt[1] = 0; }
    if (SORT && threadIdx.x < 16) s_hist[threadIdx.x] = 0;
    __syncthreads();
    WfAppender apN = {s_bufN, &s_nN, &s_gbN, nextQueue, nextCount}, apS = {s_bufS, &s_nS, &s_gbS, shadowQueue, shadowCount};
    WfQueuePair qp = {s_bufN, s_bufS, &s_nN, &s_nS, &s_gbN, &s_gbS, nextQueue, nextCount, shadowQueue, shadowCount, QCAP};
    const uint32_t count = countPtr ? *countPtr : countImm;
    const int lane = threadIdx.x & 63;
    const bool compact = !EXT && !P.regularization;
    Counters cn = {0, 0, 0, 0, 0, 0};
    KzSst sst;
    uint32_t round = 0;
    for (uint32_t base = blockIdx.x * KZ_BLOCK;; base += gridDim.x * KZ_BLOCK, ++round) {
        const bool more = base < count;
        sst.mark(9);
        bool survivor = false;
        uint32_t slot = 0;
        Its its;
        uint32_t modelKey = 0;
        if (more && base + threadIdx.x < count) {
            const uint32_t qi = base + threadIdx.x;
            slot = queue ? queue[qi] : qi;
            survivor = wfClassify<STATS, EXT>(P, T, W, pixList, S, sampleBegin, iter, compact, slot, its, modelKey, cn, sst);
        }
        sst.mark(0);
        {
            const unsigned long long m = __ballot(survivor);
            uint32_t b = 0;
            if (lane == 0 && m) b = atomicAdd(&s_svCnt[round & 1u], (uint32_t)__popcll(m));
            b = __shfl(b, 0, 64);
            if (survivor) {
                const uint32_t e = b + __builtin_amdgcn_mbcnt_hi((uint32_t)(m >> 32), __builtin_amdgcn_mbcnt_lo((uint32_t)m, 0u));
                uint32_t *r = s_sv + e;
                r[0] = slot; r[KZ_SV_CAP] = __float_as_uint(its.p.x); r[2 * KZ_SV_CAP] = __float_as_uint(its.p.y); r[3 * KZ_SV_CAP] = __float_as_uint(its.p.z);
                r[4 * KZ_SV_CAP] = __float_as_uint(its.sh.s.x); r[5 * KZ_SV_CAP] = __float_as_uint(its.sh.s.y); r[6 * KZ_SV_CAP] = __float_as_uint(its.sh.s.z);
                r[7 * KZ_SV_CAP] = __float_as_uint(its.sh.t.x); r[8 * KZ_SV_CAP] = __float_as_uint(its.sh.t.y); r[9 * KZ_SV_CAP] = __float_as_uint(its.sh.t.z);
                r[10 * KZ_SV_CAP] = __float_as_uint(its.sh.n.x); r[11 * KZ_SV_CAP] = __float_as_uint(its.sh.n.y); r[12 * KZ_SV_CAP] = __float_as_uint(its.sh.n.z);
                r[13 * KZ_SV_CAP] = __float_as_uint(its.uvx); r[14 * KZ_SV_CAP] = __float_as_uint(its.uvy); r[15 * KZ_SV_CAP] = EXT ? (its.bsdf | (modelKey << 24)) : its.bsdf;
                if (NMAPX) { r[16 * KZ_SV_CAP] = __float_as_uint(its.dpdu.x); r[17 * KZ_SV_CAP] = __float_as_uint(its.dpdu.y); r[18 * KZ_SV_CAP] = __float_as_uint(its.dpdu.z); }
            }
        }
        __syncthreads();
        sst.mark(1);
        const uint32_t n0 = s_svCnt[round & 1u];
        bool pushNext = false, pushShadow = false;
        const uint32_t take = n0 >= KZ_BLOCK ? (uint32_t)KZ_BLOCK : (more ? 0u : n0);
        if (threadIdx.x == 0) s_svCnt[(round + 1u) & 1u] = n0 - take;
        uint32_t mine = threadIdx.x;
        if (SORT && take > 64u) {
            uint32_t key = 0, rank = 0;
            if (threadIdx.x < take) { key = s_sv[15 * KZ_SV_CAP + (n0 - take) + threadIdx.x] >> 24; rank = atomicAdd(&s_hist[key & 15u], 1u); }
            __syncthreads();
            if (threadIdx.x < take) {
                uint32_t basePos = 0;
                for (uint32_t k = 0; k < (key & 15u); ++k) basePos += s_hist[k];
                s_perm[basePos + rank] = (uint16_t)threadIdx.x;
            }
            __syncthreads();
            if (threadIdx.x < take) mine = s_perm[threadIdx.x];
        }
        if (threadIdx.x < take) {
            const uint32_t *r = s_sv + (n0 - take) + mine;
            slot = r[0];
            its.p = mk(__uint_as_float(r[KZ_SV_CAP]), __uint_as_float(r[2 * KZ_SV_CAP]), __uint_as_float(r[3 * KZ_SV_CAP]));
            its.sh.s = mk(__uint_as_float(r[4 * KZ_SV_CAP]), __uint_as_float(r[5 * KZ_SV_CAP]), __uint_as_float(r[6 * KZ_SV_CAP]));
            its.sh.t = mk(__uint_as_float(r[7 * KZ_SV_CAP]), __uint_as_float(r[8 * KZ_SV_CAP]), __uint_as_float(r[9 * KZ_SV_CAP]));
            its.sh.n = mk(__uint_as_float(r[10 * KZ_SV_CAP]), __uint_as_float(r[11 * KZ_SV_CAP]), __uint_as_float(r[12 * KZ_SV_CAP]));
            its.uvx = __uint_as_float(r[13 * KZ_SV_CAP]); its.uvy = __uint_as_float(r[14 * KZ_SV_CAP]); its.bsdf = EXT ? (r[15 * KZ_SV_CAP] & 0xFFFFFFu) : r[15 * KZ_SV_CAP];
            if (NMAPX) its.dpdu = mk(__uint_as_float(r[16 * KZ_SV_CAP]), __uint_as_float(r[17 * KZ_SV_CAP]), __uint_as_float(r[18 * KZ_SV_CAP]));
            wfShadeSurvivor<STATS, EXT>(P, T, W, pixList, S, sampleBegin, iter, compact, slot, its, pushNext, pushShadow, cn, sst);
        }
        sst.mark(7);
        apN.push(pushNext, slot); apS.push(pushShadow, slot);
        __syncthreads();
        if (SORT && threadIdx.x < 16) s_hist[threadIdx.x] = 0;
        qp.flush(false);
        sst.mark(8);
        if (!more && n0 - take == 0) break;
        if (!more) base -= gridDim.x * KZ_BLOCK;
    }
    __syncthreads();
    qp.flush(true);
    if (STATS) wfStatsFlush(W.stats, cn, 0);
    sst.flush(W.stats);
}



#ifndef KZ_TRACE_WAVES
#define KZ_TRACE_WAVES 8
#endif
template <int MODE, bool STATS>
__global__ __launch_bounds__(KZ_BLOCK) __attribute__((amdgpu_waves_per_eu(STATS ? KZ_TRACE_WAVES - 1 : KZ_TRACE_WAVES, STATS ? KZ_TRACE_WAVES - 1 : KZ_TRACE_WAVES)))
void kz_wf_trace(KzParams P, KzDevTables T, KzWf W, const uint32_t *__restrict__ queue,
                                                        const uint32_t *__restrict__ countPtr, uint32_t countImm, uint32_t *__restrict__ head, KzTune tune,
                                                        uint32_t *__restrict__ queueB, uint32_t *__restrict__ countPtrB) {
    extern __shared__ uint32_t s_stack[];
    const uint32_t count = countPtr ? *countPtr : countImm;
    [[maybe_unused]] constexpr bool SHADOW = MODE == 2 || MODE == 4;
    constexpr int kind = MODE == 4 ? 2 : MODE;
    const int lane = threadIdx.x & 63;
    constexpr uint32_t rowB = KZ_BLOCK * 4u;
    const uint32_t stkBase = kzLdsAddr(s_stack + threadIdx.x), ldsRows = (uint32_t)tune.ldsStack * rowB;
    uint32_t top = stkBase;
    uint32_t *const ovfBase = tune.ovf;
    const uint32_t ovfLane = blockIdx.x * KZ_BLOCK + threadIdx.x;
    const size_t ovfStride = tune.ovfStride;
#define ovf(row) ovfBase[(size_t)(row) * ovfStride + ovfLane]
    auto push = [&](uint32_t v) {
// ... 516 lines not shown
```

Measured before the change: 1843.

## Apply Russian roulette ahead of tracing unless the ray can reach an emitter

At depth 3 and beyond, the shade stage now peeks at the next roulette draw. A path that would be killed is not pushed to the next wavefront, unless its ray could hit one of a small set of emitter triangles, tested with a bounding box and then a wave-cooperative triangle test. This is meant to avoid tracing extension rays and re-classifying paths that roulette would end anyway, with emission hits still counted. The change also returns early when no next ray is needed, skipping BSDF sampling. It adds an emitter-triangle table and upload path, and only applies to MIS scenes with no background and at most 64 emitter triangles.

```diff
diff --git a/include/kazen_mi355x_dev.h b/include/kazen_mi355x_dev.h
--- a/include/kazen_mi355x_dev.h
+++ b/include/kazen_mi355x_dev.h
@@ -73,6 +73,7 @@
 void kz_debug_grow_delay(int ms);
 void kz_debug_trace(int on);
 void kz_debug_alias_devices(int n);
+void kz_debug_rr_ahead(int on);
 
 typedef struct KzPlanQuery {
     int32_t pipeline;
@@ -101,7 +102,8 @@
 int kz_kat_pow4(int32_t spp, int32_t *out4);
 
 enum { KZ_TABLE_NODES = 0, KZ_TABLE_NODES4 = 1, KZ_TABLE_TRIS = 2, KZ_TABLE_SHADE = 3, KZ_TABLE_CDF = 4, KZ_TABLE_LIGHTS = 5, KZ_TABLE_IL_TRIS = 6, KZ_TABLE_PARAMS = 7,
-       KZ_TABLE_BSDFS = 8  };
+       KZ_TABLE_BSDFS = 8 ,
+       KZ_TABLE_EM_TRIS = 9  };
 int kz_scene_table(KzScene *scene, int device, int table, void *out, size_t cap, size_t *bytes);
 
 #define KZ_BUILD_EXPERIMENTS 1
diff --git a/nano-kazen_amd/abi.py b/nano-kazen_amd/abi.py
--- a/nano-kazen_amd/abi.py
+++ b/nano-kazen_amd/abi.py
@@ -186,8 +186,8 @@
            "kz_tiles_packed_floats", "kz_film_download_tiles", "kz_film_merge_tiles", "kz_film_merge_rects", "kz_device_trim", "kz_kat_dpdf", "kz_kat_pow4", "kz_last_grow_note",
            "kz_plan_passes", "kz_plan_schedule", "kz_pass_mode_info", "kz_scene_table"]
 EDIT_EXPORTS = ["kz_scene_set_camera", "kz_scene_set_vertices", "kz_scene_set_bsdfs", "kz_scene_set_lights", "kz_scene_set_transforms"]
-KZ_TABLE_NODES, KZ_TABLE_NODES4, KZ_TABLE_TRIS, KZ_TABLE_SHADE, KZ_TABLE_CDF, KZ_TABLE_LIGHTS, KZ_TABLE_IL_TRIS, KZ_TABLE_PARAMS, KZ_TABLE_BSDFS = range(9)
-DEV_ONLY_EXPORTS = ["kz_debug_fail_alloc", "kz_debug_fail_device", "kz_debug_grow_delay", "kz_debug_trace", "kz_debug_alias_devices"]
+KZ_TABLE_NODES, KZ_TABLE_NODES4, KZ_TABLE_TRIS, KZ_TABLE_SHADE, KZ_TABLE_CDF, KZ_TABLE_LIGHTS, KZ_TABLE_IL_TRIS, KZ_TABLE_PARAMS, KZ_TABLE_BSDFS, KZ_TABLE_EM_TRIS = range(10)
+DEV_ONLY_EXPORTS = ["kz_debug_fail_alloc", "kz_debug_fail_device", "kz_debug_grow_delay", "kz_debug_trace", "kz_debug_alias_devices", "kz_debug_rr_ahead"]
 
 _HERE = os.path.dirname(os.path.abspath(__file__))
 LIB_PATH = os.environ.get("KZ_LIB_PATH") or os.path.join(_HERE, "csrc", "libkazen_mi355x.so")
diff --git a/nano-kazen_amd/csrc/kz_debug.hip b/nano-kazen_amd/csrc/kz_debug.hip
--- a/nano-kazen_amd/csrc/kz_debug.hip
+++ b/nano-kazen_amd/csrc/kz_debug.hip
@@ -307,3 +307,8 @@
 
 
 }
+
+#ifdef KZ_EXPERIMENTS
+std::atomic<int> g_kzRrAhead{1};
+extern "C" void kz_debug_rr_ahead(int on) { g_kzRrAhead.store(on == 2 ? 2 : on ? 1 : 0); }
+#endif
diff --git a/nano-kazen_amd/csrc/kz_host.cpp b/nano-kazen_amd/csrc/kz_host.cpp
--- a/nano-kazen_amd/csrc/kz_host.cpp
+++ b/nano-kazen_amd/csrc/kz_host.cpp
@@ -195,6 +195,36 @@
         float m = std::max(std::fabs(p.ilLo[a]), std::fabs(p.ilHi[a]));
         if (std::isfinite(m)) { float e = m * 4e-7f + 1e-30f; p.ilLo[a] -= e; p.ilHi[a] += e; }
     }
+    kzEmitterTris(sc);
+}
+
+void kzEmitterTris(KzScene *sc) {
+    const KzParams &p = sc->prm;
+    sc->emTris.clear();
+    for (int a = 0; a < 3; ++a) { sc->emLo[a] = INFINITY; sc->emHi[a] = -INFINITY; }
+    size_t total = 0;
+    for (const KzLightRow &lr : sc->lightRows) total += lr.nF;
+    const bool on = total <= KZ_EM_MAX && !p.bgPresent && p.integrator == KZ_INTEGRATOR_PATH_MIS;
+    if (on) for (const KzLightRow &lr : sc->lightRows)
+        for (uint32_t f = 0; f < lr.nF; ++f) {
+            const KzTriShade &s = sc->shade[lr.triOffset + f];
+            KzTri t; std::memset(&t, 0, sizeof t);
+            for (int a = 0; a < 3; ++a) {
+                t.p0[a] = s.p[a]; t.e1[a] = s.p[3 + a] - s.p[a]; t.e2[a] = s.p[6 + a] - s.p[a];
+                for (int v = 0; v < 3; ++v) { sc->emLo[a] = std::min(sc->emLo[a], s.p[3 * v + a]); sc->emHi[a] = std::max(sc->emHi[a], s.p[3 * v + a]); }
+            }
+            t.mesh = lr.mesh; t.prim = f; t.gid = lr.triOffset + f;
+            sc->emTris.push_back(t);
+        }
+    sc->nEmTris = on ? (uint32_t)sc->emTris.size() : KZ_EM_OFF;
+    for (int a = 0; a < 3; ++a) {
+        float m = std::max(std::fabs(sc->emLo[a]), std::fabs(sc->emHi[a]));
+        if (std::isfinite(m)) { float e = m * 4e-7f + 1e-30f; sc->emLo[a] -= e; sc->emHi[a] += e; }
+    }
+    KzTri h; std::memset(&h, 0, sizeof h);
+    for (int a = 0; a < 3; ++a) { h.p0[a] = sc->emLo[a]; h.e1[a] = sc->emHi[a]; }
+    h.mesh = sc->nEmTris;
+    sc->emTris.push_back(h);
 }
 
 int kzCheckBsdfs(const char *who, const KzBSDF *rows, uint32_t n, uint32_t nTextures, int32_t integ) {
@@ -451,6 +481,7 @@
         }
         for (int a = 0; a < 3; ++a) p.bgRadiance[a] = d->background.present ? d->background.intensity * col[a] : 0.f;
     }
+    kzEmitterTris(sc);
     p.samplerType = d->sampler.type;
     p.seed = d->sampler.seed;
     p.sampleCount = d->sampler.sampleCount;
diff --git a/nano-kazen_amd/csrc/kz_internal.h b/nano-kazen_amd/csrc/kz_internal.h
--- a/nano-kazen_amd/csrc/kz_internal.h
+++ b/nano-kazen_amd/csrc/kz_internal.h
@@ -11,6 +11,8 @@
 #define KZ_MAX_LEAF 4
 #define KZ_MAX_FILTER_TAPS 9
 #define KZ_PATH_MATS_MAX_DEPTH 512
+#define KZ_EM_MAX 64
+#define KZ_EM_OFF 0xFFFFFFFFu
 
 struct KzNode { float q[12]; uint32_t child[2]; uint32_t pad[2]; };
 static_assert(sizeof(KzNode) == 64, "node packet must be 64 B");
@@ -104,6 +106,9 @@
     const KzImageRow *images;
     const uint8_t *texels;
     uint32_t texPow2;
+    uint32_t nEmTris = KZ_EM_OFF;
+    const KzTri *emTris;
+    float emLo[3], emHi[3];
 };
 
 struct KzXform {
@@ -126,6 +131,7 @@
     std::vector<float> pixelSamples;
     std::vector<KzPcgJump> jump;
     std::vector<KzTri> ilTris;
+    std::vector<KzTri> emTris; uint32_t nEmTris = KZ_EM_OFF; float emLo[3] = {0, 0, 0}, emHi[3] = {0, 0, 0};
     std::vector<KzTexProg> texProgs;
     std::vector<KzTexOp> texOps;
     std::vector<KzImageRow> images;
@@ -160,6 +166,7 @@
 int kzCameraParams(const KzCamera &c, KzParams &p);
 void kzLightCdf(const KzTriShade *shade, uint32_t nF, std::vector<float> &t, float &normalization);
 void kzInvisibleLights(KzScene *sc);
+void kzEmitterTris(KzScene *sc);
 int kzCheckBsdfs(const char *who, const KzBSDF *rows, uint32_t n, uint32_t nTextures, int32_t integrator);
 void kzResolveBsdf(KzBSDF &b);
 int32_t kzBsdfExt(const std::vector<KzBSDF> &rows);
diff --git a/nano-kazen_amd/csrc/kz_refit.hip b/nano-kazen_amd/csrc/kz_refit.hip
--- a/nano-kazen_amd/csrc/kz_refit.hip
+++ b/nano-kazen_amd/csrc/kz_refit.hip
@@ -170,6 +170,7 @@
     if (!lightRows.empty()) {
         HIP_TRY(hipMemcpy(const_cast<KzLightRow *>(ds->T.lights), scene->lightRows.data(), scene->lightRows.size() * sizeof(KzLightRow), hipMemcpyHostToDevice));
         if (!scene->ilTris.empty()) HIP_TRY(hipMemcpy(const_cast<KzTri *>(ds->T.ilTris), scene->ilTris.data(), scene->ilTris.size() * sizeof(KzTri), hipMemcpyHostToDevice));
+        const int erc = kzEmitterUpload(scene, ds); if (erc) return erc;
     }
     const int rc = beamsUnbuilt(ds); if (rc) return rc;
     HIP_TRY(hipDeviceSynchronize());
@@ -227,6 +228,7 @@
         }
         if (!scene->lightRows.empty()) HIP_TRY(hipMemcpy(const_cast<KzLightRow *>(ds->T.lights), scene->lightRows.data(), scene->lightRows.size() * sizeof(KzLightRow), hipMemcpyHostToDevice));
         if (!scene->ilTris.empty()) HIP_TRY(hipMemcpy(const_cast<KzTri *>(ds->T.ilTris), scene->ilTris.data(), scene->ilTris.size() * sizeof(KzTri), hipMemcpyHostToDevice));
+        { const int erc = kzEmitterUpload(scene, ds); if (erc) return erc; }
         HIP_TRY(hipDeviceSynchronize());
         return KZ_OK;
     });
@@ -296,7 +298,7 @@
 
 extern "C" int kz_scene_table(KzScene *scene, int device, int table, void *out, size_t cap, size_t *bytes) {
     if (!scene || !bytes) return kz_fail(KZ_ERR_INVALID_ARG, "kz_scene_table: null argument");
-    if (table < KZ_TABLE_NODES || table > KZ_TABLE_BSDFS) return kz_fail(KZ_ERR_INVALID_ARG, "kz_scene_table: table %d (KZ_TABLE_NODES .. KZ_TABLE_BSDFS)", table);
+    if (table < KZ_TABLE_NODES || table > KZ_TABLE_EM_TRIS) return kz_fail(KZ_ERR_INVALID_ARG, "kz_scene_table: table %d (KZ_TABLE_NODES .. KZ_TABLE_EM_TRIS)", table);
     if (device >= 0 && table == KZ_TABLE_PARAMS) return kz_fail(KZ_ERR_INVALID_ARG, "kz_scene_table: the render constants (KZ_TABLE_PARAMS) are a host table: device must be -1");
     kzHostSync(scene);
     const void *host = nullptr; size_t n = 0;
@@ -309,6 +311,7 @@
     case KZ_TABLE_LIGHTS: host = scene->lightRows.data(); n = scene->lightRows.size() * sizeof(KzLightRow); break;
     case KZ_TABLE_IL_TRIS: host = scene->ilTris.data(); n = scene->ilTris.size() * sizeof(KzTri); break;
     case KZ_TABLE_BSDFS: host = scene->bsdfs.data(); n = scene->bsdfs.size() * sizeof(KzBSDF); break;
+    case KZ_TABLE_EM_TRIS: host = scene->emTris.data(); n = scene->emTris.size() * sizeof(KzTri); break;
     default: host = &scene->prm; n = sizeof(KzParams); break;
     }
     *bytes = n;
@@ -328,6 +331,7 @@
     case KZ_TABLE_CDF: src = ds->T.cdf; break;
     case KZ_TABLE_LIGHTS: src = ds->T.lights; break;
     case KZ_TABLE_BSDFS: src = ds->T.bsdfs; break;
+    case KZ_TABLE_EM_TRIS: src = ds->T.emTris; break;
     default: src = ds->T.ilTris; break;
     }
     HIP_TRY(hipDeviceSynchronize());
diff --git a/nano-kazen_amd/csrc/kz_render.hip b/nano-kazen_amd/csrc/kz_render.hip
--- a/nano-kazen_amd/csrc/kz_render.hip
+++ b/nano-kazen_amd/csrc/kz_render.hip
@@ -81,6 +81,21 @@
     if (v.empty()) HIP_TRY(hipMemset(p, 0, bytes));
     else HIP_TRY(hipMemcpy(p, v.data(), bytes, hipMemcpyHostToDevice));
     *out = (const Tp *)p;
+    return KZ_OK;
+}
+
+int kzEmitterUpload(KzScene *scene, KzDeviceState *ds) {
+    if (!ds->T.emTris) {
+        void *p = nullptr;
+        KZ_ALLOC(&p, (KZ_EM_MAX + 1) * sizeof(KzTri));
+        ds->allocs.push_back(p);
+        HIP_TRY(hipMemset(p, 0, (KZ_EM_MAX + 1) * sizeof(KzTri)));
+        ds->T.emTris = (const KzTri *)p;
+    }
+    if (!scene->emTris.empty() && scene->emTris.size() <= KZ_EM_MAX + 1)
+        HIP_TRY(hipMemcpy(const_cast<KzTri *>(ds->T.emTris), scene->emTris.data(), scene->emTris.size() * sizeof(KzTri), hipMemcpyHostToDevice));
+    ds->T.nEmTris = scene->nEmTris;
+    for (int a = 0; a < 3; ++a) { ds->T.emLo[a] = scene->emLo[a]; ds->T.emHi[a] = scene->emHi[a]; }
     return KZ_OK;
 }
 
@@ -188,6 +203,7 @@
     std::vector<float> ft(scene->filter, scene->filter + KZ_FILTER_RESOLUTION + 1);
     if ((rc = uploadVec(ds, ft, &ds->T.filter))) return rc;
     if ((rc = uploadVec(ds, scene->ilTris, &ds->T.ilTris))) return rc;
+    if ((rc = kzEmitterUpload(scene, ds))) return rc;
     if ((rc = uploadVec(ds, scene->texProgs, &ds->T.texProgs))) return rc;
     if ((rc = uploadVec(ds, scene->texOps, &ds->T.texOps))) return rc;
     if ((rc = uploadVec(ds, scene->images, &ds->T.images))) return rc;
@@ -494,6 +510,12 @@
     const bool mis = scene->prm.integrator == KZ_INTEGRATOR_PATH_MIS;
     KzParams P = scene->prm;
     if (!mis) { P.anyInvisibleLight = 0; P.nIlTris = 0; P.shadowFast = 1; }
+    KzDevTables Tsh = ds->T;
+    if (ds->statsOn) Tsh.nEmTris = KZ_EM_OFF;
+#ifdef KZ_EXPERIMENTS
+    { const int mode = g_kzRrAhead.load(std::memory_order_relaxed);
+      if (mode == 0) Tsh.nEmTris = KZ_EM_OFF; else if (mode == 2) Tsh.nEmTris = ds->T.nEmTris; }
+#endif
     KzWf W = c.wf;
     W.outJx = c.plane[0]; W.outJy = c.plane[1]; W.outR = c.plane[2]; W.outG = c.plane[3]; W.outB = c.plane[4]; W.stats = ds->stats;
     const bool st = ds->statsOn;
@@ -578,7 +600,7 @@
         }
         for (int iter = 0; iter < maxDepth; ++iter) {
             uint32_t *nextQ = W.queue[iter & 1], *nextCount = W.counts + 4 * (iter + 1), *shQ = W.queue[2], *shCount = W.counts + 4 * (iter + 1) + 1;
-#define KZ_SHADE(ST, EX) hipLaunchKernelGGL((kz_wf_shade<ST, EX>), gShade, blk, 0, stream, P, ds->T, W, pixList, Sp, sBegin, iter, cur, curCount, items, nextQ, nextCount, shQ, shCount)
+#define KZ_SHADE(ST, EX) hipLaunchKernelGGL((kz_wf_shade<ST, EX>), gShade, blk, 0, stream, P, Tsh, W, pixList, Sp, sBegin, iter, cur, curCount, items, nextQ, nextCount, shQ, shCount)
             const int xsel = P.bsdfExt == 0 ? 0 : (P.bsdfExt == KZ_X_MODELS ? KZ_X_MODELS : KZ_X_ALL);
             if (st) { if (xsel == KZ_X_ALL) KZ_SHADE(true, KZ_X_ALL); else if (xsel) KZ_SHADE(true, KZ_X_MODELS); else KZ_SHADE(true, 0); }
             else { if (xsel == KZ_X_ALL) KZ_SHADE(false, KZ_X_ALL); else if (xsel) KZ_SHADE(false, KZ_X_MODELS); else KZ_SHADE(false, 0); }
diff --git a/nano-kazen_amd/csrc/kz_state.h b/nano-kazen_amd/csrc/kz_state.h
--- a/nano-kazen_amd/csrc/kz_state.h
+++ b/nano-kazen_amd/csrc/kz_state.h
@@ -56,6 +56,7 @@
 void kzTraceLine(const char *fmt, ...);
 #define KZ_TRACE(...) do { if (g_kzTrace.load(std::memory_order_relaxed)) kzTraceLine(__VA_ARGS__); } while (0)
 int kzPhysicalDevice(int logical);
+extern std::atomic<int> g_kzRrAhead;
 #else
 #define KZ_TRACE(...) do { } while (0)
 static inline int kzPhysicalDevice(int logical) { return logical; }
@@ -185,6 +186,7 @@
 static inline KzReplicaSet *replicaSet(const KzScene *scene) { return (KzReplicaSet *)scene->dev; }
 int findReplica(const KzScene *scene, int device, KzDeviceState **out);
 int kzEnsureBvh2(KzScene *scene, KzDeviceState *ds);
+int kzEmitterUpload(KzScene *scene, KzDeviceState *ds);
 static inline int requireDevice(KzScene *scene, KzDeviceState **out) { return findReplica(scene, -1, out); }
 size_t packedFloats(const KzParams &P, const KzTile *tiles, uint32_t nTiles);
 int checkTiles(const KzParams &P, const KzTile *tiles, uint32_t nTiles);
diff --git a/nano-kazen_amd/csrc/kz_wavefront.h b/nano-kazen_amd/csrc/kz_wavefront.h
--- a/nano-kazen_amd/csrc/kz_wavefront.h
+++ b/nano-kazen_amd/csrc/kz_wavefront.h
@@ -133,6 +133,45 @@
 #endif
 };
 
+__device__ __forceinline__ bool wfRouletteEnds(V3 throughput, float eta, float draw, float &probability) {
+    probability = fminf(maxCoeff(throughput) * eta * eta, 0.95f);
+    return probability <= draw;
+}
+
+__device__ __forceinline__ bool wfEmitterBox(const KzDevTables &T, V3 o, V3 d, float tmin) {
+    const float rx = rcpExact(d.x), ry = rcpExact(d.y), rz = rcpExact(d.z);
+    float t0 = (T.emLo[0] - o.x) * rx, t1 = (T.emHi[0] - o.x) * rx;
+    float n = fminf(t0, t1), f = fmaxf(t0, t1);
+    t0 = (T.emLo[1] - o.y) * ry; t1 = (T.emHi[1] - o.y) * ry; n = fmaxf(n, fminf(t0, t1)); f = fminf(f, fmaxf(t0, t1));
+    t0 = (T.emLo[2] - o.z) * rz; t1 = (T.emHi[2] - o.z) * rz; n = fmaxf(n, fminf(t0, t1)); f = fminf(f, fmaxf(t0, t1));
+    f *= 1.0000004f;
+    return fmaxf(n, tmin) <= f;
+}
+__device__ __forceinline__ bool wfEmitterHit(const KzDevTables &T, bool cand, V3 o, V3 d, float tmin) {
+    const unsigned long long m = __ballot(cand);
+    if (m == 0) return false;
+    const uint32_t n = T.nEmTris;
+    const uint32_t lane = threadIdx.x & 63u;
+    bool hit = false;
+    float t, u, v; uint32_t g;
+    if (__ballot(true) == ~0ull && (uint32_t)__popcll(m) < n) {
+        const float4 *tp = reinterpret_cast<const float4 *>(T.emTris + min(lane, n - 1u));
+        const float4 a = tp[0], b = tp[1], c = tp[2];
+        for (unsigned long long r = m; r; r &= r - 1ull) {
+            const int src = __ffsll(r) - 1;
+            const V3 so = mk(__int_as_float(__builtin_amdgcn_readlane(__float_as_int(o.x), src)), __int_as_float(__builtin_amdgcn_readlane(__float_as_int(o.y), src)),
+                             __int_as_float(__builtin_amdgcn_readlane(__float_as_int(o.z), src)));
+            const V3 sd = mk(__int_as_float(__builtin_amdgcn_readlane(__float_as_int(d.x), src)), __int_as_float(__builtin_amdgcn_readlane(__float_as_int(d.y), src)),
+                             __int_as_float(__builtin_amdgcn_readlane(__float_as_int(d.z), src)));
+            const bool h = lane < n && triTestV(a, b, c, so, sd, tmin, KZ_INF, t, u, v, g);
+            if (__ballot(h) != 0ull && lane == (uint32_t)src) hit = true;
+        }
+    } else if (cand) {
+        for (uint32_t i = 0; i < n && !hit; ++i) hit = triTest(T.emTris + i, o, d, tmin, KZ_INF, t, u, v, g);
+    }
+    return hit;
+}
+
 template <bool STATS, int EXT>
 __device__ __forceinline__ bool wfClassify(const KzParams &P, const KzDevTables &T, const KzWf &W, const uint32_t *__restrict__ pixList, uint32_t S, uint32_t sampleBegin,
                                            int iter, bool compact, uint32_t slot, Its &its, uint32_t &modelKey, Counters &cn, KzSst &sst) {
@@ -186,8 +225,8 @@
         const float4 th = kzLoadStream(&W.thr[slot]);
         V3 throughput = mk(th.x, th.y, th.z);
         const float etaA = compact ? 1.f : th.w;
-        const float probability = fminf(maxCoeff(throughput) * etaA * etaA, 0.95f);
-        if (probability <= smp.next1D(P, T)) survivor = false;
+        float probability;
+        if (wfRouletteEnds(throughput, etaA, smp.next1D(P, T), probability)) survivor = false;
         else {
             throughput = throughput / probability;
             kzStoreStream(&W.thr[slot], make_float4(throughput.x, throughput.y, throughput.z, th.w));
@@ -200,7 +239,8 @@
             Sampler smp; wfLoadSampler(P, W, slot, (int)(pxy & 0xffffu), (int)(pxy >> 16), sampleBegin + (slot - pl * S), smp, wfPmjDim(P, iter));
             const float4 th = kzLoadStream(&W.thr[slot]);
             const float etaA = compact ? 1.f : th.w;
-            if (fminf(maxCoeff(mk(th.x, th.y, th.z)) * etaA * etaA, 0.95f) <= smp.next1D(P, T)) alive = false;
+            float probability;
+            if (wfRouletteEnds(mk(th.x, th.y, th.z), etaA, smp.next1D(P, T), probability)) alive = false;
         }
         if (alive) cn.lsamples++;
     }
@@ -246,6 +286,7 @@
         }
     }
     sst.mark(4);
+    if (!(iter + 1 < P.maxDepth || P.bgPresent)) return;
     if (P.regularization && bsdf.type == KZ_BSDF_KAZENSTANDARD) accRough += bsdf.roughness * P.accumulatedRoughness;
     float s2x, s2y; smp.next2D(P, T, s2x, s2y);
     const float s1 = smp.next1D(P, T);
@@ -255,17 +296,31 @@
     sst.mark(6);
     throughput = throughput * weight;
     const float etaNext = eta * etaScale;
-    if (ok && !(weight.x == 0.f && weight.y == 0.f && weight.z == 0.f)) {
-        const float bpdf = pdfS >= 0.f ? pdfS : surfPdf<EXT>(bsdf, nm, its, wiLocal, woLocal, accRough, solid);
-        const V3 nd = toWorld(its.sh, woLocal);
-        if (iter + 1 < P.maxDepth || P.bgPresent) {
-            kzStoreStream(&W.rayA[slot], make_float4(its.p.x, its.p.y, its.p.z, eps));
-            kzStoreStream(&W.rayB[slot], make_float4(nd.x, nd.y, nd.z, KZ_INF));
-            kzStoreStream(&W.thr[slot], make_float4(throughput.x, throughput.y, throughput.z, compact ? bpdf : etaNext));
-            if (!compact) kzStoreStream(&W.misc[slot], make_float4(bpdf, accRough, discrete ? 1.f : 0.f, 0.f));
-            wfStoreSampler(P, W, slot, smp);
-            pushNext = true;
-        }
+    bool keep = ok && !(weight.x == 0.f && weight.y == 0.f && weight.z == 0.f);
+    float bpdf = 0.f; V3 nd = mk(0.f);
+    if (keep) {
+        bpdf = pdfS >= 0.f ? pdfS : surfPdf<EXT>(bsdf, nm, its, wiLocal, woLocal, accRough, solid);
+        nd = toWorld(its.sh, woLocal);
+    }
+    if (iter + 1 >= 3 && T.nEmTris != KZ_EM_OFF) {
+        bool cand = false;
+        if (keep) {
+            Sampler peek = smp;
+            float probability;
+            if (wfRouletteEnds(throughput, compact ? 1.f : etaNext, peek.next1D(P, T), probability)) {
+                keep = false;
+                cand = T.nEmTris != 0u && rayIsFinite(its.p, nd) && wfEmitterBox(T, its.p, nd, eps);
+            }
+        }
+        if (wfEmitterHit(T, cand, its.p, nd, eps)) keep = true;
+    }
+    if (keep) {
+        kzStoreStream(&W.rayA[slot], make_float4(its.p.x, its.p.y, its.p.z, eps));
+        kzStoreStream(&W.rayB[slot], make_float4(nd.x, nd.y, nd.z, KZ_INF));
+        kzStoreStream(&W.thr[slot], make_float4(throughput.x, throughput.y, throughput.z, compact ? bpdf : etaNext));
+        if (!compact) kzStoreStream(&W.misc[slot], make_float4(bpdf, accRough, discrete ? 1.f : 0.f, 0.f));
+        wfStoreSampler(P, W, slot, smp);
+        pushNext = true;
     }
 }
 
```

Result: faster. 1934, median of 6 (+5.0%).
